# chenchen235/SemStereo

Measured on AMD Instinct MI355X. Metric: stereo pairs/sec, hot segment (gwc+concat volumes, 3-D hourglass stack, soft-argmax), 1024x1024 maxdisp=128, higher is better.
Workload: dtype f32; 1 GPU; BASELINE.json configs[1]: 1024x1024, maxdisp=128, batch=1/GPU x 1 GPU(s); features [B,128,H/4,W/4]+[B,256,H/8,W/8] -> disparity; input_sets_rotated=3, execution=steps round-robin on 6 HIP streams (PairPipeline); bit-identical to one stream, conv_engine=f16x3, hip_graph=False

## Files before the change

### include/semstereo_hip.h

```cpp
#ifndef SEMSTEREO_HIP_H
#define SEMSTEREO_HIP_H

#ifdef __cplusplus
extern "C" {
#endif

typedef void* ss_stream_t;

enum ss_status {
    SS_OK = 0,
    SS_ERR_INVALID = -1,
    SS_ERR_UNSUPPORTED = -2,
    SS_ERR_LAUNCH = -3
};

int ss_abi_version(void);
int ss_reload_tuning(void);
int ss_set_fill_hint(int pairs_in_flight);
int ss_get_fill_hint(void);
const char* ss_status_string(int status);
const char* ss_last_hip_error(void);


int ss_groupwise_correlation_fwd(const float* fea1, const float* fea2, float* out,
                                 int B, int C, int H, int W, int groups, int normalize,
                                 ss_stream_t stream);

int ss_gwc_volume_fwd(const float* ref, const float* tgt, float* out,
                      int B, int C, int H, int W, int dmin, int ndisp, int groups, int normalize,
                      ss_stream_t stream);
int ss_gwc_patch_gate_fwd(const float* ref, const float* tgt, const float* patch_w, const float* gate_logits, float* out,
                          int B, int C, int H, int W, int dmin, int ndisp, int groups, int normalize, ss_stream_t stream);
int ss_gwc_volume_bwd(const float* grad_out, const float* ref, const float* tgt,
                      float* grad_ref, float* grad_tgt,
                      int B, int C, int H, int W, int dmin, int ndisp, int groups,
                      ss_stream_t stream);

int ss_concat_volume_fwd(const float* ref, const float* tgt, float* out,
                         int B, int C, int H, int W, int dmin, int ndisp, int mask_left, ss_stream_t stream);
int ss_concat_volume_bwd(const float* grad_out, float* grad_ref, float* grad_tgt,
                         int B, int C, int H, int W, int dmin, int ndisp, int mask_left, ss_stream_t stream);

int ss_warp_sampled_fwd(const float* x, const float* y, const float* disp,
                        float* y_warped, float* x_warped,
                        int B, int C, int H, int W, int nd, ss_stream_t stream);
int ss_warp_sampled_bwd(const float* grad_y_warped, const float* grad_x_warped, const float* y, const float* disp,
                        float* grad_x, float* grad_y, float* grad_disp, int B, int C, int H, int W, int nd,
                        ss_stream_t stream);
int ss_concat_sampled_fwd(const float* left, const float* right, const float* disp, const float* att,
                          float* out, int B, int C, int H, int W, int nd, ss_stream_t stream);
int ss_concat_sampled_bwd(const float* grad_out, const float* left, const float* right, const float* disp, const float* att,
                          float* grad_left, float* grad_right, float* grad_att, int B, int C, int H, int W, int nd, int margin,
                          ss_stream_t stream);
int ss_concat_sampled_presplit_fwd(const float* right, const float* disp, const float* att, void* xs, int* xexp,
                                   int B, int C, int H, int W, int nd, ss_stream_t stream);
int ss_stem_left_fwd(const float* q, const float* att, float* out, int B, int Cout, int nd, int H, int W,
                     ss_stream_t stream);
int ss_stem_left_fused_fwd(const float* left, const void* wsplit, const float* att, float* out, int B, int C,
                           int Cout, int nd, int H, int W, int nterms, ss_stream_t stream);
int ss_stem_left_mfma_fwd(const float* left, const void* wsplit, const float* att, float* out, int B, int C,
                          int Cout, int nd, int H, int W, ss_stream_t stream);
int ss_pack_stem_left_weights_f16s(const float* w, void* wsplit, int Cout, int C, ss_stream_t stream);
int ss_pack_stem_left_weights_f16s_bytes(int Cout, int C, long long* bytes);
int ss_warp_correlation_fwd(const float* x, const float* y, const float* disp, float* out,
                            int B, int C, int H, int W, int nd, ss_stream_t stream);

int ss_disparity_regression_fwd(const float* prob, float* out, int B, int dmin, int ndisp, int H, int W,
                                ss_stream_t stream);
int ss_disparity_regression_bwd(const float* grad_out, float* grad_prob, int B, int dmin, int ndisp, int H, int W,
                                ss_stream_t stream);
int ss_disparity_variance_fwd(const float* prob, const float* disparity, float* out,
                              int B, int dmin, int ndisp, int H, int W, ss_stream_t stream);
int ss_softmax_regression_fwd(const float* logits, float* prob, float* disp, float* var,
                              int B, int dmin, int ndisp, int H, int W, ss_stream_t stream);
int ss_upsample_softmax_regression_fwd(const float* coarse, float* up, float* disp, float* var,
                                       int B, int dmin, int ndisp, int H, int W, ss_stream_t stream);

int ss_sample_strength_fwd(const float* left, const float* right, const float* pred0, const float* var,
                           const float* gamma, const float* beta, float* strength,
                           int B, int C, int H, int W, ss_stream_t stream);
int ss_topk_candidates_fwd(const float* logits, const float* strength, float* samples, float* att_topk,
                           float* pred_att, int B, int dmin, int ndisp, int H, int W, int k, ss_stream_t stream);

int ss_regression_topk_fwd(const float* cost, const float* samples, float* out,
                           int B, int nd, int H, int W, int k, ss_stream_t stream);
int ss_regression_topk_bwd(const float* grad_out, const float* cost, const float* samples, float* grad_cost,
                           float* grad_samples, int B, int nd, int H, int W, int k, ss_stream_t stream);

int ss_ssr_upsample_fwd(const float* depth_low, const float* weights, const float* pred_label,
                        const float* params, float* out, int B, int h, int w, int num_classes,
                        ss_stream_t stream);
int ss_ssr_param_count(void);
int ss_ssr_upsample_train_fwd(const float* depth_low, const float* weights, const float* pred_label, const float* params,
                              float* out, float* saved, float* rm0, float* rv0, long long* nbt0, float* rma, float* rva,
                              long long* nbta, float* rm1, float* rv1, long long* nbt1, float* rm2, float* rv2, long long* nbt2,
                              float eps0, float epsa, float eps1, float eps2, double mom0, double moma, double mom1, double mom2,
                              int batch_stats, int B, int h, int w, int num_classes, double* workspace, long long workspace_bytes,
                              ss_stream_t stream);
int ss_ssr_upsample_train_bwd(const float* depth_low, const float* weights, const float* pred_label, const float* params,
                              const float* saved, const float* grad_out, float* grad_depth_low, float* grad_weights,
                              float* grad_pred_label, float* grad_params, int batch_stats, int B, int h, int w, int num_classes,
                              double* workspace, long long workspace_bytes, ss_stream_t stream);

int ss_channel_gate_fwd(const float* att_logits, const float* cv, float* out,
                        int B, int C, int D, int H, int W, ss_stream_t stream);

int ss_channel_att_logits_fwd(const float* im, const void* w1_split, const float* scale1, const float* shift1,
                              const void* w2_split, const float* bias2, float* out,
                              int B, int Cin, int Cmid, int Cout, int H, int W, int sigmoid, ss_stream_t stream);

int ss_conv3d_fwd(const float* in, const float* wpack, const float* scale, const float* shift,
                  const float* residual, const float* gate, float* out,
                  int B, int Cin, int D, int H, int W, int Cout, int k, int stride, int relu,
                  ss_stream_t stream);
int ss_conv3d_bf16s_fwd(const float* in, const void* wsplit, const float* scale, const float* shift,
                        const float* residual, const float* gate, float* out,
                        int B, int Cin, int D, int H, int W, int Cout, int stride, int relu, int nterms,
                        ss_stream_t stream);
int ss_conv3d_bf16s_partial_fwd(const float* in, const void* wsplit, const float* partial, const float* scale,
                                const float* shift, const float* gate, float* out,
                                int B, int Cin, int D, int H, int W, int Cout, int relu, int nterms,
                                ss_stream_t stream);
int ss_conv3d_gather_fwd(const float* right, const float* cand, const float* att, const void* wsplit, const float* partial,
                         const float* scale, const float* shift, const float* gate, float* out,
                         int B, int Cin, int nd, int H, int W, int Cout, int relu, int nterms, ss_stream_t stream);
int ss_conv3d_presplit_fwd(const void* xs, const int* xexp, const void* wsplit, const float* partial, const float* scale,
                           const float* shift, const float* gate, float* out, int B, int Cin, int D, int H, int W,
                           int Cout, int relu, ss_stream_t stream);
int ss_pack_conv3d_weights_bf16s(const float* w, void* wsplit, int Cout, int Cin, ss_stream_t stream);
int ss_pack_conv3d_weights_bf16s_bytes(int Cout, int Cin, long long* bytes);
int ss_pack_conv3d_weights_f16s(const float* w, void* wsplit, int Cout, int Cin, ss_stream_t stream);
int ss_pack_conv3d_weights_f16s_bytes(int Cout, int Cin, long long* bytes);
int ss_conv2d_bf16s_fwd(const float* in, const void* wsplit, const float* scale, const float* shift,
                        const float* residual, float* out, int B, int Cin, int H, int W, int Cout, int relu,
                        int nterms, ss_stream_t stream);
int ss_conv2d_bf16s_pair_fwd(const float* in_a, const float* in_b, const void* wsplit, const float* scale, const float* shift,
                             float* out, int B, int Cin, int H, int W, int Cout, int relu, int nterms, ss_stream_t stream);
int ss_pack_conv2d_weights_bf16s(const float* w, void* wsplit, int Cout, int Cin, ss_stream_t stream);
int ss_pack_conv2d_weights_bf16s_bytes(int Cout, int Cin, long long* bytes);
int ss_conv2d_bf16s_cat_fwd(const float* x_a, const float* rem_a, const float* x_b, const float* rem_b, const void* wsplit,
                            const float* scale, const float* shift, float* out, int B, int Csplit, int Cin, int H, int W, int Cout,
                            int relu, int nterms, ss_stream_t stream);
int ss_deconv2d_bf16s_fwd(const float* in, const void* wsplit, const float* scale, const float* shift, float* out, int B, int Cin,
                          int H, int W, int Cout, int relu, int nterms, ss_stream_t stream);
int ss_deconv2d_bf16s_pair_fwd(const float* in_a, const float* in_b, const void* wsplit, const float* scale, const float* shift,
                               float* out, int B, int Cin, int H, int W, int Cout, int relu, int nterms, ss_stream_t stream);
int ss_pack_deconv2d_weights_f16s(const float* w, void* wsplit, int Cin, int Cout, ss_stream_t stream);
int ss_pack_deconv2d_weights_f16s_bytes(int Cin, int Cout, long long* bytes);
int ss_conv2d_k4s2_f16s_fwd(const float* in, const void* wsplit, float* out, int B, int Cin, int H, int W, int Cout, ss_stream_t stream);
int ss_pack_conv2d_k4s2_weights_f16s(const float* w, void* wsplit, int Cout, int Cin, ss_stream_t stream);
int ss_pack_conv2d_k4s2_weights_f16s_bytes(int Cout, int Cin, long long* bytes);
int ss_deconv2d_k4s2_wgrad_fwd(const float* in, const float* grad_out, float* grad_w, float* workspace, int B, int Cin, int H, int W,
                               int Cout, ss_stream_t stream);
int ss_deconv2d_k4s2_wgrad_workspace_bytes(int B, int Cin, int H, int W, int Cout, long long* bytes);
int ss_conv2d_k3_wgrad_fwd(const float* grad_out, const float* in0, const float* in1, float* grad_w, float* workspace, int B, int C0,
                           int C1, int H, int W, int Cout, ss_stream_t stream);
int ss_conv2d_k3_wgrad_workspace_bytes(int B, int C0, int C1, int H, int W, int Cout, long long* bytes);
int ss_conv2d_k1_f16s_fwd(const float* in, const void* wsplit, const float* scale, const float* shift, float* out, int B, int Cin,
                          long long npos, int Cout, int relu, ss_stream_t stream);
int ss_conv2d_k1_f16s_pair_fwd(const float* in_a, const float* in_b, const void* wsplit, const float* scale, const float* shift,
                               float* out, int B, int Cin, long long npos, int Cout, int relu, ss_stream_t stream);
int ss_pack_conv2d_k1_weights_f16s(const float* w, void* wsplit, int Cout, int Cin, ss_stream_t stream);
int ss_pack_conv2d_k1_weights_f16s_bytes(int Cout, int Cin, long long* bytes);
int ss_seghead_logits_fwd(const float* in, const void* wsplit, const float* scale, const float* shift, const float* w2,
                          const float* bias, float* out, int B, int Cin, int H, int W, int K, ss_stream_t stream);
int ss_pack_seghead_weights_f16s(const float* w, void* wsplit, int Cin, ss_stream_t stream);
int ss_pack_seghead_weights_f16s_bytes(int Cin, long long* bytes);
int ss_bilinear_up2_fwd(const float* in, float* out, int B, int C, int H, int W, ss_stream_t stream);
int ss_seghead_tail_fwd(const float* a, const float* w2, const float* bias, float* out, int B, int K, int C, int H, int W, int up2,
                        ss_stream_t stream);
int ss_seghead_tail_bwd(const float* grad_out, const float* a, const float* w2, float* grad_a, float* grad_w2, float* grad_bias,
                        float* workspace, int B, int K, int C, int H, int W, int up2, ss_stream_t stream);
int ss_seghead_tail_workspace_bytes(int B, int K, int C, int H, int W, long long* bytes);
int ss_pack_conv2d_weights_f16s(const float* w, void* wsplit, int Cout, int Cin, ss_stream_t stream);
int ss_pack_conv2d_weights_f16s_bytes(int Cout, int Cin, long long* bytes);
int ss_conv3d_head_bf16s_fwd(const float* in, const void* wsplit, const float* scale, const float* shift,
                             float* out, int B, int Cin, int D, int H, int W, int relu, int nterms,
                             ss_stream_t stream);
int ss_pack_conv3d_head_weights_bf16s(const float* w, void* wsplit, int Cin, ss_stream_t stream);
int ss_pack_conv3d_head_weights_bf16s_bytes(int Cin, long long* bytes);
int ss_pack_conv3d_head_weights_f16s(const float* w, void* wsplit, int Cin, ss_stream_t stream);
int ss_pack_conv3d_head_weights_f16s_bytes(int Cin, long long* bytes);
int ss_conv3d_bf16s_cl_fwd(const float* in, const void* wsplit, const float* scale, const float* shift, float* out,
                           int B, int Cin, int D, int H, int W, int Cout, int relu, int nterms, ss_stream_t stream);
int ss_conv3d_head_bf16s_cl_fwd(const float* in, const void* wsplit, const float* scale, const float* shift,
                                float* out, int B, int Cin, int D, int H, int W, int relu, int nterms,
                                ss_stream_t stream);
int ss_pack_classifier_head_weights(const float* w2, void* out, ss_stream_t stream);
int ss_pack_classifier_head_weights_bytes(long long* bytes);
int ss_conv3d_classifier_fused_fwd(const float* in, const void* wsplit, const float* scale, const float* shift,
                                   const void* head_w, float* patches, float* out, int B, int Cin, int D, int H, int W,
                                   int nterms, ss_stream_t stream);
int ss_regression_topk_patched_fwd(const float* patches, const float* samples, float* out, int B, int nd, int H, int W, int k,
                                   ss_stream_t stream);
int ss_conv3d_pointwise_bf16s_fwd(const float* in, const void* wsplit, const float* scale, const float* shift,
                                  float* out, int B, int Cin, int Cout, long long npos, int relu, int nterms,
                                  ss_stream_t stream);
int ss_pack_pointwise_weights_bf16s(const float* w, void* wsplit, int Cout, int Cin, ss_stream_t stream);
int ss_pack_pointwise_weights_bf16s_bytes(int Cout, int Cin, long long* bytes);

int ss_deconv3d_fwd(const float* in, const float* wpack, const float* scale, const float* shift,
                    const float* skip, const float* skip_wpack, const float* skip_scale, const float* skip_shift,
                    float* out, int B, int Cin, int D, int H, int W, int Cout, int Cs, int relu,
                    ss_stream_t stream);
int ss_deconv3d_bf16s_fwd(const float* in, const void* wsplit, const float* shift, const float* skip,
                          const void* skip_wsplit, float* out, int B, int Cin, int D, int H, int W, int Cout,
                          int Cs, int relu, int nterms, ss_stream_t stream);
int ss_pack_deconv3d_weights_bf16s(const float* wpack, void* wsplit, int Cin, int Cout, int ntaps, ss_stream_t stream);
int ss_pack_deconv3d_weights_bf16s_bytes(int Cin, int Cout, int ntaps, long long* bytes);
int ss_pack_deconv3d_weights_f16s(const float* wpack, void* wsplit, int Cin, int Cout, ss_stream_t stream);
int ss_pack_deconv3d_weights_f16s_bytes(int Cin, int Cout, long long* bytes);
int ss_pack_conv3d_weights(const float* w, float* wpack, int Cout, int Cin, int k, int transposed,
                           ss_stream_t stream);
int ss_conv3d_wgrad_fwd(const float* grad_out, const float* in, float* grad_w, int B, int Cin, int D, int H, int W,
                        int Cout, int stride, ss_stream_t stream);
int ss_conv3d_wgrad_bf16s_fwd(const float* grad_out, const float* in, float* grad_w, float* workspace, int B, int Cin, int D, int H,
                              int W, int Cout, int stride, ss_stream_t stream);

int ss_depthwise_patch_fwd(const float* in, const float* w, const float* gate, float* out,
                           int B, int C, int D, int H, int W, ss_stream_t stream);
int ss_window_attention_fwd(const float* x, const float* wqkv_t, const float* bqkv,
                            const float* wout_t, const float* bout, float* out,
                            int B, int C, int D, int H, int W, int heads, int bd, int bh, int bw,
                            ss_stream_t stream);
int ss_window_attention_core_fwd(const float* qkv, const float* bqkv, float* y, int B, int C, int D, int H,
                                 int W, int heads, int bd, int bh, int bw, ss_stream_t stream);

int ss_batchnorm_train_fwd(const float* x, const float* weight, const float* bias, float* y, float* mean, float* invstd,
                           float* var_unbiased, double* work, int B, int C, long long N, float eps, int relu,
                           ss_stream_t stream);
int ss_batchnorm_train_bwd(const float* grad_y, const float* x, const float* y, const float* mean, const float* invstd,
                           const float* weight, float* grad_x, double* work, int B, int C, long long N, int relu,
                           ss_stream_t stream);
int ss_batchnorm_train_res_fwd(const float* x, const float* residual, const float* weight, const float* bias, float* y, float* mean,
                               float* invstd, float* var_unbiased, double* work, int B, int C, long long N, float eps, int relu,
                               ss_stream_t stream);
int ss_batchnorm_train_res_bwd(const float* grad_y, const float* x, const float* y, const float* mean, const float* invstd,
                               const float* weight, float* grad_x, float* grad_residual, double* work, int B, int C, long long N,
                               int relu, ss_stream_t stream);
int ss_batchnorm_eval_fwd(const float* x, const float* residual, const float* mean, const float* invstd, const float* weight,
                          const float* bias, float* y, int B, int C, long long N, int relu, ss_stream_t stream);
int ss_batchnorm_eval_bwd(const float* grad_y, const float* x, const float* y, const float* mean, const float* invstd,
                          const float* weight, float* grad_x, float* grad_residual, double* work, int B, int C, long long N,
                          int relu, ss_stream_t stream);
int ss_batchnorm_train_fwd_rs(const float* x, const float* residual, const float* weight, const float* bias, float* y, float* mean,
                              float* invstd, float* var_unbiased, double* work, float* running_mean, float* running_var,
                              long long* num_batches_tracked, double momentum, int B, int C, long long N, float eps, int relu,
                              ss_stream_t stream);
int ss_batchnorm_bwd_pg(const float* grad_y, const float* x, const float* y, const float* mean, const float* invstd,
                        const float* weight, const float* bias, float* grad_x, float* grad_residual, double* work, float* grad_weight,
                        float* grad_bias, int batch_statistics, int B, int C, long long N, int relu, ss_stream_t stream);
int ss_group_normalise_fwd(const float* x, float* y, int B, int C, int H, int W, int groups, float eps, ss_stream_t stream);
int ss_group_normalise_bwd(const float* grad_y, const float* x, float* grad_x, int B, int C, int H, int W, int groups, float eps,
                           ss_stream_t stream);
int ss_conv_k1_wgrad_fwd(const float* grad_out, const float* in, float* grad_w, int B, int Cin, int Cout, long long npos,
                         ss_stream_t stream);
int ss_channel_sum_fwd(const float* a, double* sums, int B, int C, long long N, ss_stream_t stream);
int ss_depthwise_patch_wgrad_fwd(const float* grad_out, const float* in, float* grad_w, int B, int C, int D, int H, int W,
                                 ss_stream_t stream);
int ss_channel_gate_bwd_logits(const float* grad_out, const float* cv, const float* att_logits, float* grad_att, int B, int C,
                               int D, int H, int W, ss_stream_t stream);
int ss_window_attention_core_bwd(const float* qkv, const float* grad_y, float* grad_qkv, int B, int C, int D, int H, int W,
                                 int heads, int bd, int bh, int bw, ss_stream_t stream);
int ss_window_attention_core_pad_bwd(const float* qkv, const float* bqkv, const float* grad_y, float* grad_qkv, float* grad_bias, int B,
                                     int C, int D, int H, int W, int heads, int bd, int bh, int bw, ss_stream_t stream);
int ss_upsample_softmax_regression_bwd(const float* up, const float* grad_up, const float* grad_disp, const float* grad_var,
                                       float* grad_coarse, float* work, int B, int dmin, int ndisp, int H, int W, ss_stream_t stream);
int ss_sample_strength_bwd(const float* left, const float* right, const float* pred0, const float* var, const float* gamma,
                           const float* beta, const float* grad_strength, float* grad_left, float* grad_right, float* grad_pred0,
                           float* grad_var, float* grad_gamma_beta, int B, int C, int H, int W, ss_stream_t stream);
int ss_sample_strength_bwd_ws(const float* left, const float* right, const float* pred0, const float* var, const float* gamma,
                              const float* beta, const float* grad_strength, float* grad_left, float* grad_right, float* grad_pred0,
                              float* grad_var, float* grad_gamma_beta, float* work, int B, int C, int H, int W, ss_stream_t stream);
int ss_topk_candidates_bwd(const float* logits, const float* strength, const float* samples, const float* grad_att_topk,
                           const float* grad_pred_att, float* grad_logits, float* grad_strength, int B, int dmin, int ndisp, int H, int W,
                           int k, ss_stream_t stream);
int ss_loss_workspace_bytes(int kind, long long* bytes);
int ss_disparity_loss_fwd(const float* est0, const float* gt0, const unsigned char* mask0, long long n0, const float* est1,
                          const float* gt1, const unsigned char* mask1, long long n1, const float* est2, const float* gt2,
                          const unsigned char* mask2, long long n2, const float* est3, const float* gt3, const unsigned char* mask3,
                          long long n3, float w0, float w1, float w2, float w3, float lo, float hi, int nterms, int l1, double* record,
                          float* loss, double* workspace, long long workspace_bytes, ss_stream_t stream);
int ss_disparity_loss_bwd(const float* est0, const float* gt0, const unsigned char* mask0, float* grad0, long long n0, const float* est1,
                          const float* gt1, const unsigned char* mask1, float* grad1, long long n1, const float* est2, const float* gt2,
                          const unsigned char* mask2, float* grad2, long long n2, const float* est3, const float* gt3,
                          const unsigned char* mask3, float* grad3, long long n3, float w0, float w1, float w2, float w3, float lo,
                          float hi, int nterms, int l1, const double* record, const float* grad_loss, ss_stream_t stream);
int ss_label_loss_fwd(const float* logits, const void* labels, int label_dtype, int B, int num_classes, int H, int W, int ignore, float scale,
                      double* record, float* loss, double* workspace, long long workspace_bytes, ss_stream_t stream);
int ss_label_loss_bwd(const float* logits, const void* labels, int label_dtype, int B, int num_classes, int H, int W, int ignore, float scale,
                      const double* record, const float* grad_loss, float* grad_logits, ss_stream_t stream);
int ss_lrsc_loss_fwd(const float* logits_right, const float* disp, const void* labels, int label_dtype, int B, int num_classes, int H, int W,
                     double* record, float* loss, long long* warped, double* workspace, long long workspace_bytes, ss_stream_t stream);
int ss_lrsc_loss_bwd(const float* logits_right, const float* disp, const void* labels, int label_dtype, int B, int num_classes, int H, int W,
                     const double* record, const float* grad_loss, float* grad_logits, ss_stream_t stream);
int ss_metrics_workspace_bytes(int kind, long long* bytes);
int ss_disparity_metrics_fwd(const float* est0, const float* est1, const float* est2, const float* est3, const float* gt,
                             const unsigned char* mask, const unsigned char* mask_img, int n_est, int B, long long pixels_per_image,
                             float lo, float hi, float t0, float t1, float t2, float t3, int n_thr, float* out, long long* counts,
                             double* sums, void* workspace, long long workspace_bytes, ss_stream_t stream);
int ss_seg_confusion_fwd(const float* logits, const void* labels, int label_dtype, int B, int num_classes, int H, int W,
                         long long label_row_stride, long long label_image_stride, long long* joint, int accumulate, void* workspace,
                         long long workspace_bytes, ss_stream_t stream);
int ss_vis_workspace_bytes(int kind, long long* bytes);
int ss_disp_error_image_fwd(const float* est, const float* gt, const float* table, int B, int H, int W, float abs_thres, float rel_thres,
                            int legend, int is_signed, float lo, float hi, float* out, ss_stream_t stream);
int ss_class_color_fwd(const void* src, int src_dtype, int B, int num_classes, int H, int W, long long label_row_stride,
                       long long label_image_stride, void* out, int out_dtype, ss_stream_t stream);
int ss_image_minmax_fwd(const float* x, int B, long long elements_per_image, float* minmax, void* workspace, long long workspace_bytes,
                        ss_stream_t stream);
int ss_image_normalize_fwd(const float* x, const float* minmax, float* out, int B, int C, long long pixels_per_channel, ss_stream_t stream);
int ss_prep_workspace_bytes(int B, int H, int W, long long* bytes);
int ss_prep_views_fwd(const unsigned char* left, const unsigned char* right, const float* table, int B, int H, int W, float* out_left,
                      float* out_right, ss_stream_t stream);
int ss_prep_pyramid_fwd(const void* disparity, int disp_dtype, float disp_scale, const void* label, int label_dtype,
                        long long label_row_stride, long long label_image_stride, int B, int H, int W, float* disparity_out,
                        float* disparity_4, float* disparity_8, float* disparity_16, float* label_out, float* label_2, float* label_4,
                        ss_stream_t stream);
int ss_prep_luma_stats_fwd(const unsigned char* left, int B, int H, int W, void* workspace, long long workspace_bytes, ss_stream_t stream);
int ss_prep_gradients_fwd(const void* workspace, long long workspace_bytes, int B, int H, int W, float* gx, float* gy, ss_stream_t stream);
int ss_tool_copy_fwd(const void* src, void* dst, long long bytes, ss_stream_t stream);

#ifdef __cplusplus
}
#endif
#endif
```

### semstereo_amd/csrc/deconv3d_bf16s.hip

```cpp
#include <algorithm>
#include <type_traits>

#include "common.h"
#include "split_f16.h"

namespace {

using ss_u32x2 = __attribute__((ext_vector_type(2))) unsigned;

__host__ __device__ constexpr int tap_of(int s) {
    constexpr int T[27] = {13, 14, 16, 17, 22, 23, 25, 26, 12, 15, 21, 24, 10, 11, 19, 20, 9, 18, 4, 5, 7, 8, 3, 6, 1, 2, 0};
    return T[s];
}
__host__ __device__ constexpr int cls_of(int s) {
    constexpr int T[27] = {0, 1, 2, 3, 4, 5, 6, 7, 1, 3, 5, 7, 2, 3, 6, 7, 3, 7, 4, 5, 6, 7, 5, 7, 6, 7, 7};
    return T[s];
}
__host__ __device__ constexpr int off_of(int s) {
    constexpr int T[27] = {0, 0, 0, 0, 0, 0, 0, 0, 1, 1, 1, 1, 2, 2, 2, 2, 3, 3, 4, 4, 4, 4, 5, 5, 6, 6, 7};
    return T[s];
}

constexpr int KST = 27;
#ifndef SS_DECONV_XCD
#define SS_DECONV_XCD 0
#endif
#ifndef SS_DECONV_SKIP_AUX
#define SS_DECONV_SKIP_AUX 0
#endif

struct GrpTable { int ns; int step[KST]; int next_off[KST]; };
constexpr bool grp_has(int grp, int cls) { return grp < 0 || (grp == 0 ? (cls < 2 || cls >= 6) : (cls >= 2 && cls < 6)); }
constexpr GrpTable make_grp_table(int grp) {
    GrpTable t{};
    for (int s = 0; s < KST; ++s)
        if (grp_has(grp, cls_of(s))) t.step[t.ns++] = s;
    for (int k = t.ns; k < KST; ++k) t.step[k] = KST - 1;
    for (int k = 0; k < KST; ++k) {
        t.next_off[k] = -1;
        for (int j = k + 1; j < t.ns; ++j)
            if (off_of(t.step[j]) != off_of(t.step[k])) { t.next_off[k] = off_of(t.step[j]); break; }
    }
    return t;
}
template <int GRP>
struct Grp {
    static constexpr int NA = GRP < 0 ? 8 : 4;
    static constexpr int NQ2 = GRP < 0 ? 4 : 2;
    static constexpr int idx(int cls) { return GRP < 0 ? cls : (GRP == 0 ? (cls < 2 ? cls : cls - 4) : cls - 2); }
    static constexpr int q(int j) { return GRP < 0 ? j : (GRP == 0 ? (j == 0 ? 0 : 3) : (j == 0 ? 1 : 2)); }
    static constexpr GrpTable T = make_grp_table(GRP);
    static constexpr int NS = T.ns;
};
struct GroupSteps { int s[2][16]; };
constexpr GroupSteps make_group_steps() {
    GroupSteps t{};
    for (int k = 0; k < 16; ++k) { t.s[0][k] = Grp<0>::T.step[k]; t.s[1][k] = Grp<1>::T.step[k]; }
    return t;
}
__device__ const GroupSteps kGroupSteps = make_group_steps();

template <int TD, int TH, int LT = 3, bool WLDS = false, int WSTEPS = 27>
struct DB {
    static constexpr int ID = TD + 1, IH = TH + 1, IW = 33;
    static constexpr int CS = ID * IH * IW;
    static constexpr int NPOS = (CS + 255) / 256;
    static constexpr int WSLOTS = WLDS ? WSTEPS * 2 * 64 : 0;
    static constexpr size_t LDS_BYTES = (size_t)(LT * 2 * CS + 1 + 16 + WSLOTS) * 16;
    static_assert(TD * TH == 4, "4 waves x one input row each");
};

template <int TD, int TH, int NTERMS, bool HAS_SKIP, bool SPLIT = false, bool ACCB = false, bool STREAM = false>
__global__ __launch_bounds__(256, (SPLIT && !ACCB) ? 3 : 2) void deconv3d_bf16s(const float* __restrict__ in, const uint4* __restrict__ wsplit,
                                                          const float* __restrict__ shift, const float* __restrict__ skip,
                                                          const uint4* __restrict__ skip_wsplit, float* __restrict__ out,
                                                          int Cin, int D, int H, int W, int Cout, int Cs, int tiles_w,
                                                          int tiles_h, int relu, int nunits) {
    static_assert(!SPLIT || NTERMS == F16X3, "the class-group split exists for the fp16 form (weights through LDS)");
    static_assert(!ACCB || SPLIT, "chunk-blocked accumulation: in the registers the split frees");
    constexpr bool F16 = (NTERMS == F16X3);
    constexpr int NC = (NTERMS == 6) ? 3 : 2;
    constexpr int NCW = F16 ? 2 : 3;
    using C = DB<TD, TH, NC, F16, SPLIT ? 15 : 27>;
    constexpr int MSLOT = NC * 2 * C::CS;
    constexpr int WL = MSLOT + 1 + 16;
    extern __shared__ __attribute__((aligned(16))) uint4 lds[];
    const int tid = threadIdx.x, lane = tid & 63, wave = tid >> 6;
    const int l31 = lane & 31, half = lane >> 5;
    int iw0 = 0, ih0 = 0, id0 = 0, grp = -1;
    auto unit_origin = [&](int u, int& w0, int& h0, int& d0) {
        int t = SPLIT ? (u >> 1) : u;
        const int tw = t % tiles_w; t /= tiles_w;
        const int th = t % tiles_h; t /= tiles_h;
        w0 = tw * 32; h0 = th * TH; d0 = t * TD;
    };
    const int co0 = blockIdx.y * 32;
    const int b = blockIdx.z;
    const int dzw = wave / TH, hyw = wave % TH;
    const int lane_pos = (dzw * C::IH + hyw) * C::IW + l31;

    const size_t in_plane = (size_t)H * W, chan = (size_t)D * in_plane;
    const float* inb = in + (size_t)b * Cin * chan;

    unsigned poff[C::NPOS];
    auto make_poff = [&](int u) {
        int w0, h0, d0;
        unit_origin(u, w0, h0, d0);
#pragma unroll
        for (int i = 0; i < C::NPOS; ++i) {
            const int p = tid + 256 * i;
            const int wx = p % C::IW;
            int r = p / C::IW;
            const int hy = r % C::IH, dz = r / C::IH;
            const int gw = w0 + wx, gh = h0 + hy, gd = d0 + dz;
            const bool ok = (p < C::CS) && gd < D && gh < H && gw < W && u < nunits;
            poff[i] = ok ? (unsigned)(((size_t)gd * in_plane + (size_t)gh * W + gw) * 4) : 0x80000000u;
        }
    };
    constexpr int NQ = 16 * C::NPOS;
    float rin[NQ];

    const int nchunks = (Cin + 15) / 16;
    const int G = nchunks * KST;
    const int wlane = (half * Cout + min(co0 + l31, Cout - 1)) * 16;
    const int wstep = NCW * 2 * Cout * 16;
    const int swstep = 3 * 2 * Cout * 16;
    const float* wunscale = reinterpret_cast<const float*>(reinterpret_cast<const char*>(wsplit) + (size_t)G * wstep);
    const __amdgpu_buffer_rsrc_t wres = __builtin_amdgcn_make_buffer_rsrc(
        const_cast<uint4*>(wsplit), 0, (int)min((long long)G * wstep, 0x7fffffffLL), 0x00020000);
    const __amdgpu_buffer_rsrc_t ires = __builtin_amdgcn_make_buffer_rsrc(
        const_cast<float*>(inb), 0, (int)min((long long)Cin * (long long)chan * 4, 0x7fffffffLL), 0x00020000);
    const int chan_b = (int)(chan * 4);
    auto load_a = [&](int g, int c) {
        return __builtin_bit_cast(uint4, __builtin_amdgcn_raw_buffer_load_b128(wres, wlane, g * wstep + c * 2 * Cout * 16, 0));
    };
    auto load_in = [&](int ch, int i) {
        return __builtin_bit_cast(float, __builtin_amdgcn_raw_buffer_load_b32(ires, (int)poff[i], min(ch, Cin - 1) * chan_b, 0));
    };
    auto load_in_masked = [&](int ch, int i, unsigned mask) {
        return __builtin_bit_cast(float, __builtin_amdgcn_raw_buffer_load_b32(ires, (int)(poff[i] | mask), min(ch, Cin - 1) * chan_b, 0));
    };
    constexpr int AQ = F16 ? 2 : 3;
    uint4 aq[AQ][NC];

    const int Do = 2 * D, Ho = 2 * H, Wo = 2 * W;
    const size_t out_plane = (size_t)Ho * Wo;
    float* aff = reinterpret_cast<float*>(&lds[MSLOT + 1]);
    if (tid < 32) {
        const int co = min(co0 + tid, Cout - 1);
        aff[tid] = shift ? shift[co] : 0.0f;
        aff[32 + tid] = F16 ? wunscale[co] : 1.0f;
    }
    constexpr int SNT = F16 ? 6 : NTERMS, SNC = (SNT == 6) ? 3 : 2;
    auto body = [&](auto grp_tag, const int unit) {
    constexpr int GRP = decltype(grp_tag)::value;
    using GP = Grp<GRP>;
    constexpr int NA = GP::NA, NS = GP::NS;
    constexpr bool XPF = false;
    const bool has_next = XPF && unit + (int)gridDim.x < nunits;
    if (!XPF) {
        make_poff(unit);
#pragma unroll
        for (int q = 0; q < NQ; ++q) rin[q] = load_in(q / C::NPOS, q % C::NPOS);
    }
    if (!F16) {
#pragma unroll
        for (int k = 0; k < 2; ++k)
#pragma unroll
            for (int c = 0; c < NC; ++c) aq[k][c] = load_a(min(k, G - 1), c);
    }
    f32x16 acc[NA];
#pragma unroll
    for (int p = 0; p < NA; ++p)
#pragma unroll
        for (int r = 0; r < 16; ++r) acc[p][r] = 0.f;
    auto skip_phase = [&]() {
#ifdef SS_EXP_DECONV_NOSKIP
        return;
#endif
        const size_t schan = (size_t)Do * out_plane;
        const int jw_ = min(iw0 + l31, W - 1), jd_ = min(id0 + dzw, D - 1), jh_ = min(ih0 + hyw, H - 1);
        const __amdgpu_buffer_rsrc_t sres = __builtin_amdgcn_make_buffer_rsrc(
            const_cast<float*>(skip + (size_t)b * Cs * schan), 0, (int)min((long long)Cs * (long long)schan * 4, 0x7fffffffLL), 0x00020000);
        const int nks = (Cs + 15) / 16;
        const __amdgpu_buffer_rsrc_t swres = __builtin_amdgcn_make_buffer_rsrc(
            const_cast<uint4*>(skip_wsplit), 0, nks * swstep, 0x00020000);
        const unsigned lane_s = (unsigned)(((size_t)(2 * jd_) * out_plane + (size_t)(2 * jh_) * Wo + 2 * jw_) * 4);
        const unsigned schan_b = (unsigned)(schan * 4);
        auto batch_load = [&](float2 (&v)[2][8], int ks, auto q0_tag, unsigned dead) {
            constexpr int q0 = decltype(q0_tag)::value;
#pragma unroll
            for (int q = 0; q < 2; ++q) {
                const unsigned qo = (unsigned)(((size_t)(GP::q(q0 + q) >> 1) * out_plane + (size_t)(GP::q(q0 + q) & 1) * Wo) * 4);
#pragma unroll
                for (int j = 0; j < 8; ++j) {
                    const int cs = ks * 16 + 8 * half + j;
                    v[q][j] = __builtin_bit_cast(float2, __builtin_amdgcn_raw_buffer_load_b64(
                                                             sres, (int)((lane_s + qo + (unsigned)min(cs, Cs - 1) * schan_b) | dead), 0, SS_DECONV_SKIP_AUX));
                }
            }
        };
        auto batch_mfma = [&](float2 (&v)[2][8], int ks, auto q0_tag, const bf16x8 (&a)[SNC]) {
            constexpr int q0 = decltype(q0_tag)::value;
#pragma unroll
            for (int q = 0; q < 2; ++q) {
#pragma unroll
                for (int j = 0; j < 8; ++j)
                    if (ks * 16 + 8 * half + j >= Cs) v[q][j] = make_float2(0.f, 0.f);
#pragma unroll
                for (int pw = 0; pw < 2; ++pw) {
                    unsigned bh[4], bm[4], bl[4];
#pragma unroll
                    for (int c = 0; c < 4; ++c)
                        split3_pk(pw ? v[q][2 * c].y : v[q][2 * c].x, pw ? v[q][2 * c + 1].y : v[q][2 * c + 1].x, bh[c], bm[c], bl[c]);
                    const bf16x8 h8 = __builtin_bit_cast(bf16x8, make_uint4(bh[0], bh[1], bh[2], bh[3]));
                    const bf16x8 m8 = __builtin_bit_cast(bf16x8, make_uint4(bm[0], bm[1], bm[2], bm[3]));
                    const int cls = (q0 + q) * 2 + pw;
                    if (SNT == 6) {
                        const bf16x8 l8 = __builtin_bit_cast(bf16x8, make_uint4(bl[0], bl[1], bl[2], bl[3]));
                        acc[cls] = __builtin_amdgcn_mfma_f32_32x32x16_bf16(a[1], m8, acc[cls], 0, 0, 0);
                        acc[cls] = __builtin_amdgcn_mfma_f32_32x32x16_bf16(a[0], l8, acc[cls], 0, 0, 0);
                        acc[cls] = __builtin_amdgcn_mfma_f32_32x32x16_bf16(a[SNC - 1], h8, acc[cls], 0, 0, 0);
                    }
                    acc[cls] = __builtin_amdgcn_mfma_f32_32x32x16_bf16(a[0], m8, acc[cls], 0, 0, 0);
                    acc[cls] = __builtin_amdgcn_mfma_f32_32x32x16_bf16(a[1], h8, acc[cls], 0, 0, 0);
                    acc[cls] = __builtin_amdgcn_mfma_f32_32x32x16_bf16(a[0], h8, acc[cls], 0, 0, 0);
                }
            }
        };
        using Q0 = std::integral_constant<int, 0>;
        using Q2 = std::integral_constant<int, 2>;
#pragma unroll 1
        for (int ks = 0; ks < nks; ++ks) {
            bf16x8 a[SNC];
#pragma unroll
            for (int c = 0; c < SNC; ++c)
                a[c] = __builtin_bit_cast(bf16x8, __builtin_amdgcn_raw_buffer_load_b128(swres, wlane, ks * swstep + c * 2 * Cout * 16, 0));
            float2 v[2][8];
            batch_load(v, ks, Q0{}, 0u);
            __builtin_amdgcn_sched_barrier(0);
            batch_mfma(v, ks, Q0{}, a);
            if constexpr (GP::NQ2 == 4) {
                batch_load(v, ks, Q2{}, 0u);
                __builtin_amdgcn_sched_barrier(0);
                batch_mfma(v, ks, Q2{}, a);
            }
        }
    };


    const bool skip_first = !SPLIT && HAS_SKIP && ((unit ^ blockIdx.y) & 1);
    if (HAS_SKIP && skip_first) {
        skip_phase();
        if (F16) {
#pragma unroll
            for (int r = 0; r < 16; ++r) {
                const float ws = __uint_as_float((254u << 23) - __float_as_uint(wunscale[min(co0 + (r & 3) + 8 * (r >> 2) + 4 * half, Cout - 1)]));
#pragma unroll
                for (int p = 0; p < NA; ++p) acc[p][r] *= ws;
            }
        }
    }
    BlockExp bexp;
    auto publish_max = [&](float m0) {
        const unsigned wm = wave_max_bits(__float_as_uint(abs_max<false>(rin, m0)));
        if (lane == 0) reinterpret_cast<unsigned*>(&lds[MSLOT])[wave] = wm;
    };
    if (F16) {
        float m0 = 0.f;
        if (HAS_SKIP && skip_first) {
#pragma unroll
            for (int p = 0; p < NA; ++p)
#pragma unroll
                for (int r = 0; r < 16; ++r) m0 = fmaxf(m0, fabsf(acc[p][r]));
            m0 *= pow2_biased(127 - E_INIT_SHIFT);
        }
        publish_max(m0);
        __syncthreads();
    }
    const int nchunks_run = nchunks;
    for (int ck = 0, g0 = 0; ck < nchunks_run; ++ck, g0 += KST) {
        const int ci0 = ck * 16;
        if (F16) {
            int wv = __builtin_amdgcn_readfirstlane(wave);
            asm volatile("" : "+s"(wv));
#pragma unroll
            for (int k = 0; k < (NS * 2 + 3) / 4; ++k) {
                const int i = wv + 4 * k;
                if (i < NS * 2) {
                    const int sg = GRP < 0 ? i / 2 : __builtin_amdgcn_readfirstlane(kGroupSteps.s[GRP < 0 ? 0 : GRP][i / 2]);
                    lds_dma16(wres, &lds[WL + i * 64], wlane, (g0 + sg) * wstep + (i & 1) * 2 * Cout * 16);
                }
            }
        }
        float in_scale = 1.f;
        if (F16) {
            if (bexp.advance(lds[MSLOT])) {
                const float ratio = bexp.rescale();
#pragma unroll
                for (int p = 0; p < NA; ++p)
#pragma unroll
                    for (int r = 0; r < 16; ++r) acc[p][r] *= ratio;
            }
            in_scale = bexp.in_scale();
        }
#pragma unroll
        for (int i = 0; i < C::NPOS; ++i) {
            const int p = tid + 256 * i;
            if (p >= C::CS) continue;
#pragma unroll
            for (int hf = 0; hf < 2; ++hf) {
                unsigned hh[4], mm[4], ll[4];
#pragma unroll
                for (int c = 0; c < 4; ++c) {
                    const int c0 = hf * 8 + 2 * c;
                    const float x0 = (ci0 + c0 < Cin) ? rin[c0 * C::NPOS + i] : 0.f;
                    const float x1 = (ci0 + c0 + 1 < Cin) ? rin[(c0 + 1) * C::NPOS + i] : 0.f;
                    if (F16) split2_pk_f16(x0 * in_scale, x1 * in_scale, hh[c], mm[c]);
                    else split3_pk(x0, x1, hh[c], mm[c], ll[c]);
                }
                lds[(0 * 2 + hf) * C::CS + p] = make_uint4(hh[0], hh[1], hh[2], hh[3]);
                lds[(1 * 2 + hf) * C::CS + p] = make_uint4(mm[0], mm[1], mm[2], mm[3]);
                if (NC == 3) lds[(2 * 2 + hf) * C::CS + p] = make_uint4(ll[0], ll[1], ll[2], ll[3]);
            }
        }
#ifndef SS_EXP_DECONV_NOWAIT
        if (F16) __builtin_amdgcn_s_waitcnt(0x0F70);
#endif
        __syncthreads();
        const bool more = ck + 1 < nchunks;
        if (XPF && !more) make_poff(unit + (int)gridDim.x);
        const unsigned nomore = (more || has_next) ? 0u : 0x80000000u;
        const int ch_next = more ? ci0 + 16 : 0;

        uint4 bcur[NC], bnxt[NC];
        auto read_b = [&](uint4 (&dst)[NC], int o) {
            const int slot = lane_pos + (((o >> 2) & 1) * C::IH + ((o >> 1) & 1)) * C::IW + (o & 1);
#pragma unroll
            for (int c = 0; c < NC; ++c) dst[c] = lds[(c * 2 + half) * C::CS + slot];
        };
        constexpr int QSG = (NQ + (NS * 20 / 27) - 1) / (NS * 20 / 27);
        read_b(bcur, off_of(GP::T.step[0]));
        if (F16) {
#pragma unroll
            for (int c = 0; c < NC; ++c) aq[0][c] = lds[WL + c * 64 + lane];
        }
        f32x16 tacc[ACCB ? NA : 1];
        if constexpr (ACCB) {
#pragma unroll
            for (int p = 0; p < NA; ++p)
#pragma unroll
                for (int r = 0; r < 16; ++r) tacc[p][r] = 0.f;
        }
#pragma unroll
        for (int k = 0; k < NS; ++k) {
            const int s = GP::T.step[k];
            if (!F16) {
#pragma unroll
                for (int c = 0; c < NC; ++c) aq[(s + 2) % AQ][c] = load_a(min(g0 + s + 2, G - 1), c);
            } else if (k + 1 < NS) {
#pragma unroll
                for (int c = 0; c < NC; ++c) aq[(k + 1) % AQ][c] = lds[WL + ((k + 1) * 2 + c) * 64 + lane];
            }
#pragma unroll
            for (int q = k * QSG; q < (k + 1) * QSG && q < NQ; ++q) rin[q] = load_in_masked(ch_next + q / C::NPOS, q % C::NPOS, nomore);
            if ((k == 0 || off_of(s) != off_of(GP::T.step[k > 0 ? k - 1 : 0])) && GP::T.next_off[k] >= 0) read_b(bnxt, GP::T.next_off[k]);
            const int ai = GP::idx(cls_of(s));
            f32x16& dst = ACCB ? tacc[ACCB ? ai : 0] : acc[ai];
            if (F16) {
                f16x8 a[NC], bq[NC];
#pragma unroll
                for (int c = 0; c < NC; ++c) {
                    a[c] = __builtin_bit_cast(f16x8, aq[k % AQ][c]);
                    bq[c] = __builtin_bit_cast(f16x8, bcur[c]);
                }
                dst = __builtin_amdgcn_mfma_f32_32x32x16_f16(a[0], bq[1], dst, 0, 0, 0);
                dst = __builtin_amdgcn_mfma_f32_32x32x16_f16(a[1], bq[0], dst, 0, 0, 0);
                dst = __builtin_amdgcn_mfma_f32_32x32x16_f16(a[0], bq[0], dst, 0, 0, 0);
            } else {
                bf16x8 a[NC], bq[NC];
#pragma unroll
                for (int c = 0; c < NC; ++c) {
                    a[c] = __builtin_bit_cast(bf16x8, aq[s % AQ][c]);
                    bq[c] = __builtin_bit_cast(bf16x8, bcur[c]);
                }
                if (NTERMS == 6) {
                    dst = __builtin_amdgcn_mfma_f32_32x32x16_bf16(a[1], bq[1], dst, 0, 0, 0);
                    dst = __builtin_amdgcn_mfma_f32_32x32x16_bf16(a[0], bq[NC - 1], dst, 0, 0, 0);
                    dst = __builtin_amdgcn_mfma_f32_32x32x16_bf16(a[NC - 1], bq[0], dst, 0, 0, 0);
                }
                dst = __builtin_amdgcn_mfma_f32_32x32x16_bf16(a[0], bq[1], dst, 0, 0, 0);
                dst = __builtin_amdgcn_mfma_f32_32x32x16_bf16(a[1], bq[0], dst, 0, 0, 0);
                dst = __builtin_amdgcn_mfma_f32_32x32x16_bf16(a[0], bq[0], dst, 0, 0, 0);
            }
            if (k + 1 < NS && off_of(GP::T.step[k + 1 < NS ? k + 1 : k]) != off_of(s)) {
#pragma unroll
                for (int c = 0; c < NC; ++c) bcur[c] = bnxt[c];
            }
            __builtin_amdgcn_sched_barrier(0);
        }
        if constexpr (ACCB) {
#pragma unroll
            for (int p = 0; p < NA; ++p)
#pragma unroll
                for (int r = 0; r < 16; ++r) acc[p][r] += tacc[p][r];
        }
        if (F16 && more) publish_max(0.f);
        __syncthreads();
    }
    if (F16) {
        const float au = bexp.acc_unscale();
#pragma unroll
        for (int r = 0; r < 16; ++r) {
            const float un = au * aff[32 + (r & 3) + 8 * (r >> 2) + 4 * half];
#pragma unroll
            for (int p = 0; p < NA; ++p) acc[p][r] *= un;
        }
    }

    if (HAS_SKIP && !skip_first) skip_phase();

    const int jw = iw0 + l31, jd = id0 + dzw, jh = ih0 + hyw;
    const unsigned ochan_b = (unsigned)((size_t)Do * out_plane * 4);
    const __amdgpu_buffer_rsrc_t ores = __builtin_amdgcn_make_buffer_rsrc(
        out + (size_t)b * Cout * Do * out_plane, 0, (int)min((long long)Cout * (long long)ochan_b, 0x7fffffffLL), 0x00020000);
    const bool ok = jw < W && jd < D && jh < H;
    unsigned vo[GP::NQ2];
#pragma unroll
    for (int j = 0; j < GP::NQ2; ++j)
        vo[j] = ok ? (unsigned)((((size_t)(2 * jd + (GP::q(j) >> 1)) * Ho + 2 * jh + (GP::q(j) & 1)) * Wo + 2 * jw) * 4) + 4u * half * ochan_b
                   : 0x80000000u;
    const float floor_v = relu ? 0.f : -__builtin_inff();
#pragma unroll
    for (int r = 0; r < 16; ++r) {
        const int cb = co0 + (r & 3) + 8 * (r >> 2);
        const bool cok = cb + 4 * half < Cout;
        const float sh = aff[(r & 3) + 8 * (r >> 2) + 4 * half];
#pragma unroll
        for (int j = 0; j < GP::NQ2; ++j) {
            const float v0 = fmaxf(ss::add_rn(acc[j * 2 + 0][r], sh), floor_v);
            const float v1 = fmaxf(ss::add_rn(acc[j * 2 + 1][r], sh), floor_v);
#ifdef SS_EXP_DECONV_NOSTORE
            if (r == 0 && j == 0)
#endif
            __builtin_amdgcn_raw_buffer_store_b64(__builtin_bit_cast(ss_u32x2, make_float2(v0, v1)), ores,
                                                  (int)(cok ? vo[j] : 0x80000000u), cb * (int)ochan_b, STREAM ? 2 : 0);
        }
    }
    };
#if SS_DECONV_XCD
    const int unit = [&]() {
        const int x = blockIdx.x & 7, j = blockIdx.x >> 3, q = nunits >> 3, r = nunits & 7;
        return x * q + min(x, r) + j;
    }();
#else
    const int unit = blockIdx.x;
#endif
    unit_origin(unit, iw0, ih0, id0);
    if constexpr (!SPLIT) {
        body(std::integral_constant<int, -1>{}, unit);
    } else {
        grp = unit & 1;
        if (grp == 0) body(std::integral_constant<int, 0>{}, unit);
        else body(std::integral_constant<int, 1>{}, unit);
    }
}

__global__ void pack_deconv_weights_kernel(const float* __restrict__ wpack, unsigned short* __restrict__ wsplit, int Cin,
                                           int Cout, int ntaps, long long total) {
    const long long i = blockIdx.x * (long long)blockDim.x + threadIdx.x;
    if (i >= total) return;
    const int j = (int)(i % 8);
    long long r = i / 8;
    const int co = (int)(r % Cout); r /= Cout;
    const int hf = (int)(r % 2); r /= 2;
    const int term = (int)(r % 3); r /= 3;
    const int s = (int)(r % ntaps);
    const int chunk = (int)(r / ntaps);
    const int ci = chunk * 16 + hf * 8 + j;
    const int tap = (ntaps == 27) ? tap_of(s) : 0;
    const float x = (ci < Cin) ? wpack[((size_t)ci * ntaps + tap) * Cout + co] : 0.f;
    unsigned h, m, l;
    split3_pk(x, 0.f, h, m, l);
    wsplit[i] = (unsigned short)((term == 0 ? h : (term == 1 ? m : l)) & 0xffffu);
}

__global__ __launch_bounds__(256) void deconv_weight_unscale_f16s_kernel(const float* __restrict__ wpack, float* __restrict__ wunscale,
                                                                          int Cout, int rows) {
    __shared__ unsigned wmax[4];
    float m = 0.f;
    for (int i = threadIdx.x; i < rows; i += 256) m = fmaxf(m, fabsf(wpack[(size_t)i * Cout + blockIdx.x]));
    const float u = weight_unscale(m, wmax);
    if (threadIdx.x == 0) wunscale[blockIdx.x] = u;
}
__global__ void pack_deconv_weights_f16s_kernel(const float* __restrict__ wpack, unsigned short* __restrict__ wsplit,
                                                const float* __restrict__ wunscale, int Cin, int Cout, long long total) {
    const long long i = blockIdx.x * (long long)blockDim.x + threadIdx.x;
    if (i >= total) return;
    const int j = (int)(i % 8);
    long long r = i / 8;
    const int co = (int)(r % Cout); r /= Cout;
    const int hf = (int)(r % 2); r /= 2;
    const int term = (int)(r % 2); r /= 2;
    const int s = (int)(r % 27);
    const int chunk = (int)(r / 27);
    const int ci = chunk * 16 + hf * 8 + j;
    const float x = (ci < Cin) ? wpack[((size_t)ci * 27 + tap_of(s)) * Cout + co] / wunscale[co] : 0.f;
    wsplit[i] = split_weight_f16(x, term);
}

template <int TD, int TH, int NTERMS, bool HAS_SKIP, bool SPLIT = false, bool ACCB = false, bool STREAM = false>
int launch_db(const float* in, const void* wsplit, const float* shift, const float* skip, const void* skip_wsplit, float* out,
              int B, int Cin, int D, int H, int W, int Cout, int Cs, int relu, hipStream_t st) {
    using C = DB<TD, TH, (NTERMS == 6) ? 3 : 2, NTERMS == F16X3, SPLIT ? 15 : 27>;
    const int tiles_w = ss::ceil_div(W, 32), tiles_h = ss::ceil_div(H, TH), tiles_d = ss::ceil_div(D, TD);
    const long long nt = (long long)tiles_w * tiles_h * tiles_d;
    if (nt > 0x7fffffffLL || B > 65535) return SS_ERR_UNSUPPORTED;
    auto kern = deconv3d_bf16s<TD, TH, NTERMS, HAS_SKIP, SPLIT, ACCB, STREAM>;
    if (C::LDS_BYTES > 64 * 1024) {
        if (ss::ensure_dynamic_lds(reinterpret_cast<const void*>(kern), (int)C::LDS_BYTES) != SS_OK) return SS_ERR_LAUNCH;
    }
    if (nt > 0x3fffffffLL) return SS_ERR_UNSUPPORTED;
    const long long nunits = SPLIT ? 2 * nt : nt;
    dim3 grid((unsigned)nunits, ss::ceil_div(Cout, 32), B);
    hipLaunchKernelGGL(kern, grid, dim3(256), C::LDS_BYTES, st, in, reinterpret_cast<const uint4*>(wsplit), shift, skip,
                       reinterpret_cast<const uint4*>(skip_wsplit), out, Cin, D, H, W, Cout, Cs, tiles_w, tiles_h, relu, (int)nunits);
    return ss::check_launch();
}

template <int TD, int TH>
int launch_db_all(const float* in, const void* wsplit, const float* shift, const float* skip, const void* skip_wsplit,
                  float* out, int B, int Cin, int D, int H, int W, int Cout, int Cs, int relu, int nterms, hipStream_t st) {
#define SS_DB(NTERMS, HAS_SKIP) launch_db<TD, TH, NTERMS, HAS_SKIP>(in, wsplit, shift, skip, skip_wsplit, out, B, Cin, D, H, W, Cout, Cs, relu, st)
#define SS_DF(HAS_SKIP, SPLIT, ACCB, STREAM) \
    launch_db<TD, TH, F16X3, HAS_SKIP, SPLIT, ACCB, STREAM>(in, wsplit, shift, skip, skip_wsplit, out, B, Cin, D, H, W, Cout, Cs, relu, st)
    if (nterms == F16X3) {
        const long long per_pair = (long long)ss::ceil_div(W, 32) * ss::ceil_div(H, TH) * ss::ceil_div(D, TD) * ss::ceil_div(Cout, 32);
        int groups = ss::tuning().deconv_groups;
        if (groups < 0) groups = per_pair < 256 ? 2 : 0;
        const int stream_env = ss::tuning().deconv_stream;
        const bool stream = stream_env >= 0 ? stream_env != 0 : (long long)B * Cout * 8 * D * H * W * 4 >= (192LL << 20);
        if (groups == 2) return skip != nullptr ? SS_DF(true, true, true, false) : SS_DF(false, true, true, false);
        if (groups == 1) return skip != nullptr ? SS_DF(true, true, false, false) : SS_DF(false, true, false, false);
        if (stream) return skip != nullptr ? SS_DF(true, false, false, true) : SS_DF(false, false, false, true);
        return skip != nullptr ? SS_DF(true, false, false, false) : SS_DF(false, false, false, false);
    }
    if (skip != nullptr) return nterms == 6 ? SS_DB(6, true) : SS_DB(3, true);
    return nterms == 6 ? SS_DB(6, false) : SS_DB(3, false);
#undef SS_DF
#undef SS_DB
}

}

static ss::Packed deconv_packed(int Cin, int Cout, int ntaps, bool f16) {
    const long long terms = (long long)ss::ceil_div(Cin, 16) * ntaps * (f16 ? 2 : 3) * 2 * Cout * 16;
    return {terms, terms + (f16 ? 4LL * Cout : 0)};
}

extern "C" int ss_pack_deconv3d_weights_bf16s_bytes(int Cin, int Cout, int ntaps, long long* bytes) {
    SS_REQUIRE(bytes && Cin > 0 && Cout > 0 && (ntaps == 27 || ntaps == 1));
    *bytes = deconv_packed(Cin, Cout, ntaps, false).total;
    return SS_OK;
}

extern "C" int ss_pack_deconv3d_weights_f16s_bytes(int Cin, int Cout, long long* bytes) {
    SS_REQUIRE(bytes && Cin > 0 && Cout > 0);
    *bytes = deconv_packed(Cin, Cout, 27, true).total;
    return SS_OK;
}

extern "C" int ss_pack_deconv3d_weights_bf16s(const float* wpack, void* wsplit, int Cin, int Cout, int ntaps, ss_stream_t stream) {
    SS_REQUIRE(wpack && wsplit && Cin > 0 && Cout > 0 && (ntaps == 27 || ntaps == 1));
    const long long total = deconv_packed(Cin, Cout, ntaps, false).terms / 2;
    hipLaunchKernelGGL(pack_deconv_weights_kernel, dim3((unsigned)ss::ceil_div_ll(total, 256)), dim3(256), 0, ss::as_stream(stream),
                       wpack, reinterpret_cast<unsigned short*>(wsplit), Cin, Cout, ntaps, total);
    return ss::check_launch();
}

extern "C" int ss_pack_deconv3d_weights_f16s(const float* wpack, void* wsplit, int Cin, int Cout, ss_stream_t stream) {
    SS_REQUIRE(wpack && wsplit && Cin > 0 && Cout > 0);
    const ss::Packed p = deconv_packed(Cin, Cout, 27, true);
    const long long total = p.terms / 2;
    float* wunscale = ss::scales_of(wsplit, p);
    hipLaunchKernelGGL(deconv_weight_unscale_f16s_kernel, dim3(Cout), dim3(256), 0, ss::as_stream(stream), wpack, wunscale, Cout, Cin * 27);
    hipLaunchKernelGGL(pack_deconv_weights_f16s_kernel, dim3((unsigned)ss::ceil_div_ll(total, 256)), dim3(256), 0, ss::as_stream(stream),
                       wpack, reinterpret_cast<unsigned short*>(wsplit), wunscale, Cin, Cout, total);
    return ss::check_launch();
}

extern "C" int ss_deconv3d_bf16s_fwd(const float* in, const void* wsplit, const float* shift, const float* skip,
                                     const void* skip_wsplit, float* out, int B, int Cin, int D, int H, int W, int Cout,
                                     int Cs, int relu, int nterms, ss_stream_t stream) {
    SS_REQUIRE(in && wsplit && out);
    SS_REQUIRE(B > 0 && Cin > 0 && D > 0 && H > 0 && W > 0 && Cout > 0 && (nterms == 3 || nterms == 6 || nterms == F16X3));
    SS_REQUIRE((skip == nullptr) || (skip_wsplit != nullptr && Cs > 0));
    SS_REQUIRE((reinterpret_cast<uintptr_t>(wsplit) & 15) == 0 && (reinterpret_cast<uintptr_t>(skip_wsplit) & 15) == 0);
    if ((reinterpret_cast<uintptr_t>(out) & 7) != 0) return SS_ERR_INVALID;
    if ((long long)Cin * D * H * W * 4 >= 0x7fffffffLL) return SS_ERR_UNSUPPORTED;
    if (skip != nullptr && (long long)Cs * 8 * D * H * W * 4 >= 0x7fffffffLL) return SS_ERR_UNSUPPORTED;
    if ((long long)Cout * 8 * D * H * W * 4 >= 0x7fffffffLL) return SS_ERR_UNSUPPORTED;
    hipStream_t st = ss::as_stream(stream);
    if (D >= 2 && H < 4)
        return launch_db_all<2, 2>(in, wsplit, shift, skip, skip_wsplit, out, B, Cin, D, H, W, Cout, Cs, relu, nterms, st);
    return launch_db_all<1, 4>(in, wsplit, shift, skip, skip_wsplit, out, B, Cin, D, H, W, Cout, Cs, relu, nterms, st);
}
```

### semstereo_amd/csrc/window_attention.hip

```cpp
#include <algorithm>

#include "common.h"
#include "split_f16.h"

namespace {


constexpr int HD = 8;
constexpr int HG = 4;

template <int T, int C>
struct ACfg {
    static constexpr int NTL = (T + 31) / 32;
    static constexpr int TP = NTL * 32;
    static constexpr int XS = C * TP;
    static constexpr int QKV = 3 * 32 * TP;
    static constexpr int YG = 32 * TP;
    static constexpr int FLAGS = TP;
    static constexpr int WL = C * 96;
    static constexpr size_t LDS_BYTES = (size_t)(XS + QKV + YG + FLAGS + WL) * 4;
};

template <int T, int C>
__global__ __launch_bounds__(256) void window_attention_kernel(
    const float* __restrict__ x, const float* __restrict__ wqkv_t, const float* __restrict__ bqkv,
    const float* __restrict__ wout_t, const float* __restrict__ bout, float* __restrict__ out, int D, int H, int W,
    int bd, int bh, int bw, int nwh, int nww, int use_mask) {
    using A = ACfg<T, C>;
    extern __shared__ __attribute__((aligned(16))) float lds[];
    float* xs = lds;
    float* qkv = xs + A::XS;
    float* yg = qkv + A::QKV;
    float* flag = yg + A::YG;
    float* wl = flag + A::FLAGS;

    const int tid = threadIdx.x, lane = tid & 63, wave = tid >> 6;
    const int l31 = lane & 31, half = lane >> 5;
    int wi = blockIdx.x;
    const int ww = wi % nww; wi /= nww;
    const int wh = wi % nwh; wi /= nwh;
    const int wd = wi;
    const int b = blockIdx.y;
    const size_t plane = (size_t)H * W, vol = (size_t)D * plane;
    const float* xb = x + (size_t)b * C * vol;

    if (bw == 4 && (W & 3) == 0 && ((reinterpret_cast<uintptr_t>(x) & 15) == 0)) {
        constexpr int NQ = C * (A::TP / 4) / 256;
        static_assert(C * (A::TP / 4) % 256 == 0, "whole batches");
#pragma unroll
        for (int i = 0; i < NQ; ++i) {
            const int e = tid + 256 * i;
            const int tq = e % (A::TP / 4), c = e / (A::TP / 4);
            const int ih = tq % bh, id = tq / bh;
            const int gh = wh * bh + ih, gd = wd * bd + id, gw = ww * 4;
            const bool ok = gh < H && gw < W;
            const float4 q = *reinterpret_cast<const float4*>(xb + (size_t)c * vol + (size_t)gd * plane +
                                                              (size_t)min(gh, H - 1) * W + min(gw, W - 4));
            *reinterpret_cast<float4*>(&xs[e * 4]) = ok ? q : make_float4(0.f, 0.f, 0.f, 0.f);
        }
    } else {
        for (int e = tid; e < C * A::TP; e += 256) {
            const int t = e % A::TP, c = e / A::TP;
            float v = 0.f;
            if (t < T) {
                const int iw = t % bw, ih = (t / bw) % bh, id = t / (bw * bh);
                const int gw = ww * bw + iw, gh = wh * bh + ih, gd = wd * bd + id;
                if (gh < H && gw < W) v = xb[(size_t)c * vol + (size_t)gd * plane + (size_t)gh * W + gw];
            }
            xs[e] = v;
        }
    }
    for (int t = tid; t < A::TP; t += 256) {
        float f = 0.f;
        if (t < T) {
            const int iw = t % bw, ih = (t / bw) % bh;
            f = ((wh * bh + ih >= H) || (ww * bw + iw >= W)) ? 1.f : 0.f;
        }
        flag[t] = f;
    }
    __syncthreads();

    static_assert(C == 128, "4 waves x 32 output channels");
    f32x16 oacc[A::NTL];
#pragma unroll
    for (int n = 0; n < A::NTL; ++n)
#pragma unroll
        for (int r = 0; r < 16; ++r) oacc[n][r] = 0.f;

    const float scale = 0.35355339059327379f;
    constexpr int NGROUPS = C / (HG * HD);

    constexpr int NWQ = C * 24 / 256;
    float4 wreg[NWQ];
    const float* wsrc[NWQ];
#pragma unroll
    for (int i = 0; i < NWQ; ++i) {
        const int e = tid + 256 * i;
        wsrc[i] = wqkv_t + (size_t)(e / 24) * 3 * C + ((e % 24) / 8) * C + ((e % 24) % 8) * 4;
        wreg[i] = *reinterpret_cast<const float4*>(wsrc[i]);
    }

    for (int g = 0; g < NGROUPS; ++g) {
#pragma unroll
        for (int i = 0; i < NWQ; ++i) {
            const int e = tid + 256 * i;
            *reinterpret_cast<float4*>(&wl[(e / 24) * 96 + (e % 24) * 4]) = wreg[i];
        }
        __syncthreads();
        if (g + 1 < NGROUPS) {
#pragma unroll
            for (int i = 0; i < NWQ; ++i) wreg[i] = *reinterpret_cast<const float4*>(wsrc[i] + (g + 1) * 32);
        }
        for (int u = wave; u < 3 * A::NTL; u += 4) {
            const int mt = u / A::NTL, nt = u % A::NTL;
            const int f0 = mt * C + g * 32;
            f32x16 acc;
#pragma unroll
            for (int r = 0; r < 16; ++r) acc[r] = 0.f;
            const float* ap = wl + half * 96 + mt * 32 + l31;
            const float* bp = xs + half * A::TP + nt * 32 + l31;
#pragma unroll 8
            for (int kk = 0; kk < C; kk += 2)
                acc = __builtin_amdgcn_mfma_f32_32x32x2f32(ap[kk * 96], bp[kk * A::TP], acc, 0, 0, 0);
#pragma unroll
            for (int r = 0; r < 16; ++r) {
                const int row = (r & 3) + 8 * (r >> 2) + 4 * half;
                qkv[(mt * 32 + row) * A::TP + nt * 32 + l31] = ss::add_rn(acc[r], bqkv[f0 + row]);
            }
        }
        __syncthreads();

        static_assert(A::TP == T, "windows of 64 / 96 tokens are whole 32-token tiles");
        for (int u = wave; u < HG * A::NTL; u += 4) {
            const int hh = u / A::NTL, qt = u % A::NTL;
            f32x16 st[A::NTL];
#pragma unroll
            for (int kt = 0; kt < A::NTL; ++kt) {
#pragma unroll
                for (int r = 0; r < 16; ++r) st[kt][r] = 0.f;
#pragma unroll
                for (int sd = 0; sd < HD / 2; ++sd)
                    st[kt] = __builtin_amdgcn_mfma_f32_32x32x2f32(
                        qkv[(32 + hh * HD + 2 * sd + half) * A::TP + kt * 32 + l31],
                        qkv[(hh * HD + 2 * sd + half) * A::TP + qt * 32 + l31],
                        st[kt], 0, 0, 0);
            }
            const float fq = flag[qt * 32 + l31];
            float mx = -INFINITY;
#pragma unroll
            for (int kt = 0; kt < A::NTL; ++kt)
#pragma unroll
                for (int r = 0; r < 16; ++r) {
                    float d = ss::mul_rn(st[kt][r], scale);
                    if (use_mask && flag[kt * 32 + (r & 3) + 8 * (r >> 2) + 4 * half] != fq) d = ss::add_rn(d, -1000.0f);
                    st[kt][r] = d;
                    mx = fmaxf(mx, d);
                }
            mx = fmaxf(mx, __shfl_xor(mx, 32));
            float sum = 0.f;
#pragma unroll
            for (int kt = 0; kt < A::NTL; ++kt)
#pragma unroll
                for (int r = 0; r < 16; ++r) { st[kt][r] = ss::exp_fast(st[kt][r] - mx); sum = ss::add_rn(sum, st[kt][r]); }
            sum = ss::add_rn(sum, __shfl_xor(sum, 32));
            const float rsum = 1.0f / sum;
            f32x16 ot;
#pragma unroll
            for (int r = 0; r < 16; ++r) ot[r] = 0.f;
            const float* vrow = qkv + (64 + hh * HD + (l31 & 7)) * A::TP + 4 * half;
#pragma unroll
            for (int kt = 0; kt < A::NTL; ++kt)
#pragma unroll
                for (int r = 0; r < 16; ++r) {
                    const float vv = (l31 < HD) ? vrow[kt * 32 + (r & 3) + 8 * (r >> 2)] : 0.f;
                    ot = __builtin_amdgcn_mfma_f32_32x32x2f32(vv, ss::mul_rn(st[kt][r], rsum), ot, 0, 0, 0);
                }
#pragma unroll
            for (int r = 0; r < 4; ++r) yg[(hh * HD + 4 * half + r) * A::TP + qt * 32 + l31] = ot[r];
        }
        __syncthreads();

        {
            const float* ap = wout_t + (size_t)(g * 32 + half) * C + wave * 32 + l31;
            const float* bp = yg + half * A::TP + l31;
#pragma unroll
            for (int kk = 0; kk < 32; kk += 2) {
                const float a = ap[(size_t)kk * C];
#pragma unroll
                for (int n = 0; n < A::NTL; ++n)
                    oacc[n] = __builtin_amdgcn_mfma_f32_32x32x2f32(a, bp[kk * A::TP + n * 32], oacc[n], 0, 0, 0);
            }
        }
        __syncthreads();
    }

    float* ob = out + (size_t)b * C * vol;
#pragma unroll
    for (int n = 0; n < A::NTL; ++n) {
        const int t = n * 32 + l31;
        if (t >= T) continue;
        const int iw = t % bw, ih = (t / bw) % bh, id = t / (bw * bh);
        const int gw = ww * bw + iw, gh = wh * bh + ih, gd = wd * bd + id;
        if (gh >= H || gw >= W) continue;
        const size_t pos = (size_t)gd * plane + (size_t)gh * W + gw;
#pragma unroll
        for (int r = 0; r < 16; ++r) {
            const int co = wave * 32 + (r & 3) + 8 * (r >> 2) + 4 * half;
            ob[(size_t)co * vol + pos] = ss::add_rn(oacc[n][r], bout[co]);
        }
    }
}

template <int T, int C>
__global__ __launch_bounds__(256) void window_attention_core(const float* __restrict__ qkv_in, const float* __restrict__ bqkv,
                                                              float* __restrict__ y, int D, int H, int W, int bd, int bh,
                                                              int bw, int nwh, int nww, int use_mask) {
    using A = ACfg<T, C>;
    static_assert(A::TP == T, "windows of 64 / 96 tokens are whole 32-token tiles");
    __shared__ __attribute__((aligned(16))) float qkv[3 * 32 * A::TP];
    __shared__ float flag[A::TP];
    const int tid = threadIdx.x, lane = tid & 63, wave = tid >> 6;
    const int l31 = lane & 31, half = lane >> 5;
    constexpr int NGROUPS = C / (HG * HD);
    int wi = blockIdx.x;
    const int g = wi % NGROUPS; wi /= NGROUPS;
    const int ww = wi % nww; wi /= nww;
    const int wh = wi % nwh; wi /= nwh;
    const int wd = wi;
    const int b = blockIdx.y;
    const size_t plane = (size_t)H * W, vol = (size_t)D * plane;
    const float* qb = qkv_in + (size_t)b * 3 * C * vol;

    __shared__ unsigned vmax_w[4];
    float vm = 0.f;
    if (bw == 4 && (W & 3) == 0 && ((reinterpret_cast<uintptr_t>(qkv_in) & 15) == 0)) {
        constexpr int NQ = 96 * (A::TP / 4) / 256;
        static_assert(96 * (A::TP / 4) % 256 == 0, "whole batches");
#pragma unroll
        for (int i = 0; i < NQ; ++i) {
            const int e = tid + 256 * i;
            const int tq = e % (A::TP / 4), row = e / (A::TP / 4);
            const int f = (row >> 5) * C + g * 32 + (row & 31);
            const int ih = tq % bh, id = tq / bh;
            const int gh = wh * bh + ih, gd = wd * bd + id, gw = ww * 4;
            const bool ok = gh < H && gw < W;
            const float4 q = *reinterpret_cast<const float4*>(qb + (size_t)f * vol + (size_t)gd * plane +
                                                              (size_t)min(gh, H - 1) * W + min(gw, W - 4));
            const float bf = bqkv[f];
            const float4 v4 = ok ? q : make_float4(bf, bf, bf, bf);
            *reinterpret_cast<float4*>(&qkv[e * 4]) = v4;
            if (row >= 64) vm = fmaxf(vm, fmaxf(fmaxf(fabsf(v4.x), fabsf(v4.y)), fmaxf(fabsf(v4.z), fabsf(v4.w))));
        }
    } else {
        for (int e = tid; e < 96 * A::TP; e += 256) {
            const int t = e % A::TP, row = e / A::TP;
            const int f = (row >> 5) * C + g * 32 + (row & 31);
            const int iw = t % bw, ih = (t / bw) % bh, id = t / (bw * bh);
            const int gw = ww * bw + iw, gh = wh * bh + ih, gd = wd * bd + id;
            const float v1 = (gh < H && gw < W) ? qb[(size_t)f * vol + (size_t)gd * plane + (size_t)gh * W + gw] : bqkv[f];
            qkv[e] = v1;
            if (row >= 64) vm = fmaxf(vm, fabsf(v1));
        }
    }
    {
        const unsigned wm = wave_max_bits(__float_as_uint(vm));
        if (lane == 0) vmax_w[wave] = wm;
    }
    for (int t = tid; t < A::TP; t += 256) {
        const int iw = t % bw, ih = (t / bw) % bh;
        flag[t] = ((wh * bh + ih >= H) || (ww * bw + iw >= W)) ? 1.f : 0.f;
    }
    __syncthreads();

    const float scale = 0.35355339059327379f;
    const int e_v = workgroup_exponent(vmax_w);
    const float v_scale = scale_for(e_v);
    const float pv_unscale = unscale_for(e_v) * (1.0f / 16384.0f);
    for (int wk = tid; wk < 32 * (A::TP / 16); wk += 256) {
        float* base = qkv + (64 + wk / (A::TP / 16)) * A::TP + (wk % (A::TP / 16)) * 16;
        float f[16];
#pragma unroll
        for (int k4 = 0; k4 < 4; ++k4) ss::lds_read16(base + 4 * k4, &f[4 * k4]);
#pragma unroll
        for (int h = 0; h < 2; ++h) {
            unsigned hi[4], lo[4];
#pragma unroll
            for (int j = 0; j < 4; ++j) {
                const int t0 = (j < 2) ? 4 * h + 2 * j : 8 + 4 * h + 2 * (j - 2);
                split2_pk_f16(f[t0] * v_scale, f[t0 + 1] * v_scale, hi[j], lo[j]);
            }
            *reinterpret_cast<uint4*>(base + 8 * h) = make_uint4(hi[0], hi[1], hi[2], hi[3]);
            *reinterpret_cast<uint4*>(base + 8 * h + 4) = make_uint4(lo[0], lo[1], lo[2], lo[3]);
        }
    }
    __syncthreads();
    float* yb = y + (size_t)b * C * vol;
    for (int u = wave; u < HG * A::NTL; u += 4) {
        const int hh = u / A::NTL, qt = u % A::NTL;
        f32x16 st[A::NTL];
#pragma unroll
        for (int kt = 0; kt < A::NTL; ++kt) {
#pragma unroll
            for (int r = 0; r < 16; ++r) st[kt][r] = 0.f;
#pragma unroll
            for (int sd = 0; sd < HD / 2; ++sd)
                st[kt] = __builtin_amdgcn_mfma_f32_32x32x2f32(
                    qkv[(32 + hh * HD + 2 * sd + half) * A::TP + kt * 32 + l31],
                    qkv[(hh * HD + 2 * sd + half) * A::TP + qt * 32 + l31],
                    st[kt], 0, 0, 0);
        }
        const float fq = flag[qt * 32 + l31];
        float mx = -INFINITY;
#pragma unroll
        for (int kt = 0; kt < A::NTL; ++kt)
#pragma unroll
            for (int r = 0; r < 16; ++r) {
                float d = ss::mul_rn(st[kt][r], scale);
                if (use_mask && flag[kt * 32 + (r & 3) + 8 * (r >> 2) + 4 * half] != fq) d = ss::add_rn(d, -1000.0f);
                st[kt][r] = d;
                mx = fmaxf(mx, d);
            }
        mx = fmaxf(mx, __shfl_xor(mx, 32));
        float sum = 0.f;
#pragma unroll
        for (int kt = 0; kt < A::NTL; ++kt)
#pragma unroll
            for (int r = 0; r < 16; ++r) { st[kt][r] = ss::exp_fast(st[kt][r] - mx); sum = ss::add_rn(sum, st[kt][r]); }
        sum = ss::add_rn(sum, __shfl_xor(sum, 32));
        const float rsum = 1.0f / sum;
        f32x16 ot;
#pragma unroll
        for (int r = 0; r < 16; ++r) ot[r] = 0.f;
        const float* vrow = qkv + (64 + hh * HD + (l31 & 7)) * A::TP + 8 * half;
        const float ps = rsum * 16384.0f;
#pragma unroll
        for (int kt = 0; kt < A::NTL; ++kt)
#pragma unroll
            for (int s8 = 0; s8 < 2; ++s8) {
                float vh[4], vl[4];
                ss::lds_read16(vrow + kt * 32 + 16 * s8, vh);
                ss::lds_read16(vrow + kt * 32 + 16 * s8 + 4, vl);
                unsigned bh_[4], bl_[4];
#pragma unroll
                for (int j = 0; j < 4; ++j)
                    split2_pk_f16(st[kt][8 * s8 + 2 * j] * ps, st[kt][8 * s8 + 2 * j + 1] * ps, bh_[j], bl_[j]);
                const f16x8 a_hi = __builtin_bit_cast(f16x8, make_float4(vh[0], vh[1], vh[2], vh[3]));
                const f16x8 a_lo = __builtin_bit_cast(f16x8, make_float4(vl[0], vl[1], vl[2], vl[3]));
                const f16x8 b_hi = __builtin_bit_cast(f16x8, make_uint4(bh_[0], bh_[1], bh_[2], bh_[3]));
                const f16x8 b_lo = __builtin_bit_cast(f16x8, make_uint4(bl_[0], bl_[1], bl_[2], bl_[3]));
                ot = __builtin_amdgcn_mfma_f32_32x32x16_f16(a_hi, b_lo, ot, 0, 0, 0);
                ot = __builtin_amdgcn_mfma_f32_32x32x16_f16(a_lo, b_hi, ot, 0, 0, 0);
                ot = __builtin_amdgcn_mfma_f32_32x32x16_f16(a_hi, b_hi, ot, 0, 0, 0);
            }
#pragma unroll
        for (int r = 0; r < 4; ++r) ot[r] *= pv_unscale;
        const int t = qt * 32 + l31;
        const int iw = t % bw, ih = (t / bw) % bh, id = t / (bw * bh);
        const int gw = ww * bw + iw, gh = wh * bh + ih, gd = wd * bd + id;
        if (gh < H && gw < W) {
            const size_t pos = (size_t)gd * plane + (size_t)gh * W + gw;
#pragma unroll
            for (int r = 0; r < 4; ++r) yb[(size_t)(g * 32 + hh * HD + 4 * half + r) * vol + pos] = ot[r];
        }
    }
}

template <int T>
int launch_attn_core(const float* qkv, const float* bqkv, float* y, int B, int D, int H, int W, int bd, int bh, int bw,
                     hipStream_t st) {
    const int nwd = D / bd, nwh = ss::ceil_div(H, bh), nww = ss::ceil_div(W, bw);
    const int use_mask = (H % bh != 0) && (W % bw != 0);
    const long long nblk = (long long)nwd * nwh * nww * (128 / (HG * HD));
    if (nblk > 0x7fffffffLL || B > 65535) return SS_ERR_UNSUPPORTED;
    hipLaunchKernelGGL((window_attention_core<T, 128>), dim3((unsigned)nblk, B), dim3(256), 0, st, qkv, bqkv, y, D, H, W, bd,
                       bh, bw, nwh, nww, use_mask);
    return ss::check_launch();
}

template <int T>
int launch_attn(const float* x, const float* wqkv_t, const float* bqkv, const float* wout_t, const float* bout,
                float* out, int B, int D, int H, int W, int bd, int bh, int bw, hipStream_t st) {
    using A = ACfg<T, 128>;
    const int nwd = D / bd, nwh = ss::ceil_div(H, bh), nww = ss::ceil_div(W, bw);
    const int use_mask = (H % bh != 0) && (W % bw != 0);
    auto kern = window_attention_kernel<T, 128>;
    if (A::LDS_BYTES > 64 * 1024) {
        if (ss::ensure_dynamic_lds(reinterpret_cast<const void*>(kern), (int)A::LDS_BYTES) != SS_OK) return SS_ERR_LAUNCH;
    }
    const long long nwin = (long long)nwd * nwh * nww;
    if (nwin > 0x7fffffffLL || B > 65535) return SS_ERR_UNSUPPORTED;
    hipLaunchKernelGGL(kern, dim3((unsigned)nwin, B), dim3(256), A::LDS_BYTES, st, x, wqkv_t, bqkv, wout_t, bout, out, D,
                       H, W, bd, bh, bw, nwh, nww, use_mask);
    return ss::check_launch();
}

}

extern "C" int ss_window_attention_fwd(const float* x, const float* wqkv_t, const float* bqkv, const float* wout_t,
                                       const float* bout, float* out, int B, int C, int D, int H, int W, int heads,
                                       int bd, int bh, int bw, ss_stream_t stream) {
    SS_REQUIRE(x && wqkv_t && bqkv && wout_t && bout && out);
    SS_REQUIRE(B > 0 && C > 0 && D > 0 && H > 0 && W > 0 && heads > 0 && bd > 0 && bh > 0 && bw > 0);
    SS_REQUIRE(D % bd == 0);
    if (C != 128 || heads != 16) return SS_ERR_UNSUPPORTED;
    const int T = bd * bh * bw;
    hipStream_t st = ss::as_stream(stream);
    if (T == 64) return launch_attn<64>(x, wqkv_t, bqkv, wout_t, bout, out, B, D, H, W, bd, bh, bw, st);
    if (T == 96) return launch_attn<96>(x, wqkv_t, bqkv, wout_t, bout, out, B, D, H, W, bd, bh, bw, st);
    return SS_ERR_UNSUPPORTED;
}

extern "C" int ss_window_attention_core_fwd(const float* qkv, const float* bqkv, float* y, int B, int C, int D, int H,
                                            int W, int heads, int bd, int bh, int bw, ss_stream_t stream) {
    SS_REQUIRE(qkv && bqkv && y);
    SS_REQUIRE(B > 0 && C > 0 && D > 0 && H > 0 && W > 0 && heads > 0 && bd > 0 && bh > 0 && bw > 0);
    SS_REQUIRE(D % bd == 0);
    if (C != 128 || heads != 16) return SS_ERR_UNSUPPORTED;
    const int T = bd * bh * bw;
    hipStream_t st = ss::as_stream(stream);
    if (T == 64) return launch_attn_core<64>(qkv, bqkv, y, B, D, H, W, bd, bh, bw, st);
    if (T == 96) return launch_attn_core<96>(qkv, bqkv, y, B, D, H, W, bd, bh, bw, st);
    return SS_ERR_UNSUPPORTED;
}
```

### semstereo_amd/engine.py

```python
import os
import weakref

import torch
import torch.nn as nn

from . import _lib, ops
from ._host import PATH_COUNTS, _c
from ._lib import call, ptr


def _inference(module, *tensors):
    if module.training:
        return False
    if torch.is_grad_enabled():
        if any(t is not None and t.requires_grad for t in tensors):
            return False
        if any(p.requires_grad for p in module.parameters()):
            return False
        if module.__dict__.get("_is_replica", False):
            for m in module.modules():
                if any(p is not None and p.requires_grad for p in getattr(m, "_former_parameters", {}).values()):
                    return False
    return True


_CACHE_GENERATION = [0]
_RETIRED = []
_RETAIN = [0]


def cache_generation():
    return _CACHE_GENERATION[0]


def retain_replaced(on):
    _RETAIN[0] = max(0, _RETAIN[0] + (1 if on else -1))


def drop_retired():
    del _RETIRED[:]


RETIRED_CAP = 256


def _note_build(old):
    _CACHE_GENERATION[0] += 1
    if old is not None and _RETAIN[0]:
        _RETIRED.append(old)
        if len(_RETIRED) > RETIRED_CAP:
            del _RETIRED[:len(_RETIRED) - RETIRED_CAP]


class _ParamCache:

    def __init__(self):
        self._store = {}
        self.owner = None

    def get(self, key, sources, build):
        stamp = tuple((t.data_ptr(), t._version, str(t.device)) for t in sources)
        hit = self._store.get(key)
        if hit is None or hit[0] != stamp:
            _note_build(hit)
            with torch.no_grad():
                hit = (stamp, build())
            self._store[key] = hit
        return hit[1]


class _ReplicaCache:

    def __init__(self, shared, owner, device):
        self.shared, self.owner, self.device = shared, owner, str(device)

    def get(self, key, sources, build):
        stamp = tuple((t.data_ptr(), t._version) for t in list(self.owner.parameters()) + list(self.owner.buffers()))
        k = ("replica", self.device, key)
        hit = self.shared._store.get(k)
        if hit is None or hit[0] != stamp:
            _note_build(hit)
            with torch.no_grad():
                hit = (stamp, build())
            self.shared._store[k] = hit
        return hit[1]


def _cache(module):
    c = module.__dict__.get("_ss_cache")
    if module.__dict__.get("_is_replica", False):
        owner = c.owner() if c is not None and c.owner is not None else None
        if owner is None:
            return _ParamCache()
        dev_ = next((t.device for t in list(module.__dict__.get("_former_parameters", {}).values()) + list(module.buffers()) if t is not None), "?")
        for m in module.modules():
            fp = [t for t in getattr(m, "_former_parameters", {}).values() if t is not None]
            if fp:
                dev_ = fp[0].device
                break
        return _ReplicaCache(c, owner, dev_)
    if c is None:
        c = module.__dict__["_ss_cache"] = _ParamCache()
        c.owner = weakref.ref(module)
    return c


def fold_bn(bn):
    invstd = 1.0 / torch.sqrt(bn.running_var + bn.eps)
    scale = (bn.weight * invstd) if bn.weight is not None else invstd
    shift = (bn.bias if bn.bias is not None else 0.0) - bn.running_mean * scale
    return scale.float().contiguous(), shift.float().contiguous()


def _packed_affine(owner, key, conv, bn, pack, bias=False):
    b = conv.bias if bias else None
    srcs = [conv.weight] + ([b] if b is not None else []) + ([bn.weight, bn.bias, bn.running_mean, bn.running_var] if bn is not None else [])

    def build():
        sc, sh = fold_bn(bn) if bn is not None else (None, None)
        if b is not None:
            sh = (b.detach().float() if bn is None else sh + sc * b.detach().float()).contiguous()
        return pack(conv.weight), sc, sh
    return _cache(owner).get(key, srcs, build)


def pack_conv_weight(w, transposed=False):
    w = w.detach().float().contiguous()
    _lib.require_device(w)
    if transposed:
        Cin, Cout, k = w.shape[0], w.shape[1], w.shape[2]
    else:
        Cout, Cin, k = w.shape[0], w.shape[1], w.shape[2]
    assert w.shape[2] == w.shape[3] == w.shape[4], "cubic kernels only"
    out = torch.empty((Cin, k * k * k, Cout), dtype=torch.float32, device=w.device)
    with torch.cuda.device(w.device):
        call("ss_pack_conv3d_weights", ptr(w), ptr(out), Cout, Cin, k, int(transposed))
    return out


def _pack(entry, w, *dims):
    w = _c(w.detach().float())
    _lib.require_device(w)
    out = torch.empty(_lib.query_bytes(entry + "_bytes", *dims) // 2, dtype=torch.int16, device=w.device)
    with torch.cuda.device(w.device):
        call(entry, ptr(w), ptr(out), *dims)
    return out


def conv3d_hip(x, wpack, scale, shift, k, stride, relu, residual=None, gate=None):
    x = _c(x)
    dev = _lib.require_device(x, wpack, scale, shift, residual, gate)
    B, Cin, D, H, W = x.shape
    assert wpack.shape[0] == Cin and wpack.shape[1] == k ** 3
    Cout = wpack.shape[2]
    pad = k // 2
    Do, Ho, Wo = [(n + 2 * pad - k) // stride + 1 for n in (D, H, W)]
    out = torch.empty((B, Cout, Do, Ho, Wo), dtype=x.dtype, device=x.device)
    if residual is not None:
        assert residual.shape == out.shape and residual.is_contiguous()
    if gate is not None:
        assert gate.shape == (B, Cout, Ho, Wo) and gate.is_contiguous()
    with torch.cuda.device(dev):
        call("ss_conv3d_fwd", ptr(x), ptr(wpack), ptr(scale), ptr(shift), ptr(residual), ptr(gate), ptr(out),
             B, Cin, D, H, W, Cout, k, stride, int(relu))
    return out


def deconv3d_hip(x, wpack, shift, relu, skip=None, skip_wpack=None):
    x = _c(x)
    dev = _lib.require_device(x, wpack, shift, skip, skip_wpack)
    B, Cin, D, H, W = x.shape
    Cout = wpack.shape[2]
    out = torch.empty((B, Cout, 2 * D, 2 * H, 2 * W), dtype=x.dtype, device=x.device)
    Cs = 0
    if skip is not None:
        skip = _c(skip)
        Cs = skip.shape[1]
        assert skip.shape == (B, Cs, 2 * D, 2 * H, 2 * W) and skip_wpack.shape == (Cs, Cout)
    with torch.cuda.device(dev):
        call("ss_deconv3d_fwd", ptr(x), ptr(wpack), None, ptr(shift), ptr(skip), ptr(skip_wpack), None, None,
             ptr(out), B, Cin, D, H, W, Cout, Cs, int(relu))
    return out


def pack_deconv_weight_bf16s(wpack, nterms=6):
    Cin, Cout = wpack.shape[0], wpack.shape[-1]
    ntaps = 1 if wpack.dim() == 2 else wpack.shape[1]
    if nterms == 19:
        assert ntaps == 27
        return _pack("ss_pack_deconv3d_weights_f16s", wpack, Cin, Cout)
    return _pack("ss_pack_deconv3d_weights_bf16s", wpack, Cin, Cout, ntaps)


def deconv3d_bf16s_hip(x, wsplit, Cout, shift, relu, nterms, skip=None, skip_wsplit=None):
    x = _c(x)
    dev = _lib.require_device(x, shift, skip)
    B, Cin, D, H, W = x.shape
    out = torch.empty((B, Cout, 2 * D, 2 * H, 2 * W), dtype=x.dtype, device=x.device)
    Cs = 0
    if skip is not None:
        skip = _c(skip)
        Cs = skip.shape[1]
        assert skip.shape == (B, Cs, 2 * D, 2 * H, 2 * W)
    with torch.cuda.device(dev):
        call("ss_deconv3d_bf16s_fwd", ptr(x), ptr(wsplit), ptr(shift), ptr(skip), ptr(skip_wsplit), ptr(out),
             B, Cin, D, H, W, Cout, Cs, int(relu), int(nterms))
    return out


CONV_ENGINE = os.environ.get("SS_CONV_ENGINE", "f16x3")
_NTERMS_TILED = {"bf16x6": 6, "bf16x3": 3, "f16x3": 19}
_NTERMS_AUX = {"bf16x6": 6, "bf16x3": 3, "f16x3": 6, "f32": 6}


def _tiled_nterms():
    return _NTERMS_TILED[CONV_ENGINE]


def _aux_nterms():
    return _NTERMS_AUX[CONV_ENGINE]


DECONV_F16 = os.environ.get("SS_DECONV_F16", "1") != "0"


def _deconv_nterms():
    return _NTERMS_TILED[CONV_ENGINE] if DECONV_F16 else _NTERMS_AUX[CONV_ENGINE]
DECONV_MIN_WORKGROUPS = int(os.environ.get("SS_DECONV_MIN_WGS", "0"))
DECONV_BF16S = os.environ.get("SS_DECONV_BF16S", "1") != "0"


def pack_conv_weight_bf16s(w, nterms=6):
    Cout, Cin = w.shape[0], w.shape[1]
    assert tuple(w.shape[2:]) == (3, 3, 3)
    return _pack("ss_pack_conv3d_weights_f16s" if nterms == 19 else "ss_pack_conv3d_weights_bf16s", w, Cout, Cin)


def conv3d_bf16s_hip(x, wsplit, Cout, scale, shift, relu, nterms, residual=None, gate=None, partial=None, stride=1):
    x = _c(x)
    dev = _lib.require_device(x, scale, shift, residual, gate, partial)
    B, Cin, D, H, W = x.shape
    Do, Ho, Wo = [(n - 1) // stride + 1 for n in (D, H, W)]
    out = torch.empty((B, Cout, Do, Ho, Wo), dtype=x.dtype, device=x.device)
    if gate is not None:
        assert gate.shape == (B, Cout, Ho, Wo) and gate.is_contiguous()
    with torch.cuda.device(dev):
        if partial is not None:
            assert residual is None and stride == 1 and partial.shape == out.shape and partial.is_contiguous()
            call("ss_conv3d_bf16s_partial_fwd", ptr(x), ptr(wsplit), ptr(partial), ptr(scale), ptr(shift), ptr(gate), ptr(out),
                 B, Cin, D, H, W, Cout, int(relu), int(nterms))
        else:
            call("ss_conv3d_bf16s_fwd", ptr(x), ptr(wsplit), ptr(scale), ptr(shift), ptr(residual), ptr(gate), ptr(out),
                 B, Cin, D, H, W, Cout, int(stride), int(relu), int(nterms))
    return out


def classifier_cl_hip(x, ws0, scale0, shift0, nterms0, ws2, nterms2):
    x = _c(x)
    dev = _lib.require_device(x, scale0, shift0)
    B, C, D, H, W = x.shape
    mid = torch.empty((B, D, H, W, C), dtype=x.dtype, device=x.device)
    out = torch.empty((B, 1, D, H, W), dtype=x.dtype, device=x.device)
    with torch.cuda.device(dev):
        call("ss_conv3d_bf16s_cl_fwd", ptr(x), ptr(ws0), ptr(scale0), ptr(shift0), ptr(mid), B, C, D, H, W, C, 1, int(nterms0))
        call("ss_conv3d_head_bf16s_cl_fwd", ptr(mid), ptr(ws2), None, None, ptr(out), B, C, D, H, W, 0, int(nterms2))
    return out


def classifier_fused_applies(x, nterms0):
    if not (x.is_cuda and x.dtype == torch.float32 and x.dim() == 5 and nterms0 == 19):
        return False
    B, C, D, H, W = x.shape
    return (C % 8 == 0 and D % 4 == 0 and ((W + 31) // 32) * ((H + 7) // 8) * ((D + 1) // 2) >= 512 and C * D * H * W * 4 < 0x7fffffff
            and H <= 65535 and B * D <= 65535)


def pack_classifier_head_weight(w2):
    assert tuple(w2.shape) == (1, 32, 3, 3, 3)
    return _pack("ss_pack_classifier_head_weights", w2)


class PatchedCost:

    def __init__(self, patches, shape):
        self.patches, self.shape = patches, tuple(shape)


CLASSIFIER_FOLD = os.environ.get("SS_CLASSIFIER_FOLD", "0") != "0"


def classifier_fused_hip(x, ws0, scale0, shift0, nterms0, head_w, sum_patches=True):
    x = _c(x)
    dev = _lib.require_device(x, scale0, shift0)
    B, C, D, H, W = x.shape
    ntiles = ((W + 31) // 32) * ((H + 3) // 4) * (D // 4)
    patches = torch.empty((B, ntiles, 6 * 6 * 34), dtype=x.dtype, device=x.device)
    out = torch.empty((B, 1, D, H, W), dtype=x.dtype, device=x.device) if sum_patches else None
    with torch.cuda.device(dev):
        call("ss_conv3d_classifier_fused_fwd", ptr(x), ptr(ws0), ptr(scale0), ptr(shift0), ptr(head_w), ptr(patches), ptr(out),
             B, C, D, H, W, int(nterms0))
    return out if sum_patches else PatchedCost(patches, (B, D, H, W))


def pack_conv2d_weight_bf16s(w, nterms=6):
    Cout, Cin = w.shape[0], w.shape[1]
    assert tuple(w.shape[2:]) == (3, 3)
    return _pack("ss_pack_conv2d_weights_f16s" if nterms == 19 else "ss_pack_conv2d_weights_bf16s", w, Cout, Cin)


def conv2d_bf16s_hip(x, wsplit, Cout, scale, shift, relu, nterms, residual=None):
    x = _c(x)
    dev = _lib.require_device(x, scale, shift, residual)
    B, Cin, H, W = x.shape
    out = torch.empty((B, Cout, H, W), dtype=x.dtype, device=x.device)
    with torch.cuda.device(dev):
        call("ss_conv2d_bf16s_fwd", ptr(x), ptr(wsplit), ptr(scale), ptr(shift), ptr(residual), ptr(out), B, Cin, H, W, Cout,
             int(relu), int(nterms))
    return out


def _is_plain_3x3(conv):
    return (isinstance(conv, nn.Conv2d) and conv.kernel_size == (3, 3) and conv.stride == (1, 1) and conv.padding == (1, 1)
            and conv.dilation == (1, 1) and conv.groups == 1 and conv.bias is None and conv.padding_mode == "zeros")


_c2d = os.environ.get("SS_CONV2D_HIP", "auto")
CONV2D_HIP = "auto" if _c2d == "auto" else (_c2d != "0")


def _conv2d_hip_on():
    return CONV_ENGINE == "f16x3" if CONV2D_HIP == "auto" else bool(CONV2D_HIP)


def run_conv2d(owner, key, conv, bn, x, relu):
    if not (_conv2d_hip_on() and CONV_ENGINE != "f32" and _is_plain_3x3(conv) and x.is_cuda):
        return None
    nterms = _tiled_nterms()
    ws, scale, shift = _packed_affine(owner, key + "/2d_" + CONV_ENGINE, conv, bn, lambda w: pack_conv2d_weight_bf16s(w, nterms))
    return conv2d_bf16s_hip(x, ws, conv.out_channels, scale, shift, relu, nterms)


def run_conv2d_pair(owner, key, conv, bn, xa, xb, relu):
    if not (_conv2d_hip_on() and CONV_ENGINE != "f32" and _is_plain_3x3(conv) and xa.is_cuda and xb.is_cuda
            and xa.shape == xb.shape and xa.dtype == xb.dtype == torch.float32):
        return None
    nterms = _tiled_nterms()
    ws, scale, shift = _packed_affine(owner, key + "/2d_" + CONV_ENGINE, conv, bn, lambda w: pack_conv2d_weight_bf16s(w, nterms))
    xa, xb = xa.contiguous(), xb.contiguous()
    dev = _lib.require_device(xa, xb, scale, shift)
    B, Cin, H, W = xa.shape
    out = torch.empty((2 * B, conv.out_channels, H, W), dtype=xa.dtype, device=xa.device)
    with torch.cuda.device(dev):
        call("ss_conv2d_bf16s_pair_fwd", ptr(xa), ptr(xb), ptr(ws), ptr(scale), ptr(shift), ptr(out), B, Cin, H, W,
             conv.out_channels, int(relu), int(nterms))
    return out


def run_conv2d_cat(owner, key, conv, bn, xa, rema, relu, xb=None, remb=None):
    ts = [xa, rema] + ([xb, remb] if xb is not None else [])
    Cs, Cin = xa.shape[1], xa.shape[1] + rema.shape[1]
    if not (_decoder_hip_on() and CONV_ENGINE != "f32" and _is_plain_3x3(conv) and conv.in_channels == Cin and Cs % 8 == 0
            and all(t.is_cuda and t.dtype == torch.float32 and t.dim() == 4 for t in ts)
            and xa.shape[0] == rema.shape[0] and xa.shape[2:] == rema.shape[2:]
            and (xb is None or (xb.shape == xa.shape and remb.shape == rema.shape))):
        return None
    nterms = _tiled_nterms()
    ws, scale, shift = _packed_affine(owner, key + "/2d_" + CONV_ENGINE, conv, bn, lambda w: pack_conv2d_weight_bf16s(w, nterms))
    ts = [t.contiguous() for t in ts]
    dev = _lib.require_device(*ts, scale, shift)
    B, _, H, W = xa.shape
    out = torch.empty(((2 if xb is not None else 1) * B, conv.out_channels, H, W), dtype=xa.dtype, device=xa.device)
    with torch.cuda.device(dev):
        call("ss_conv2d_bf16s_cat_fwd", ptr(ts[0]), ptr(ts[1]), ptr(ts[2]) if xb is not None else None, ptr(ts[3]) if xb is not None else None,
             ptr(ws), ptr(scale), ptr(shift), ptr(out), B, Cs, Cin, H, W, conv.out_channels, int(relu), int(nterms))
    return out


_dec = os.environ.get("SS_DECODER_HIP", "auto")
DECODER_HIP = "auto" if _dec == "auto" else (_dec != "0")


def _decoder_hip_on():
    return CONV_ENGINE == "f16x3" if DECODER_HIP == "auto" else bool(DECODER_HIP)


def _is_deconv_k4s2(conv):
    return (isinstance(conv, nn.ConvTranspose2d) and conv.kernel_size == (4, 4) and conv.stride == (2, 2) and conv.padding == (1, 1)
            and conv.output_padding == (0, 0) and conv.dilation == (1, 1) and conv.groups == 1)


def pack_deconv2d_weight(w):
    Cin, Cout = w.shape[0], w.shape[1]
    assert tuple(w.shape[2:]) == (4, 4)
    return _pack("ss_pack_deconv2d_weights_f16s", w, Cin, Cout)


def deconv2d_bf16s_hip(x, wsplit, Cout, scale, shift, relu, xb=None):
    x = _c(x)
    dev = _lib.require_device(x, xb, scale, shift)
    B, Cin, H, W = x.shape
    out = torch.empty(((2 if xb is not None else 1) * B, Cout, 2 * H, 2 * W), dtype=x.dtype, device=x.device)
    with torch.cuda.device(dev):
        if xb is not None:
            xb = _c(xb)
            assert xb.shape == x.shape
            call("ss_deconv2d_bf16s_pair_fwd", ptr(x), ptr(xb), ptr(wsplit), ptr(scale), ptr(shift), ptr(out), B, Cin, H, W, Cout,
                 int(relu), 19)
        else:
            call("ss_deconv2d_bf16s_fwd", ptr(x), ptr(wsplit), ptr(scale), ptr(shift), ptr(out), B, Cin, H, W, Cout, int(relu), 19)
    return out


def run_deconv2d(owner, key, deconv, bn, x, relu, xb=None):
    if not (_decoder_hip_on() and CONV_ENGINE == "f16x3" and _is_deconv_k4s2(deconv) and x.is_cuda and x.dtype == torch.float32
            and x.dim() == 4 and x.shape[1] == deconv.in_channels and (bn is None or deconv.bias is None)
            and (xb is None or (xb.is_cuda and xb.shape == x.shape and xb.dtype == x.dtype))):
        return None
    ws, scale, shift = _packed_affine(owner, key + "/dc2d_f16s", deconv, bn, pack_deconv2d_weight, bias=True)
    return deconv2d_bf16s_hip(x, ws, deconv.out_channels, scale, shift, relu, xb)


_hd = os.environ.get("SS_HEADS_HIP", "auto")
HEADS_HIP = "auto" if _hd == "auto" else (_hd != "0")


def _heads_hip_on():
    return CONV_ENGINE == "f16x3" if HEADS_HIP == "auto" else bool(HEADS_HIP)


def _is_conv_k1(conv):
    return (isinstance(conv, nn.Conv2d) and conv.kernel_size == (1, 1) and conv.stride == (1, 1) and conv.padding == (0, 0)
            and conv.dilation == (1, 1) and conv.groups == 1)


def pack_conv2d_k1_weight(w):
    Cout, Cin = w.shape[0], w.shape[1]
    assert w.numel() == Cout * Cin
    return _pack("ss_pack_conv2d_k1_weights_f16s", w, Cout, Cin)


def conv2d_k1_f16s_hip(x, wsplit, Cout, scale, shift, relu, xb=None):
    x = _c(x)
    dev = _lib.require_device(x, xb, scale, shift)
    B, Cin, H, W = x.shape
    out = torch.empty(((2 if xb is not None else 1) * B, Cout, H, W), dtype=x.dtype, device=x.device)
    with torch.cuda.device(dev):
        if xb is not None:
            xb = _c(xb)
            assert xb.shape == x.shape
            call("ss_conv2d_k1_f16s_pair_fwd", ptr(x), ptr(xb), ptr(wsplit), ptr(scale), ptr(shift), ptr(out), B, Cin, H * W, Cout,
                 int(relu))
        else:
            call("ss_conv2d_k1_f16s_fwd", ptr(x), ptr(wsplit), ptr(scale), ptr(shift), ptr(out), B, Cin, H * W, Cout, int(relu))
    return out


def run_conv2d_k1(owner, key, conv, bn, x, relu, xb=None):
    if not (_heads_hip_on() and CONV_ENGINE == "f16x3" and _is_conv_k1(conv) and conv.in_channels % 8 == 0
            and isinstance(x, torch.Tensor) and x.is_cuda and x.dtype == torch.float32 and x.dim() == 4
            and x.shape[1] == conv.in_channels and x.numel() > 0
            and max(conv.in_channels, conv.out_channels) * x.shape[2] * x.shape[3] * 4 < 0x7fffffff
            and (xb is None or (xb.is_cuda and xb.shape == x.shape and xb.dtype == x.dtype))):
        return None
    ws, scale, shift = _packed_affine(owner, key + "/k1_f16s", conv, bn, pack_conv2d_k1_weight, bias=True)
    return conv2d_k1_f16s_hip(x, ws, conv.out_channels, scale, shift, relu, xb)


def pack_seghead_weight(w):
    Cin = w.shape[1]
    assert tuple(w.shape) == (32, Cin, 3, 3) and Cin % 8 == 0
    return _pack("ss_pack_seghead_weights_f16s", w, Cin)


def bilinear_up2_hip(x):
    x = _c(x)
    dev = _lib.require_device(x)
    B, C, H, W = x.shape
    out = torch.empty((B, C, 2 * H, 2 * W), dtype=x.dtype, device=x.device)
    with torch.cuda.device(dev):
        call("ss_bilinear_up2_fwd", ptr(x), ptr(out), B, C, H, W)
    return out


def seghead_applies(head, x):
    a, b = head.conv1, head.conv2
    return (_heads_hip_on() and CONV_ENGINE == "f16x3" and _is_plain_3x3(a.conv) and a.conv.out_channels == 32
            and a.conv.in_channels % 8 == 0 and a.use_bn and a.relu and _is_conv_k1(b) and b.bias is not None
            and b.in_channels == 32 and b.out_channels <= 8 and head.scale_factor in (None, 2)
            and isinstance(x, torch.Tensor) and x.is_cuda and x.dtype == torch.float32 and x.dim() == 4
            and x.shape[1] == a.conv.in_channels and x.numel() > 0 and x.shape[1] * x.shape[2] * x.shape[3] * 4 < 0x7fffffff)


def run_seghead(owner, head, x):
    if not seghead_applies(head, x):
        return None
    a, b = head.conv1, head.conv2
    srcs = [a.conv.weight, a.bn.weight, a.bn.bias, a.bn.running_mean, a.bn.running_var, b.weight, b.bias]

    def build():
        sc, sh = fold_bn(a.bn)
        return (pack_seghead_weight(a.conv.weight), sc, sh, b.weight.detach().float().reshape(b.out_channels, 32).contiguous(),
                b.bias.detach().float().contiguous())
    ws, scale, shift, w2, bias = _cache(owner).get("seghead_f16s", srcs, build)
    x = _c(x)
    dev = _lib.require_device(x, scale, shift, w2, bias)
    B, Cin, H, W = x.shape
    logits = torch.empty((B, b.out_channels, H, W), dtype=x.dtype, device=x.device)
    with torch.cuda.device(dev):
        call("ss_seghead_logits_fwd", ptr(x), ptr(ws), ptr(scale), ptr(shift), ptr(w2), ptr(bias), ptr(logits), B, Cin, H, W,
             b.out_channels)
    return logits if head.scale_factor is None else bilinear_up2_hip(logits)


def pack_head_weight_bf16s(w, nterms=6):
    Cin = w.shape[1]
    assert w.shape[0] == 1 and tuple(w.shape[2:]) == (3, 3, 3) and Cin % 16 == 0
    return _pack("ss_pack_conv3d_head_weights_f16s" if nterms == 19 else "ss_pack_conv3d_head_weights_bf16s", w, Cin)


HEAD_F16 = os.environ.get("SS_HEAD_F16", "0") != "0"


def _head_nterms():
    return 19 if (CONV_ENGINE == "f16x3" and HEAD_F16) else _aux_nterms()


def conv3d_head_bf16s_hip(x, wsplit, scale, shift, relu, nterms):
    x = _c(x)
    dev = _lib.require_device(x, scale, shift)
    B, Cin, D, H, W = x.shape
    out = torch.empty((B, 1, D, H, W), dtype=x.dtype, device=x.device)
    with torch.cuda.device(dev):
        call("ss_conv3d_head_bf16s_fwd", ptr(x), ptr(wsplit), ptr(scale), ptr(shift), ptr(out), B, Cin, D, H, W,
             int(relu), int(nterms))
    return out


def pack_pointwise_weight_bf16s(w):
    Cout, Cin = w.shape[0], w.shape[1]
    assert Cin % 16 == 0
    return _pack("ss_pack_pointwise_weights_bf16s", w.reshape(Cout, Cin), Cout, Cin)


def conv3d_pointwise_bf16s_hip(x, wsplit, Cout, scale, shift, relu, nterms):
    x = _c(x)
    dev = _lib.require_device(x, scale, shift)
    B, Cin = x.shape[0], x.shape[1]
    out = torch.empty((B, Cout) + tuple(x.shape[2:]), dtype=x.dtype, device=x.device)
    with torch.cuda.device(dev):
        call("ss_conv3d_pointwise_bf16s_fwd", ptr(x), ptr(wsplit), ptr(scale), ptr(shift), ptr(out), B, Cin, Cout,
             x[0, 0].numel(), int(relu), int(nterms))
    return out


def _conv_geometry(conv):
    k, s, p = conv.kernel_size, conv.stride, conv.padding
    assert k[0] == k[1] == k[2] and s[0] == s[1] == s[2] and p[0] == p[1] == p[2] == k[0] // 2
    assert conv.bias is None and conv.groups == 1 and conv.dilation == (1, 1, 1)
    return k[0], s[0]


def run_convbn(owner, key, conv, bn, x, relu, residual=None, gate=None):
    k, s = _conv_geometry(conv)
    if CONV_ENGINE != "f32" and k == 3 and s in (1, 2) and conv.out_channels > 1:
        nterms = _tiled_nterms()
        ws, scale, shift = _packed_affine(owner, key + ("/f16s" if nterms == 19 else "/bf16s"), conv, bn,
                                          lambda w: pack_conv_weight_bf16s(w, nterms))
        return conv3d_bf16s_hip(x, ws, conv.out_channels, scale, shift, relu, nterms, residual, gate, stride=s)
    if (CONV_ENGINE != "f32" and k == 3 and s == 1 and conv.out_channels == 1 and conv.in_channels in (16, 32, 64)
            and residual is None and gate is None):
        nterms = _head_nterms()
        ws, scale, shift = _packed_affine(owner, key + "/head_%d" % nterms, conv, bn, lambda w: pack_head_weight_bf16s(w, nterms))
        return conv3d_head_bf16s_hip(x, ws, scale, shift, relu, nterms)
    wp, scale, shift = _packed_affine(owner, key, conv, bn, pack_conv_weight)
    return conv3d_hip(x, wp, scale, shift, k, s, relu, residual, gate)


TRAIN_HIP = os.environ.get("SS_TRAIN_HIP", "1") != "0"
SSR_TRAIN_HIP = os.environ.get("SS_SSR_TRAIN_HIP", "1") != "0"
HEADS_TRAIN_HIP = os.environ.get("SS_HEADS_TRAIN_HIP", "0") != "0"
DECODER_TRAIN_HIP = os.environ.get("SS_DECODER_TRAIN_HIP", "0") != "0"
CONV2D_WGRAD_HIP = os.environ.get("SS_CONV2D_WGRAD_HIP", "0") != "0"
def _fuse_training_on():
    return os.environ.get("SS_FUSE_TRAINING", "1") != "0"


LOSS_HIP = os.environ.get("SS_LOSS_HIP", "1") != "0"
METRICS_HIP = os.environ.get("SS_METRICS_HIP", "1") != "0"
VIS_HIP = os.environ.get("SS_VIS_HIP", "1") != "0"
DATA_HIP = os.environ.get("SS_DATA_HIP", "1") != "0"
CLASSIFIER_CL = os.environ.get("SS_CLASSIFIER_CL", "1") != "0"
CLASSIFIER_FUSED = os.environ.get("SS_CLASSIFIER_FUSED", "1") != "0"


STEM_LEFT_FUSED = os.environ.get("SS_STEM_LEFT_FUSED", "1") != "0"
STEM_LEFT_MFMA = os.environ.get("SS_STEM_LEFT_MFMA", "1") != "0"


def stem_left_takes_mfma(C, Cout, nd):
    return CONV_ENGINE == "f16x3" and STEM_LEFT_FUSED and STEM_LEFT_MFMA and C == 32 and Cout == 32 and nd in (6, 24, 32)


def _stem_halves_params(stem, C):
    conv, bn = stem.conv, stem.bn if stem.use_bn else None
    Cout = conv.out_channels
    assert conv.in_channels == 2 * C and _conv_geometry(conv) == (3, 1)
    srcs = [conv.weight] + ([bn.weight, bn.bias, bn.running_mean, bn.running_var] if bn is not None else [])

    def build():
        sc, sh = fold_bn(bn) if bn is not None else (None, None)
        w = conv.weight.detach().float()
        wl = w[:, :C].reshape(Cout, C, 27)
        wq = wl.permute(2, 0, 1).reshape(27 * Cout, C)
        wf = torch.zeros(Cout // 2, 64, C, dtype=w.dtype, device=w.device)
        wf[:, :54] = wl.reshape(Cout // 2, 2, C, 27).permute(0, 3, 1, 2).reshape(Cout // 2, 54, C)
        wm = ops.pack_stem_left_weights_f16s(wl) if CONV_ENGINE == "f16x3" and C == 32 and Cout == 32 else None
        return (pack_pointwise_weight_bf16s(wq), pack_pointwise_weight_bf16s(wf.reshape(Cout // 2 * 64, C)),
                pack_conv_weight_bf16s(w[:, C:].contiguous(), _tiled_nterms()), sc, sh, wm)
    return _cache(stem).get("bc/halves/" + CONV_ENGINE, srcs, build)


def stem_broadcast_half(stem, left, att):
    assert stem.is_3d and not stem.deconv and CONV_ENGINE != "f32" and _inference(stem, left, att)
    C, Cout = left.shape[1], stem.conv.out_channels
    nterms = _aux_nterms()
    wq, wf, _, _, _, wm = _stem_halves_params(stem, C)
    PATH_COUNTS["hip"] += 1
    if stem_left_takes_mfma(C, Cout, att.shape[-3]):
        return ops.stem_left_mfma(left, wm, att, Cout)
    if C == 32 and Cout % 2 == 0 and STEM_LEFT_FUSED:
        return ops.stem_left_fused(left, wf, att, Cout, nterms)
    q = conv3d_pointwise_bf16s_hip(left, wq, 27 * Cout, None, None, False, nterms)
    return ops.stem_left(q, att)


def stem_volume_half(stem, right_vol, partial, gate=None):
    assert stem.is_3d and not stem.deconv and CONV_ENGINE != "f32" and _inference(stem, right_vol, partial, gate)
    nterms = _tiled_nterms()
    _, _, wr, scale, shift, _ = _stem_halves_params(stem, right_vol.shape[1])
    g = None if gate is None else gate.contiguous()
    return conv3d_bf16s_hip(right_vol, wr, stem.conv.out_channels, scale, shift, bool(stem.relu), nterms, None, g, partial=partial)


STEM_PRESPLIT = os.environ.get("SS_STEM_PRESPLIT", "0") != "0"


def stem_presplit_applies(stem, right):
    return (STEM_PRESPLIT and CONV_ENGINE == "f16x3" and right.shape[1] % 8 == 0 and stem.conv.in_channels == 2 * right.shape[1]
            and _conv_geometry(stem.conv) == (3, 1))


def stem_volume_half_presplit(stem, xs, xexp, partial, gate=None):
    assert stem.is_3d and not stem.deconv and CONV_ENGINE == "f16x3" and _inference(stem, partial, gate)
    B, nchunks, _, D, H, W, _ = xs.shape
    _, _, wr, scale, shift, _ = _stem_halves_params(stem, nchunks * 8)
    Cout = stem.conv.out_channels
    g = None if gate is None else gate.contiguous()
    dev = _lib.require_device(partial, scale, shift, g)
    out = torch.empty((B, Cout, D, H, W), dtype=torch.float32, device=xs.device)
    if partial is not None:
        assert partial.shape == out.shape and partial.is_contiguous()
    with torch.cuda.device(dev if dev is not None else xs.device):
        call("ss_conv3d_presplit_fwd", ptr(xs), ptr(xexp), ptr(wr), ptr(partial), ptr(scale), ptr(shift), ptr(g), ptr(out),
             B, nchunks * 8, D, H, W, Cout, int(bool(stem.relu)))
    return out


STEM_GATHER = os.environ.get("SS_STEM_GATHER", "1") != "0"
STEM_INPLACE = os.environ.get("SS_STEM_INPLACE", "1") != "0"


def stem_gather_applies(stem, right, samples):
    return (STEM_GATHER and CONV_ENGINE == "f16x3" and right.shape[1] % 8 == 0 and right.shape[1] >= 16
            and stem.conv.in_channels == 2 * right.shape[1] and _conv_geometry(stem.conv) == (3, 1)
            and right.dtype == torch.float32 and samples.dtype == torch.float32
            and right.shape[-1] > 1 and right.shape[-2] > 1)


def stem_gather_half(stem, right, samples, att, partial, gate=None, consume_partial=False):
    assert stem.is_3d and not stem.deconv and CONV_ENGINE == "f16x3" and _inference(stem, right, partial, gate)
    right, samples = right.contiguous(), samples.contiguous()
    att = att.reshape(att.shape[0], att.shape[-3], att.shape[-2], att.shape[-1]).contiguous()
    B, C, H, W = right.shape
    nd = samples.shape[1]
    assert samples.shape == (B, nd, H, W) and att.shape == samples.shape
    _, _, wr, scale, shift, _ = _stem_halves_params(stem, C)
    Cout = stem.conv.out_channels
    g = None if gate is None else gate.contiguous()
    dev = _lib.require_device(right, samples, att, partial, scale, shift, g)
    inplace = consume_partial and STEM_INPLACE and partial is not None and partial.is_contiguous() and tuple(partial.shape) == (B, Cout, nd, H, W) and not partial.requires_grad
    out = partial if inplace else torch.empty((B, Cout, nd, H, W), dtype=torch.float32, device=right.device)
    if partial is not None:
        assert partial.shape == out.shape and partial.is_contiguous()
    if g is not None:
        assert g.shape == (B, Cout, H, W)
    PATH_COUNTS["hip"] += 1
    with torch.cuda.device(dev):
        call("ss_conv3d_gather_fwd", ptr(right), ptr(samples), ptr(att), ptr(wr), ptr(partial), ptr(scale), ptr(shift), ptr(g),
             ptr(out), B, C, nd, H, W, Cout, int(bool(stem.relu)), _tiled_nterms())
    return out


def stem_of_broadcast_and_volume(stem, left, att, right_vol, gate=None):
    return stem_volume_half(stem, right_vol, stem_broadcast_half(stem, left, att), gate)

ATTENTION_FORM = os.environ.get("SS_ATTENTION", "split")

SWITCHES = ("CONV_ENGINE", "DECONV_F16", "DECONV_MIN_WORKGROUPS", "DECONV_BF16S", "CLASSIFIER_CL", "CLASSIFIER_FUSED", "CLASSIFIER_FOLD", "TRAIN_HIP", "SSR_TRAIN_HIP", "HEADS_TRAIN_HIP", "DECODER_TRAIN_HIP", "CONV2D_WGRAD_HIP", "LOSS_HIP", "METRICS_HIP", "VIS_HIP", "DATA_HIP", "ATTENTION_FORM",
            "STEM_LEFT_FUSED", "STEM_LEFT_MFMA", "STEM_PRESPLIT", "STEM_GATHER", "STEM_INPLACE", "HEAD_F16", "CONV2D_HIP", "DECODER_HIP", "HEADS_HIP")
```

### semstereo_amd/modules.py

```python
import torch
import torch.nn as nn
import torch.nn.functional as F

from . import _lib, ops
from . import deferred as dfr
from . import engine as E
from . import train as T
from . import train_decoder as TD
from . import train_heads as TH
from . import train_ssr as TS
from ._host import _c
from ._lib import call, ptr
from .engine import (PATH_COUNTS, _cache, _conv_geometry, _inference, _is_plain_3x3, _ParamCache, _ReplicaCache,
                     classifier_cl_hip, classifier_fused_applies, classifier_fused_hip, pack_classifier_head_weight, conv2d_bf16s_hip, conv3d_bf16s_hip, conv3d_head_bf16s_hip, conv3d_hip,
                     conv3d_pointwise_bf16s_hip, deconv3d_bf16s_hip, deconv3d_hip, fold_bn, pack_conv2d_weight_bf16s,
                     pack_conv_weight, pack_conv_weight_bf16s, pack_deconv_weight_bf16s, pack_head_weight_bf16s,
                     pack_pointwise_weight_bf16s, run_conv2d, run_conv2d_pair, run_convbn, stem_broadcast_half, stem_of_broadcast_and_volume,
                     stem_gather_applies, stem_gather_half, stem_presplit_applies, stem_volume_half, stem_volume_half_presplit, _aux_nterms, _deconv_nterms,
                     _head_nterms, _tiled_nterms)
from .train_layers import (_conv_k3_forward, _deconv_k3_forward, conv3d_train, conv3d_wgrad_hip, deconv3d_train)


class _ConvBN3d(nn.Sequential):

    def forward(self, x):
        x = dfr.real(x)
        if _inference(self, x):
            PATH_COUNTS["hip"] += 1
            return run_convbn(self, "cb", self[0], self[1], x, relu=False)
        return self.train_forward(x)

    def train_forward(self, x, relu=False):
        return T.batchnorm_train(self[1], conv3d_train(self[0], x), relu=relu)


def convbn_3d(in_planes, out_planes, kernel_size, stride, pad):
    return _ConvBN3d(nn.Conv3d(in_planes, out_planes, kernel_size=kernel_size, padding=pad, stride=stride, bias=False),
                     nn.BatchNorm3d(out_planes))


class BasicConv(nn.Module):

    def __init__(self, in_channels, out_channels, deconv=False, is_3d=False, bn=True, relu=True, **kwargs):
        super().__init__()
        self.relu = relu
        self.use_bn = bn
        self.is_3d = is_3d
        self.deconv = deconv
        if is_3d:
            layer = nn.ConvTranspose3d if deconv else nn.Conv3d
            self.conv = layer(in_channels, out_channels, bias=False, **kwargs)
            self.bn = nn.BatchNorm3d(out_channels)
        else:
            layer = nn.ConvTranspose2d if deconv else nn.Conv2d
            self.conv = layer(in_channels, out_channels, bias=False, **kwargs)
            self.bn = nn.BatchNorm2d(out_channels)

    @classmethod
    def adopt(cls, ref):
        self = cls.__new__(cls)
        nn.Module.__init__(self)
        self.relu, self.use_bn = ref.relu, ref.use_bn
        self.conv, self.bn = ref.conv, ref.bn
        self.is_3d = isinstance(ref.conv, (nn.Conv3d, nn.ConvTranspose3d))
        self.deconv = isinstance(ref.conv, (nn.ConvTranspose2d, nn.ConvTranspose3d))
        self.train(ref.training)
        return self

    def forward(self, x, gate_logits=None, gate=None):
        if isinstance(x, dfr.Deferred):
            if self.is_3d and not self.deconv and not x.done and gate_logits is None and gate is None and dfr.on(self):
                return dfr.Deferred.call("stem", lambda mod, v: mod(v), self, x)
            x = x.value()
        if self.is_3d and not self.deconv and _inference(self, x, gate_logits, gate):
            PATH_COUNTS["hip"] += 1
            g = gate if gate is not None else (None if gate_logits is None else torch.sigmoid(gate_logits).contiguous())
            return run_convbn(self, "bc", self.conv, self.bn if self.use_bn else None, x, relu=bool(self.relu), gate=g)
        if gate is not None:
            assert gate_logits is None
        if not self.is_3d and not self.deconv and gate_logits is None and gate is None and _inference(self, x):
            y = run_conv2d(self, "bc2d", self.conv, self.bn if self.use_bn else None, x, bool(self.relu))
            if y is not None:
                return y
        if self.deconv:
            PATH_COUNTS["torch"] += 1
            x = self.conv(x)
        elif self.is_3d or T.is_k1(self.conv):
            x = conv3d_train(self.conv, x)
        else:
            x = T.conv2d_k3(self.conv, x)
        if self.use_bn:
            x = T.batchnorm_train(self.bn, x, relu=bool(self.relu))
        elif self.relu:
            x = F.relu(x)
        if gate_logits is not None:
            x = T.channel_gate(gate_logits, x)
        if gate is not None:
            x = gate.unsqueeze(2) * x
        return x


class ConcatFeature(nn.Sequential):

    def __init__(self, channels):
        super().__init__(BasicConv(channels, channels // 2, kernel_size=3, stride=1, padding=1),
                         nn.Conv2d(channels // 2, channels // 4, 3, 1, 1, bias=False))

    @classmethod
    def adopt(cls, ref):
        assert len(ref) == 2 and isinstance(ref[1], nn.Conv2d)
        self = cls.__new__(cls)
        first = ref[0] if isinstance(ref[0], BasicConv) else BasicConv.adopt(ref[0])
        nn.Sequential.__init__(self, first, ref[1])
        self.train(ref.training)
        return self

    def forward(self, x):
        x = dfr.real(x)
        if dfr.on(self, x) and isinstance(x, torch.Tensor) and x.dim() == 4:
            node = dfr.Deferred.call("cfeat", self._forward_now, x)
            node.info["module"] = self
            pend = [r for r in self.__dict__.get("_ss_pending_cf", []) if r() is not None and not r().done]
            pend.append(__import__("weakref").ref(node))
            self.__dict__["_ss_pending_cf"] = pend
            return node
        return self._forward_now(x)

    def _forward_now(self, x):
        x = dfr.real(x)
        a, b = self[0], self[1]
        if (isinstance(getattr(a, "conv", None), nn.Conv2d) and getattr(a, "relu", False) and not getattr(a, "deconv", False)
                and _inference(self, x)):
            y = run_conv2d(a, "bc2d", a.conv, a.bn if getattr(a, "use_bn", True) else None, x, True)
            if y is not None:
                z = run_conv2d(self, "cf1", b, None, y, False)
                return z if z is not None else b(y)
        if _inference(self, x):
            return super().forward(x)
        return T.conv2d_k3(b, a(x))



class attention_block(nn.Module):

    def __init__(self, channels_3d, num_heads=8, block=4):
        super().__init__()
        self.block = block
        self.dim_3d = channels_3d
        self.num_heads = num_heads
        self.scale_3d = (channels_3d // num_heads) ** -0.5
        self.qkv_3d = nn.Linear(channels_3d, channels_3d * 3, bias=True)
        self.final1x1 = nn.Conv3d(channels_3d, channels_3d, 1)

    @classmethod
    def adopt(cls, ref):
        self = cls.__new__(cls)
        nn.Module.__init__(self)
        self.block, self.dim_3d, self.num_heads, self.scale_3d = ref.block, ref.dim_3d, ref.num_heads, ref.scale_3d
        self.qkv_3d, self.final1x1 = ref.qkv_3d, ref.final1x1
        self.train(ref.training)
        return self

    def _params(self):
        srcs = [self.qkv_3d.weight, self.qkv_3d.bias, self.final1x1.weight, self.final1x1.bias]

        def build():
            C = self.dim_3d
            return (self.qkv_3d.weight.detach().float().t().contiguous(),
                    self.qkv_3d.bias.detach().float().contiguous(),
                    self.final1x1.weight.detach().float().reshape(C, C).t().contiguous(),
                    self.final1x1.bias.detach().float().contiguous())
        return _cache(self).get("attn", srcs, build)

    def _params_split(self):
        srcs = [self.qkv_3d.weight, self.qkv_3d.bias, self.final1x1.weight, self.final1x1.bias]

        bf = E.CONV_ENGINE != "f32" and self.dim_3d in (32, 64, 128)

        def build():
            C = self.dim_3d
            pack = pack_pointwise_weight_bf16s if bf else pack_conv_weight
            return (pack(self.qkv_3d.weight.detach().float().reshape(3 * C, C, 1, 1, 1)),
                    self.qkv_3d.bias.detach().float().contiguous(),
                    pack(self.final1x1.weight.detach().float()),
                    self.final1x1.bias.detach().float().contiguous())
        return _cache(self).get("attn_split/" + ("bf16s" if bf else "f32"), srcs, build) + (bf,)

    def hip_supported(self):
        bd, bh, bw = self.block
        return self.dim_3d == 128 and self.num_heads == 16 and bd * bh * bw in (64, 96)

    def forward(self, x):
        x = dfr.real(x)
        if _inference(self, x) and self.hip_supported():
            PATH_COUNTS["hip"] += 1
            x = _c(x)
            dev = _lib.require_device(x)
            B, C, D, H, W = x.shape
            assert C == self.dim_3d and D % self.block[0] == 0
            if E.ATTENTION_FORM == "split":
                wq, bq, wo, bo, bf = self._params_split()
                nterms = _aux_nterms()
                if bf:
                    qkv = conv3d_pointwise_bf16s_hip(x, wq, 3 * C, None, bq, False, nterms)
                else:
                    qkv = conv3d_hip(x, wq, None, bq, 1, 1, False)
                y = torch.empty_like(x)
                with torch.cuda.device(dev):
                    call("ss_window_attention_core_fwd", ptr(qkv), ptr(bq), ptr(y), B, C, D, H, W, self.num_heads,
                         self.block[0], self.block[1], self.block[2])
                if bf:
                    return conv3d_pointwise_bf16s_hip(y, wo, C, None, bo, False, nterms)
                return conv3d_hip(y, wo, None, bo, 1, 1, False)
            wq, bq, wo, bo = self._params()
            out = torch.empty_like(x)
            with torch.cuda.device(dev):
                call("ss_window_attention_fwd", ptr(x), ptr(wq), ptr(bq), ptr(wo), ptr(bo), ptr(out),
                     B, C, D, H, W, self.num_heads, self.block[0], self.block[1], self.block[2])
            return out
        if not _inference(self, x) and self.hip_supported() and T.window_attention_applies(x, self.num_heads, self.block):
            return T.window_attention(x, self.qkv_3d, self.final1x1, self.num_heads, self.block)
        PATH_COUNTS["torch"] += 1
        return self._forward_torch(x)

    def _forward_torch(self, x):
        B, C, D, H0, W0 = x.shape
        bd, bh, bw = self.block
        pad_r, pad_b = (bw - W0 % bw) % bw, (bh - H0 % bh) % bh
        x = F.pad(x, (0, pad_r, 0, pad_b))
        H, W = H0 + pad_b, W0 + pad_r
        nd, nh, nw = D // bd, H // bh, W // bw
        T, hd = bd * bh * bw, C // self.num_heads
        tok = x.reshape(B, C, nd, bd, nh, bh, nw, bw).permute(0, 2, 4, 6, 3, 5, 7, 1).reshape(B, nd * nh * nw, T, C)
        qkv = self.qkv_3d(tok).reshape(B, nd * nh * nw, T, 3, self.num_heads, hd).permute(3, 0, 1, 4, 2, 5)
        logits = (qkv[0] @ qkv[1].transpose(-2, -1)) * self.scale_3d
        if pad_r > 0 and pad_b > 0:
            hh = torch.arange(H, device=x.device).reshape(H, 1) >= H0
            wwf = torch.arange(W, device=x.device).reshape(1, W) >= W0
            flag = (hh | wwf).reshape(nh, bh, nw, bw).permute(0, 2, 1, 3).reshape(nh * nw, bh * bw)
            differs = (flag.unsqueeze(1) != flag.unsqueeze(2)).to(x.dtype) * -1000.0
            logits = logits + differs.repeat(nd, bd, bd).reshape(1, nd * nh * nw, 1, T, T)
        y = torch.softmax(logits, dim=-1) @ qkv[2]
        y = y.reshape(B, nd, nh, nw, self.num_heads, bd, bh, bw, hd).permute(0, 4, 8, 1, 5, 2, 6, 3, 7)
        y = y.reshape(B, C, D, H, W)[:, :, :, :H0, :W0]
        return self.final1x1(y)


class hourglass(nn.Module):
    BLOCK = (4, 4, 4)

    def __init__(self, in_channels):
        super().__init__()
        c = in_channels
        self.conv1 = nn.Sequential(convbn_3d(c, c * 2, 3, 2, 1), nn.ReLU(inplace=True))
        self.conv2 = nn.Sequential(convbn_3d(c * 2, c * 2, 3, 1, 1), nn.ReLU(inplace=True))
        self.conv3 = nn.Sequential(convbn_3d(c * 2, c * 4, 3, 2, 1), nn.ReLU(inplace=True))
        self.conv4 = nn.Sequential(convbn_3d(c * 4, c * 4, 3, 1, 1), nn.ReLU(inplace=True))
        self.attention_block = attention_block(channels_3d=c * 4, num_heads=16, block=self.BLOCK)
        self.conv5 = nn.Sequential(
            nn.ConvTranspose3d(c * 4, c * 2, 3, padding=1, output_padding=1, stride=2, bias=False), nn.BatchNorm3d(c * 2))
        self.conv6 = nn.Sequential(
            nn.ConvTranspose3d(c * 2, c, 3, padding=1, output_padding=1, stride=2, bias=False), nn.BatchNorm3d(c))
        self.redir1 = convbn_3d(c, c, kernel_size=1, stride=1, pad=0)
        self.redir2 = convbn_3d(c * 2, c * 2, kernel_size=1, stride=1, pad=0)

    @classmethod
    def adopt(cls, ref):
        self = cls.__new__(cls)
        nn.Module.__init__(self)
        for name, child in ref.named_children():
            setattr(self, name, attention_block.adopt(child) if name == "attention_block" else child)
        self.BLOCK = tuple(self.attention_block.block)
        self.train(ref.training)
        return self

    def _up_params(self, key, deconv_seq, redir_seq):
        dc, dbn, rc, rbn = deconv_seq[0], deconv_seq[1], redir_seq[0], redir_seq[1]
        srcs = [dc.weight, dbn.weight, dbn.bias, dbn.running_mean, dbn.running_var,
                rc.weight, rbn.weight, rbn.bias, rbn.running_mean, rbn.running_var]

        def build():
            ds, db = fold_bn(dbn)
            rs, rb = fold_bn(rbn)
            wd = pack_conv_weight(dc.weight, transposed=True) * ds.reshape(1, 1, -1)
            wr = pack_conv_weight(rc.weight).reshape(rc.weight.shape[1], rc.weight.shape[0]) * rs.reshape(1, -1)
            wd, wr = wd.contiguous(), wr.contiguous()
            return (wd, wr, (db + rb).contiguous(), pack_deconv_weight_bf16s(wd, _deconv_nterms()) if E.CONV_ENGINE != "f32" else None,
                    pack_deconv_weight_bf16s(wr) if E.CONV_ENGINE != "f32" else None)
        return _cache(self).get(key + "/" + E.CONV_ENGINE, srcs, build)

    def _up(self, key, deconv_seq, redir_seq, x, skip):
        wd, wr, shift, wds, wrs = self._up_params(key, deconv_seq, redir_seq)
        B, _, D, H, W = x.shape
        workgroups = B * D * ((H + 3) // 4) * ((W + 31) // 32) * ((wd.shape[2] + 31) // 32)
        if E.CONV_ENGINE != "f32" and E.DECONV_BF16S and workgroups >= E.DECONV_MIN_WORKGROUPS:
            return deconv3d_bf16s_hip(x, wds, wd.shape[2], shift, True, _deconv_nterms(), skip, wrs)
        return deconv3d_hip(x, wd, shift, relu=True, skip=skip, skip_wpack=wr)

    def forward(self, x):
        x = dfr.real(x)
        if not _inference(self, x):
            def cbr(seq, t):
                cb = seq[0]
                return cb.train_forward(t, relu=True) if isinstance(cb, _ConvBN3d) else seq(t)
            conv1 = cbr(self.conv1, x)
            conv2 = cbr(self.conv2, conv1)
            conv3 = cbr(self.conv3, conv2)
            conv4 = self.attention_block(cbr(self.conv4, conv3))
            def up(seq, t, skip):
                return T.batchnorm_train(seq[1], deconv3d_train(seq[0], t), relu=True, residual=skip)
            conv5 = up(self.conv5, conv4, self.redir2(conv2))
            return up(self.conv6, conv5, self.redir1(x))
        PATH_COUNTS["hip"] += 1
        c1 = run_convbn(self, "c1", self.conv1[0][0], self.conv1[0][1], x, relu=True)
        hook = self.__dict__.get("_mid_hook")

        def at(point):
            if hook is not None:
                hook[1](point)
        c2 = run_convbn(self, "c2", self.conv2[0][0], self.conv2[0][1], c1, relu=True)
        at("c2")
        c3 = run_convbn(self, "c3", self.conv3[0][0], self.conv3[0][1], c2, relu=True)
        at("c3")
        c4 = run_convbn(self, "c4", self.conv4[0][0], self.conv4[0][1], c3, relu=True)
        at("c4")
        c4 = self.attention_block(c4)
        at("att")
        c5 = self._up("u5", self.conv5, self.redir2, c4, c2)
        at("u5")
        return self._up("u6", self.conv6, self.redir1, c5, x)


class hourglass2(hourglass):
    BLOCK = (6, 4, 4)


class Classifier(nn.Sequential):

    def __init__(self, channels=32):
        super().__init__(convbn_3d(channels, channels, 3, 1, 1), nn.ReLU(inplace=True),
                         nn.Conv3d(channels, 1, kernel_size=3, padding=1, stride=1, bias=False))

    @classmethod
    def adopt(cls, ref):
        self = cls.__new__(cls)
        nn.Sequential.__init__(self, ref[0], ref[1], ref[2])
        self.train(ref.training)
        return self

    def patches(self, x):
        x = dfr.real(x)
        c0, bn0, c2 = self[0][0], self[0][1], self[2]
        if not (_inference(self, x) and E.CLASSIFIER_FOLD and E.CLASSIFIER_FUSED and E.CLASSIFIER_CL and E.CONV_ENGINE != "f32"
                and c0.in_channels == c0.out_channels == c2.in_channels == 32 and _conv_geometry(c0) == (3, 1)
                and _conv_geometry(c2) == (3, 1) and c2.out_channels == 1 and classifier_fused_applies(x, _tiled_nterms())):
            return None
        nt0 = _tiled_nterms()

        def build_fused():
            sc, sh = fold_bn(bn0)
            return pack_conv_weight_bf16s(c0.weight, nt0), sc, sh, pack_classifier_head_weight(c2.weight)
        srcs = [c0.weight, bn0.weight, bn0.bias, bn0.running_mean, bn0.running_var, c2.weight]
        ws0, sc, sh, hw = _cache(self).get("fused/%d" % nt0, srcs, build_fused)
        PATH_COUNTS["hip"] += 1
        return classifier_fused_hip(x, ws0, sc, sh, nt0, hw, sum_patches=False)

    def forward(self, x):
        x = dfr.real(x)
        if dfr.on(self, x):
            with dfr.suspended():
                return dfr.Deferred.leaf(self.forward(x), role="cost")
        if _inference(self, x):
            PATH_COUNTS["hip"] += 1
            c0, bn0, c2 = self[0][0], self[0][1], self[2]
            if (E.CLASSIFIER_CL and E.CONV_ENGINE != "f32" and c0.in_channels == c0.out_channels == c2.in_channels == 32
                    and _conv_geometry(c0) == (3, 1) and _conv_geometry(c2) == (3, 1) and c2.out_channels == 1):
                nt0, nt2 = _tiled_nterms(), _head_nterms()
                if E.CLASSIFIER_FUSED and classifier_fused_applies(x, nt0):

                    def build_fused():
                        sc, sh = fold_bn(bn0)
                        return pack_conv_weight_bf16s(c0.weight, nt0), sc, sh, pack_classifier_head_weight(c2.weight)
                    srcs = [c0.weight, bn0.weight, bn0.bias, bn0.running_mean, bn0.running_var, c2.weight]
                    ws0, sc, sh, hw = _cache(self).get("fused/%d" % nt0, srcs, build_fused)
                    return classifier_fused_hip(x, ws0, sc, sh, nt0, hw)

                def build():
                    sc, sh = fold_bn(bn0)
                    return pack_conv_weight_bf16s(c0.weight, nt0), sc, sh, pack_head_weight_bf16s(c2.weight, nt2)
                srcs = [c0.weight, bn0.weight, bn0.bias, bn0.running_mean, bn0.running_var, c2.weight]
                ws0, sc, sh, ws2 = _cache(self).get("cl/%d/%d" % (nt0, nt2), srcs, build)
                return classifier_cl_hip(x, ws0, sc, sh, nt0, ws2, nt2)
            y = run_convbn(self, "h0", c0, bn0, x, relu=True)
            return run_convbn(self, "h2", c2, None, y, relu=False)
        cb = self[0]
        if isinstance(cb, _ConvBN3d) and cb[1].training:
            return conv3d_train(self[2], cb.train_forward(x, relu=True))
        return conv3d_train(self[2], F.relu(cb(x)))


_PROP_TAPS = ((-1, -1), (0, 0), (1, 1), (1, -1), (-1, 1))


def propagation(x):
    H, W = x.shape[-2:]
    p = F.pad(x, (1, 1, 1, 1), mode="replicate")
    return torch.cat([p[..., 1 + dy:1 + dy + H, 1 + dx:1 + dx + W] for dy, dx in _PROP_TAPS], dim=1)


def propagation_prob(v):
    H, W = v.shape[-2:]
    p = F.pad(v, (1, 1, 1, 1, 0, 0), mode="replicate")
    return torch.cat([p[..., 1 + dy:1 + dy + H, 1 + dx:1 + dx + W] for dy, dx in _PROP_TAPS], dim=1)


class Propagation(nn.Module):

    @classmethod
    def adopt(cls, ref):
        return cls().train(ref.training)

    def forward(self, disparity_samples):
        if dfr.on(None, disparity_samples):
            return dfr.Deferred.call("propagation", propagation, disparity_samples)
        return propagation(dfr.real(disparity_samples))


class Propagation_prob(nn.Module):

    @classmethod
    def adopt(cls, ref):
        return cls().train(ref.training)

    def forward(self, prob_volume):
        if dfr.on(None, prob_volume):
            return dfr.Deferred.call("propagation_prob", propagation_prob, prob_volume)
        return propagation_prob(dfr.real(prob_volume))


class DepthwisePatch(nn.Conv3d):

    def __init__(self, channels):
        super().__init__(channels, channels, kernel_size=(1, 3, 3), stride=1, dilation=1, groups=channels,
                         padding=(0, 1, 1), bias=False)

    @classmethod
    def adopt(cls, ref):
        assert ref.kernel_size == (1, 3, 3) and ref.groups == ref.in_channels and ref.bias is None
        self = cls.__new__(cls)
        self.__dict__.update(ref.__dict__)
        return self

    def forward(self, x, gate_logits=None):
        if isinstance(x, dfr.Deferred):
            if x.op == "gwc_norm" and not x.done and gate_logits is None and dfr.on(self):
                return dfr.Deferred.call("patch", lambda mod, v: mod(v), self, x)
            x = x.value()
        if _inference(self, x, gate_logits):
            PATH_COUNTS["hip"] += 1
            x = _c(x)
            dev = _lib.require_device(x, gate_logits)
            B, C, D, H, W = x.shape
            w = self.weight.detach()
            out = torch.empty_like(x)
            g = None if gate_logits is None else gate_logits.contiguous()
            with torch.cuda.device(dev):
                call("ss_depthwise_patch_fwd", ptr(x), ptr(w), ptr(g), ptr(out), B, C, D, H, W)
            return out
        y = T.depthwise_patch(self, x)
        return y if gate_logits is None else T.channel_gate(gate_logits, y)


class channelAtt(nn.Module):

    def __init__(self, cv_chan, im_chan):
        super().__init__()
        self.im_att = nn.Sequential(BasicConv(im_chan, im_chan // 2, kernel_size=1, stride=1, padding=0),
                                    nn.Conv2d(im_chan // 2, cv_chan, 1))

    @classmethod
    def adopt(cls, ref):
        self = cls.__new__(cls)
        nn.Module.__init__(self)
        self.im_att = ref.im_att
        self.train(ref.training)
        return self

    def _hip_params(self):
        a, b = self.im_att[0], self.im_att[1]
        c1 = getattr(a, "conv", None)
        ok = (len(self.im_att) == 2 and isinstance(c1, nn.Conv2d) and isinstance(b, nn.Conv2d) and getattr(a, "relu", False)
              and c1.kernel_size == (1, 1) and b.kernel_size == (1, 1) and c1.bias is None and c1.stride == (1, 1)
              and b.stride == (1, 1) and c1.groups == 1 and b.groups == 1 and c1.padding == (0, 0) and b.padding == (0, 0)
              and (c1.in_channels, c1.out_channels, b.out_channels) in ((256, 128, 32), (128, 64, 32))
              and b.in_channels == c1.out_channels)
        if not ok:
            return None
        bn = a.bn if getattr(a, "use_bn", True) else None
        srcs = [c1.weight, b.weight] + ([b.bias] if b.bias is not None else []) + \
               ([bn.weight, bn.bias, bn.running_mean, bn.running_var] if bn is not None else [])

        def build():
            sc, sh = fold_bn(bn) if bn is not None else (None, None)
            return (pack_pointwise_weight_bf16s(c1.weight), sc, sh, pack_pointwise_weight_bf16s(b.weight),
                    None if b.bias is None else b.bias.detach().float().contiguous())
        return _cache(self).get("im_att", srcs, build)

    def logits(self, im, sigmoid=False):
        if _inference(self, im) and im.is_cuda:
            prm = self._hip_params()
            if prm is not None and im.shape[1] * im.shape[2] * im.shape[3] * 4 < 2 ** 31:
                PATH_COUNTS["hip"] += 1
                w1, sc, sh, w2, b2 = prm
                im = _c(im)
                dev = _lib.require_device(im)
                B, Cin, H, W = im.shape
                c1, c2 = self.im_att[0].conv, self.im_att[1]
                out = torch.empty((B, c2.out_channels, H, W), dtype=im.dtype, device=im.device)
                with torch.cuda.device(dev):
                    call("ss_channel_att_logits_fwd", ptr(im), ptr(w1), ptr(sc), ptr(sh), ptr(w2), ptr(b2), ptr(out),
                         B, Cin, c1.out_channels, c2.out_channels, H, W, int(bool(sigmoid)))
                return out
        att = self.im_att(im)
        return torch.sigmoid(att) if sigmoid else att

    def forward(self, cv, im):
        im = dfr.real(im)
        if isinstance(cv, dfr.Deferred):
            if dfr.on(self, im):
                fused = dfr.gated_volume_of(cv, self, im)
                if fused is None:
                    fused = dfr.stem_of(cv, self, im)
                if fused is not None:
                    return fused
            cv = cv.value()
        if _inference(self, cv, im):
            PATH_COUNTS["hip"] += 1
            return ops.channel_gate(self.logits(im), cv)
        a, b = self.im_att[0], self.im_att[1]
        att = conv3d_train(b, a(im)) if isinstance(b, nn.Conv2d) and T.is_k1(b) else self.im_att(im)
        return T.channel_gate(att, cv)


class SSR_upsample(nn.Module):

    def __init__(self, num_classes):
        super().__init__()
        n = self.num_classes = num_classes
        self.conv = nn.Sequential(nn.BatchNorm2d(1), nn.Conv2d(1, n, kernel_size=3, padding=1), nn.BatchNorm2d(n))
        self.conv1 = nn.Sequential(nn.Conv2d(n, n, kernel_size=1, padding=0), nn.BatchNorm2d(n))
        self.conv2 = nn.Sequential(nn.Conv2d(n, n, kernel_size=1, padding=0), nn.BatchNorm2d(n))
        self.conv3 = nn.Conv2d(n, 1, kernel_size=1, padding=0)

    @classmethod
    def adopt(cls, ref):
        self = cls.__new__(cls)
        nn.Module.__init__(self)
        self.num_classes = ref.num_classes
        for name, child in ref.named_children():
            setattr(self, name, child)
        self.train(ref.training)
        return self

    def _params(self):
        srcs = [t for t in list(self.parameters()) + list(self.buffers()) if t.dtype.is_floating_point]

        def build():
            n = self.num_classes
            f64 = lambda t: t.detach().double()

            def fold64(bn_):
                sc = f64(bn_.weight) / torch.sqrt(f64(bn_.running_var) + bn_.eps)
                return sc, f64(bn_.bias) - f64(bn_.running_mean) * sc
            s0, t0 = fold64(self.conv[0])
            sa, ta = fold64(self.conv[2])
            s1, t1 = fold64(self.conv1[1])
            s2, t2 = fold64(self.conv2[1])
            nl2e = -1.4426950408889634
            parts = [s0, t0, sa[:, None] * f64(self.conv[1].weight).reshape(n, 9), sa * f64(self.conv[1].bias) + ta,
                     nl2e * s1[:, None] * f64(self.conv1[0].weight).reshape(n, n), nl2e * (s1 * f64(self.conv1[0].bias) + t1),
                     nl2e * s2[:, None] * f64(self.conv2[0].weight).reshape(n, n), nl2e * (s2 * f64(self.conv2[0].bias) + t2),
                     f64(self.conv3.weight).reshape(n), f64(self.conv3.bias)]
            return torch.cat([p.reshape(-1) for p in parts]).float().contiguous()
        return _cache(self).get("ssr", srcs, build)

    def forward(self, depth_low, weights, pred_label):
        if dfr._is(pred_label, "seghead"):
            pred_label = pred_label.value()
        if (self.num_classes == 6 and isinstance(weights, torch.Tensor) and isinstance(pred_label, torch.Tensor)
                and dfr.on(self, *[t for t in (depth_low, weights, pred_label) if isinstance(t, torch.Tensor)])):
            dfr.STATS.setdefault("ssr", {"deferred": 0, "computed": 0})["deferred"] += 1
            return dfr.Deferred.call("ssr", self._forward_counted, depth_low, weights, pred_label)
        return self._forward_now(depth_low, weights, pred_label)

    def _forward_counted(self, depth_low, weights, pred_label):
        dfr.STATS.setdefault("ssr", {"deferred": 0, "computed": 0})["computed"] += 1
        return self._forward_now(depth_low, weights, pred_label)

    def _forward_now(self, depth_low, weights, pred_label):
        depth_low, weights, pred_label = dfr.real(depth_low), dfr.real(weights), dfr.real(pred_label)
        if _inference(self, depth_low, weights, pred_label) and self.num_classes == 6:
            PATH_COUNTS["hip"] += 1
            depth_low, weights, pred_label = [_c(t) for t in (depth_low, weights, pred_label)]
            dev = _lib.require_device(depth_low, weights, pred_label)
            b, c, h, w = depth_low.shape
            assert c == 1 and weights.shape == (b, self.num_classes, 4 * h, 4 * w) and pred_label.shape == weights.shape
            prm = self._params()
            assert prm.numel() == _lib.load().ss_ssr_param_count()
            out = torch.empty((b, 4 * h, 4 * w), dtype=depth_low.dtype, device=depth_low.device)
            with torch.cuda.device(dev):
                call("ss_ssr_upsample_fwd", ptr(depth_low), ptr(weights), ptr(pred_label), ptr(prm), ptr(out),
                     b, h, w, self.num_classes)
            return out
        if not _inference(self, depth_low, weights, pred_label) and E.TRAIN_HIP and E.SSR_TRAIN_HIP and TS.supported(
                self, depth_low, weights, pred_label):
            PATH_COUNTS["hip_train"] = PATH_COUNTS.get("hip_train", 0) + 1
            PATH_COUNTS["ssr_train"] = PATH_COUNTS.get("ssr_train", 0) + 1
            return TS.ssr_train(self, depth_low, weights, pred_label)
        PATH_COUNTS["torch"] += 1
        b, c, h, w = depth_low.shape
        depth_ = F.interpolate(depth_low, (h * 4, w * 4), mode="bilinear").reshape(b, 1, h * 4, w * 4)
        depth = self.conv(depth_)
        prob = self._class_gate(weights, pred_label)
        return (depth_ + self.conv3(depth * prob)).squeeze(1)

    def _class_gate(self, weights, pred_label):
        key = (id(weights), id(pred_label), weights._version, pred_label._version, torch.is_grad_enabled(), self.training,
               tuple(p_._version for p_ in self.parameters()))
        hit = _GATE_PARKED.pop(self, None)
        if hit is not None and hit[0] == key and hit[1] is weights and hit[2] is pred_label:
            PATH_COUNTS["ssr_gate_reused"] = PATH_COUNTS.get("ssr_gate_reused", 0) + 1
            with torch.no_grad():
                for bn_, (m0, v0) in zip((self.conv1[1], self.conv2[1]), hit[4]):
                    if m0 is not None:
                        mom = bn_.momentum
                        bn_.running_mean.data.copy_((1 - mom) * bn_.running_mean + (bn_.running_mean - (1 - mom) * m0))
                        bn_.running_var.data.copy_((1 - mom) * bn_.running_var + (bn_.running_var - (1 - mom) * v0))
                        bn_.num_batches_tracked += 1
            return hit[3]
        bns = (self.conv1[1], self.conv2[1])
        tracked = [b_.training and b_.track_running_stats for b_ in bns]
        if any(tracked) and any(b_.momentum is None for b_ in bns):
            tracked = None
        before = None if tracked is None else [(b_.running_mean.clone(), b_.running_var.clone()) if t_ else (None, None)
                                               for b_, t_ in zip(bns, tracked)]
        prob = torch.sigmoid(self.conv1(F.softmax(pred_label, dim=1) * weights))
        prob = torch.sigmoid(self.conv2(prob * weights))
        if before is not None and torch.is_grad_enabled():
            _GATE_PARKED[self] = (key, weights, pred_label, prob, before)
        return prob


_GATE_PARKED = __import__("weakref").WeakKeyDictionary()


def drop_parked_gates(model=None):
    if model is None:
        _GATE_PARKED.clear()
        return
    for m_ in model.modules():
        if isinstance(m_, SSR_upsample):
            _GATE_PARKED.pop(m_, None)



def _stock_basicconv(bc, x):
    PATH_COUNTS["torch"] += 1
    x = bc.conv(x)
    if bc.use_bn:
        x = bc.bn(x)
    if bc.relu:
        x = F.relu(x)
    return x


class Conv2x(nn.Module):

    def __init__(self, in_channels, out_channels, deconv=False, is_3d=False, concat=True, keep_concat=True, bn=True, relu=True, keep_dispc=False):
        super().__init__()
        self.concat = concat
        self.is_3d = is_3d
        if deconv and is_3d:
            kernel = (4, 4, 4)
        elif deconv:
            kernel = 4
        else:
            kernel = 3
        if deconv and is_3d and keep_dispc:
            self.conv1 = BasicConv(in_channels, out_channels, deconv, is_3d, bn=True, relu=True, kernel_size=(1, 4, 4), stride=(1, 2, 2), padding=(0, 1, 1))
        else:
            self.conv1 = BasicConv(in_channels, out_channels, deconv, is_3d, bn=True, relu=True, kernel_size=kernel, stride=2, padding=1)
        if self.concat:
            mul = 2 if keep_concat else 1
            self.conv2 = BasicConv(out_channels * 2, out_channels * mul, False, is_3d, bn, relu, kernel_size=3, stride=1, padding=1)
        else:
            self.conv2 = BasicConv(out_channels, out_channels, False, is_3d, bn, relu, kernel_size=3, stride=1, padding=1)

    @classmethod
    def adopt(cls, ref):
        self = cls.__new__(cls)
        nn.Module.__init__(self)
        self.concat, self.is_3d = ref.concat, ref.is_3d
        self.conv1, self.conv2 = ref.conv1, ref.conv2
        self.train(ref.training)
        return self

    def _hip_applies(self, *xs):
        a, b = self.conv1, self.conv2
        return (self.concat and not self.is_3d and E._decoder_hip_on() and E.CONV_ENGINE == "f16x3"
                and E._is_deconv_k4s2(a.conv) and a.conv.bias is None and a.use_bn and a.relu and _is_plain_3x3(b.conv)
                and all(isinstance(t, torch.Tensor) and t.is_cuda and t.dtype == torch.float32 and t.dim() == 4 for t in xs)
                and _inference(self, *xs))

    def _conv2_after_hip_deconv(self, y, rem, xb=None, remb=None):
        b = self.conv2
        bn2 = b.bn if b.use_bn else None
        z = E.run_conv2d_cat(b, "bc2d", b.conv, bn2, y, rem, bool(b.relu), xb=xb, remb=remb)
        if z is not None:
            return (z,) if xb is None else (z[:y.shape[0]], z[y.shape[0]:])
        outs = []
        for u, r in ((y, rem),) + (((xb, remb),) if xb is not None else ()):
            c = torch.cat((u, r), 1)
            v = run_conv2d(b, "bc2d", b.conv, bn2, c, bool(b.relu))
            outs.append(v if v is not None else _stock_basicconv(b, c))
        return tuple(outs)

    def forward(self, x, rem):
        x, rem = dfr.real(x), dfr.real(rem)
        a, b = self.conv1, self.conv2
        if (self._hip_applies(x, rem)
                and tuple(rem.shape) == (x.shape[0], a.conv.out_channels, 2 * x.shape[2], 2 * x.shape[3])):
            y = E.run_deconv2d(a, "c2x", a.conv, a.bn, x, True)
            if y is not None:
                PATH_COUNTS["hip"] += 1
                return self._conv2_after_hip_deconv(y, rem)[0]
        if (not _inference(self, x, rem) and isinstance(x, torch.Tensor) and isinstance(rem, torch.Tensor)
                and TD.conv2x_train_applies(self, x, rem)):
            return TD.conv2x_train(self, x, rem)
        x = _stock_basicconv(a, x)
        if x.shape != rem.shape:
            x = F.interpolate(x, size=(rem.shape[-2], rem.shape[-1]), mode='bilinear')
        if self.concat:
            x = torch.cat((x, rem), 1)
        else:
            x = x + rem
        return _stock_basicconv(b, x)

    def forward_pair(self, xa, rema, xb, remb):
        xa, rema, xb, remb = dfr.real(xa), dfr.real(rema), dfr.real(xb), dfr.real(remb)
        a = self.conv1
        if (self._hip_applies(xa, rema, xb, remb) and xa.shape == xb.shape and rema.shape == remb.shape
                and tuple(rema.shape) == (xa.shape[0], a.conv.out_channels, 2 * xa.shape[2], 2 * xa.shape[3])):
            B = xa.shape[0]
            y = E.run_deconv2d(a, "c2x", a.conv, a.bn, xa, True, xb=xb)
            if y is not None:
                PATH_COUNTS["hip"] += 1
                return self._conv2_after_hip_deconv(y[:B], rema, xb=y[B:], remb=remb)
        return self.forward(xa, rema), self.forward(xb, remb)


class FeatUp(nn.Module):

    def __init__(self):
        super().__init__()
        chans = [64, 128, 256, 384, 512]
        self.deconv32_16 = Conv2x(chans[4], chans[3], deconv=True, concat=True)
        self.deconv16_8 = Conv2x(chans[3] * 2, chans[2], deconv=True, concat=True)
        self.deconv8_4 = Conv2x(chans[2] * 2, chans[1], deconv=True, concat=True)
        self.deconv4_2 = Conv2x(chans[1] * 2, chans[0], deconv=True, concat=True)

    @classmethod
    def adopt(cls, ref):
        self = cls.__new__(cls)
        nn.Module.__init__(self)
        for name in ("deconv32_16", "deconv16_8", "deconv8_4", "deconv4_2"):
            sub = getattr(ref, name)
            setattr(self, name, sub if isinstance(sub, Conv2x) else Conv2x.adopt(sub))
        self.train(ref.training)
        return self

    def forward(self, featL, featR=None):
        x2, x4, x8, x16, x32 = featL
        y2, y4, y8, y16, y32 = featR
        if E.DECODER_TRAIN_HIP and not _inference(self, *(dfr.real(t) for t in (*featL, *featR))):
            x16, y16 = self.deconv32_16(x32, x16), self.deconv32_16(y32, y16)
            x8, y8 = self.deconv16_8(x16, x8), self.deconv16_8(y16, y8)
            x4, y4 = self.deconv8_4(x8, x4), self.deconv8_4(y8, y4)
            x2, y2 = self.deconv4_2(x4, x2), self.deconv4_2(y4, y2)
            return [x2, x4, x8, x16, x32], [y2, y4, y8, y16, y32]
        x16, y16 = self.deconv32_16.forward_pair(x32, x16, y32, y16)
        x8, y8 = self.deconv16_8.forward_pair(x16, x8, y16, y8)
        x4, y4 = self.deconv8_4.forward_pair(x8, x4, y8, y4)
        x2, y2 = self.deconv4_2.forward_pair(x4, x2, y4, y2)
        return [x2, x4, x8, x16, x32], [y2, y4, y8, y16, y32]


class Spx2(nn.Sequential):

    def __init__(self, in_channels=128, out_channels=6):
        super().__init__(nn.ConvTranspose2d(in_channels, out_channels, kernel_size=4, stride=2, padding=1))

    @classmethod
    def adopt(cls, ref):
        assert len(ref) == 1 and isinstance(ref[0], nn.ConvTranspose2d)
        self = cls.__new__(cls)
        nn.Sequential.__init__(self, ref[0])
        self.train(ref.training)
        return self

    def forward(self, x):
        x = dfr.real(x)
        if isinstance(x, torch.Tensor) and x.is_cuda and _inference(self, x):
            y = E.run_deconv2d(self, "spx2", self[0], None, x, False)
            if y is not None:
                PATH_COUNTS["hip"] += 1
                return y
        elif isinstance(x, torch.Tensor) and TD.spx2_train_applies(self, x):
            return TD.spx2_train(self, x)
        PATH_COUNTS["torch"] += 1
        return self[0](x)



class segmenthead(nn.Module):

    def __init__(self, inplanes, interplanes, outplanes, scale_factor=None):
        super().__init__()
        self.conv1 = BasicConv(inplanes, interplanes, kernel_size=3, padding=1)
        self.conv2 = nn.Conv2d(interplanes, outplanes, kernel_size=1, padding=0, bias=True)
        self.scale_factor = scale_factor

    @staticmethod
    def adoptable(ref):
        a, b = getattr(ref, "conv1", None), getattr(ref, "conv2", None)
        return (isinstance(getattr(a, "conv", None), nn.Conv2d) and isinstance(getattr(a, "bn", None), nn.BatchNorm2d)
                and hasattr(a, "use_bn") and hasattr(a, "relu") and isinstance(b, nn.Conv2d) and hasattr(ref, "scale_factor"))

    @classmethod
    def adopt(cls, ref):
        if not cls.adoptable(ref):
            return None
        self = cls.__new__(cls)
        nn.Module.__init__(self)
        self.conv1, self.conv2 = ref.conv1, ref.conv2
        self.scale_factor = ref.scale_factor
        self.train(ref.training)
        return self

    def forward(self, x):
        if isinstance(x, torch.Tensor) and dfr.on(self, x) and E.seghead_applies(self, x):
            return dfr.Deferred.call("seghead", self._forward_now, x)
        return self._forward_now(x)

    def _forward_now(self, x):
        x = dfr.real(x)
        if isinstance(x, torch.Tensor) and x.is_cuda and _inference(self, x):
            y = E.run_seghead(self, self, x)
            if y is not None:
                PATH_COUNTS["hip"] += 1
                return y
        elif TH.seghead_train_applies(self, x):
            return TH.seghead_train(self, x)
        x = _stock_basicconv(self.conv1, x)
        out = self.conv2(x)
        if self.scale_factor is not None:
            height = x.shape[-2] * self.scale_factor
            width = x.shape[-1] * self.scale_factor
            out = F.interpolate(out, size=[height, width], mode='bilinear', align_corners=False)
        return out


class ChalProjection(nn.Sequential):

    def __init__(self, in_channels, out_channels):
        super().__init__(nn.Conv2d(in_channels, out_channels, kernel_size=1, stride=1), nn.BatchNorm2d(out_channels))

    @staticmethod
    def adoptable(ref):
        return (isinstance(ref, nn.Sequential) and len(ref) == 2 and isinstance(ref[0], nn.Conv2d) and isinstance(ref[1], nn.BatchNorm2d))

    @classmethod
    def adopt(cls, ref):
        if not cls.adoptable(ref):
            return None
        self = cls.__new__(cls)
        nn.Sequential.__init__(self, ref[0], ref[1])
        self.train(ref.training)
        return self

    def _hip(self, x, xb=None):
        ts = [x] + ([xb] if xb is not None else [])
        if all(isinstance(t, torch.Tensor) and t.is_cuda for t in ts) and _inference(self, *ts):
            return E.run_conv2d_k1(self, "chal", self[0], self[1], x, False, xb=xb)
        return None

    def forward(self, x):
        x = dfr.real(x)
        if isinstance(x, torch.Tensor) and x.is_cuda and _inference(self, x):
            y = E.run_conv2d_k1(self, "chal", self[0], self[1], x, False)
            if y is not None:
                PATH_COUNTS["hip"] += 1
                return y
        elif TH.proj_train_applies(self, x):
            return TH.proj_train(self, x)
        PATH_COUNTS["torch"] += 1
        return self[1](self[0](x))

    def forward_pair(self, xl, xr):
        xl, xr = dfr.real(xl), dfr.real(xr)
        if isinstance(xl, torch.Tensor) and isinstance(xr, torch.Tensor) and xl.shape == xr.shape and xl.dtype == xr.dtype:
            y = self._hip(xl, xr)
            if y is not None:
                PATH_COUNTS["hip"] += 1
                return y[:xl.shape[0]], y[xl.shape[0]:]
        return self.forward(xl), self.forward(xr)


def __getattr__(name):
    if name in E.SWITCHES:
        return getattr(E, name)
    raise AttributeError(f"module {__name__!r} has no attribute {name!r}")


class _TwinsModule(__import__("types").ModuleType):

    def __setattr__(self, name, value):
        if name in E.SWITCHES:
            raise AttributeError(f"set semstereo_amd.engine.{name}, not semstereo_amd.modules.{name} (the switches live in engine.py)")
        super().__setattr__(name, value)


__import__("sys").modules[__name__].__class__ = _TwinsModule
```

Before: 635.5 pairs/s.

## Fuse QKV projection into window attention and fold output projection into deconv

Adds a window_attention_proj kernel that computes the QKV pointwise projection in-kernel and then attends, so the qkv tensor is never written to or read back from global memory. The attention block's final 1x1 projection is folded algebraically into the following transposed-conv weights. Its bias becomes a 27-entry boundary-dependent shift table that the deconv epilogue reads from LDS. This removes two pointwise conv launches and their intermediate traffic, at the cost of a more complex deconv epilogue and a different rounding order for the folded weights.

Measured after the change: 645.4 pairs/s (median of 6 runs). +1.6%, better.

```diff
diff --git a/include/semstereo_hip.h b/include/semstereo_hip.h
--- a/include/semstereo_hip.h
+++ b/include/semstereo_hip.h
@@ -206,6 +206,9 @@
 int ss_deconv3d_bf16s_fwd(const float* in, const void* wsplit, const float* shift, const float* skip,
                           const void* skip_wsplit, float* out, int B, int Cin, int D, int H, int W, int Cout,
                           int Cs, int relu, int nterms, ss_stream_t stream);
+int ss_deconv3d_bf16s_shift27_fwd(const float* in, const void* wsplit, const float* shift27, const float* skip,
+                                  const void* skip_wsplit, float* out, int B, int Cin, int D, int H, int W, int Cout,
+                                  int Cs, int relu, int nterms, ss_stream_t stream);
 int ss_pack_deconv3d_weights_bf16s(const float* wpack, void* wsplit, int Cin, int Cout, int ntaps, ss_stream_t stream);
 int ss_pack_deconv3d_weights_bf16s_bytes(int Cin, int Cout, int ntaps, long long* bytes);
 int ss_pack_deconv3d_weights_f16s(const float* wpack, void* wsplit, int Cin, int Cout, ss_stream_t stream);
@@ -225,6 +228,9 @@
                             ss_stream_t stream);
 int ss_window_attention_core_fwd(const float* qkv, const float* bqkv, float* y, int B, int C, int D, int H,
                                  int W, int heads, int bd, int bh, int bw, ss_stream_t stream);
+int ss_window_attention_proj_fwd(const float* x, const void* wqkv_split, const float* bqkv, float* y, int B, int C,
+                                 int D, int H, int W, int heads, int bd, int bh, int bw, int nterms,
+                                 ss_stream_t stream);
 
 int ss_batchnorm_train_fwd(const float* x, const float* weight, const float* bias, float* y, float* mean, float* invstd,
                            float* var_unbiased, double* work, int B, int C, long long N, float eps, int relu,
diff --git a/semstereo_amd/csrc/deconv3d_bf16s.hip b/semstereo_amd/csrc/deconv3d_bf16s.hip
--- a/semstereo_amd/csrc/deconv3d_bf16s.hip
+++ b/semstereo_amd/csrc/deconv3d_bf16s.hip
@@ -70,7 +70,7 @@
     static_assert(TD * TH == 4, "4 waves x one input row each");
 };
 
-template <int TD, int TH, int NTERMS, bool HAS_SKIP, bool SPLIT = false, bool ACCB = false, bool STREAM = false>
+template <int TD, int TH, int NTERMS, bool HAS_SKIP, bool SPLIT = false, bool ACCB = false, bool STREAM = false, bool SHIFT27 = false>
 __global__ __launch_bounds__(256, (SPLIT && !ACCB) ? 3 : 2) void deconv3d_bf16s(const float* __restrict__ in, const uint4* __restrict__ wsplit,
                                                           const float* __restrict__ shift, const float* __restrict__ skip,
                                                           const uint4* __restrict__ skip_wsplit, float* __restrict__ out,
@@ -148,7 +148,7 @@
     float* aff = reinterpret_cast<float*>(&lds[MSLOT + 1]);
     if (tid < 32) {
         const int co = min(co0 + tid, Cout - 1);
-        aff[tid] = shift ? shift[co] : 0.0f;
+        aff[tid] = (shift && !SHIFT27) ? shift[co] : 0.0f;
         aff[32 + tid] = F16 ? wunscale[co] : 1.0f;
     }
     constexpr int SNT = F16 ? 6 : NTERMS, SNC = (SNT == 6) ? 3 : 2;
@@ -418,7 +418,25 @@
         }
     }
 
+    constexpr int NT27 = SHIFT27 ? (27 * 32 + 255) / 256 : 1;
+    float t27[NT27];
+    if constexpr (SHIFT27) {
+#pragma unroll
+        for (int i = 0; i < NT27; ++i) {
+            const int e = min(tid + 256 * i, 27 * 32 - 1);
+            t27[i] = shift[(e >> 5) * Cout + min(co0 + (e & 31), Cout - 1)];
+        }
+    }
+
     if (HAS_SKIP && !skip_first) skip_phase();
+
+    if constexpr (SHIFT27) {
+        static_assert(27 * 32 <= MSLOT * 4, "the table fits in the input tile");
+#pragma unroll
+        for (int i = 0; i < NT27; ++i)
+            if (tid + 256 * i < 27 * 32) reinterpret_cast<float*>(lds)[tid + 256 * i] = t27[i];
+        __syncthreads();
+    }
 
     const int jw = iw0 + l31, jd = id0 + dzw, jh = ih0 + hyw;
     const unsigned ochan_b = (unsigned)((size_t)Do * out_plane * 4);
@@ -431,6 +449,15 @@
         vo[j] = ok ? (unsigned)((((size_t)(2 * jd + (GP::q(j) >> 1)) * Ho + 2 * jh + (GP::q(j) & 1)) * Wo + 2 * jw) * 4) + 4u * half * ochan_b
                    : 0x80000000u;
     const float floor_v = relu ? 0.f : -__builtin_inff();
+    int trow[SHIFT27 ? GP::NQ2 : 1][2];
+    if constexpr (SHIFT27) {
+        const int cd = 9 * (1 + (jd == D - 1)), ch = 3 * (1 + (jh == H - 1)), cw = 1 + (jw == W - 1);
+#pragma unroll
+        for (int j = 0; j < GP::NQ2; ++j)
+#pragma unroll
+            for (int pw = 0; pw < 2; ++pw)
+                trow[j][pw] = (((GP::q(j) >> 1) ? cd : 0) + ((GP::q(j) & 1) ? ch : 0) + (pw ? cw : 0)) * 32 + 4 * half;
+    }
 #pragma unroll
     for (int r = 0; r < 16; ++r) {
         const int cb = co0 + (r & 3) + 8 * (r >> 2);
@@ -438,8 +465,14 @@
         const float sh = aff[(r & 3) + 8 * (r >> 2) + 4 * half];
 #pragma unroll
         for (int j = 0; j < GP::NQ2; ++j) {
-            const float v0 = fmaxf(ss::add_rn(acc[j * 2 + 0][r], sh), floor_v);
-            const float v1 = fmaxf(ss::add_rn(acc[j * 2 + 1][r], sh), floor_v);
+            float sh0 = sh, sh1 = sh;
+            if constexpr (SHIFT27) {
+                const float* tab = reinterpret_cast<const float*>(lds) + (r & 3) + 8 * (r >> 2);
+                sh0 = tab[trow[j][0]];
+                sh1 = tab[trow[j][1]];
+            }
+            const float v0 = fmaxf(ss::add_rn(acc[j * 2 + 0][r], sh0), floor_v);
+            const float v1 = fmaxf(ss::add_rn(acc[j * 2 + 1][r], sh1), floor_v);
 #ifdef SS_EXP_DECONV_NOSTORE
             if (r == 0 && j == 0)
 #endif
@@ -509,14 +542,14 @@
     wsplit[i] = split_weight_f16(x, term);
 }
 
-template <int TD, int TH, int NTERMS, bool HAS_SKIP, bool SPLIT = false, bool ACCB = false, bool STREAM = false>
+template <int TD, int TH, int NTERMS, bool HAS_SKIP, bool SPLIT = false, bool ACCB = false, bool STREAM = false, bool SHIFT27 = false>
 int launch_db(const float* in, const void* wsplit, const float* shift, const float* skip, const void* skip_wsplit, float* out,
               int B, int Cin, int D, int H, int W, int Cout, int Cs, int relu, hipStream_t st) {
     using C = DB<TD, TH, (NTERMS == 6) ? 3 : 2, NTERMS == F16X3, SPLIT ? 15 : 27>;
     const int tiles_w = ss::ceil_div(W, 32), tiles_h = ss::ceil_div(H, TH), tiles_d = ss::ceil_div(D, TD);
     const long long nt = (long long)tiles_w * tiles_h * tiles_d;
     if (nt > 0x7fffffffLL || B > 65535) return SS_ERR_UNSUPPORTED;
-    auto kern = deconv3d_bf16s<TD, TH, NTERMS, HAS_SKIP, SPLIT, ACCB, STREAM>;
+    auto kern = deconv3d_bf16s<TD, TH, NTERMS, HAS_SKIP, SPLIT, ACCB, STREAM, SHIFT27>;
     if (C::LDS_BYTES > 64 * 1024) {
         if (ss::ensure_dynamic_lds(reinterpret_cast<const void*>(kern), (int)C::LDS_BYTES) != SS_OK) return SS_ERR_LAUNCH;
     }
@@ -528,12 +561,13 @@
     return ss::check_launch();
 }
 
-template <int TD, int TH>
+template <int TD, int TH, bool SHIFT27 = false>
 int launch_db_all(const float* in, const void* wsplit, const float* shift, const float* skip, const void* skip_wsplit,
                   float* out, int B, int Cin, int D, int H, int W, int Cout, int Cs, int relu, int nterms, hipStream_t st) {
-#define SS_DB(NTERMS, HAS_SKIP) launch_db<TD, TH, NTERMS, HAS_SKIP>(in, wsplit, shift, skip, skip_wsplit, out, B, Cin, D, H, W, Cout, Cs, relu, st)
+#define SS_DB(NTERMS, HAS_SKIP) launch_db<TD, TH, NTERMS, (HAS_SKIP) || SHIFT27, false, false, false, SHIFT27>(in, wsplit, shift, skip, skip_wsplit, out, B, Cin, D, H, W, Cout, Cs, relu, st)
 #define SS_DF(HAS_SKIP, SPLIT, ACCB, STREAM) \
-    launch_db<TD, TH, F16X3, HAS_SKIP, SPLIT, ACCB, STREAM>(in, wsplit, shift, skip, skip_wsplit, out, B, Cin, D, H, W, Cout, Cs, relu, st)
+    launch_db<TD, TH, F16X3, (HAS_SKIP) || SHIFT27, SPLIT, ACCB, STREAM, SHIFT27>(in, wsplit, shift, skip, skip_wsplit, out, B, Cin, D, H, W, Cout, Cs, relu, st)
+    if (SHIFT27 && skip == nullptr) return SS_ERR_UNSUPPORTED;
     if (nterms == F16X3) {
         const long long per_pair = (long long)ss::ceil_div(W, 32) * ss::ceil_div(H, TH) * ss::ceil_div(D, TD) * ss::ceil_div(Cout, 32);
         int groups = ss::tuning().deconv_groups;
@@ -605,3 +639,19 @@
         return launch_db_all<2, 2>(in, wsplit, shift, skip, skip_wsplit, out, B, Cin, D, H, W, Cout, Cs, relu, nterms, st);
     return launch_db_all<1, 4>(in, wsplit, shift, skip, skip_wsplit, out, B, Cin, D, H, W, Cout, Cs, relu, nterms, st);
 }
+
+extern "C" int ss_deconv3d_bf16s_shift27_fwd(const float* in, const void* wsplit, const float* shift27, const float* skip,
+                                             const void* skip_wsplit, float* out, int B, int Cin, int D, int H, int W, int Cout,
+                                             int Cs, int relu, int nterms, ss_stream_t stream) {
+    SS_REQUIRE(in && wsplit && out && shift27 && skip && skip_wsplit && Cs > 0);
+    SS_REQUIRE(B > 0 && Cin > 0 && D > 0 && H > 0 && W > 0 && Cout > 0 && (nterms == 3 || nterms == 6 || nterms == F16X3));
+    SS_REQUIRE((reinterpret_cast<uintptr_t>(wsplit) & 15) == 0 && (reinterpret_cast<uintptr_t>(skip_wsplit) & 15) == 0);
+    if ((reinterpret_cast<uintptr_t>(out) & 7) != 0) return SS_ERR_INVALID;
+    if ((long long)Cin * D * H * W * 4 >= 0x7fffffffLL) return SS_ERR_UNSUPPORTED;
+    if ((long long)Cs * 8 * D * H * W * 4 >= 0x7fffffffLL) return SS_ERR_UNSUPPORTED;
+    if ((long long)Cout * 8 * D * H * W * 4 >= 0x7fffffffLL) return SS_ERR_UNSUPPORTED;
+    hipStream_t st = ss::as_stream(stream);
+    if (D >= 2 && H < 4)
+        return launch_db_all<2, 2, true>(in, wsplit, shift27, skip, skip_wsplit, out, B, Cin, D, H, W, Cout, Cs, relu, nterms, st);
+    return launch_db_all<1, 4, true>(in, wsplit, shift27, skip, skip_wsplit, out, B, Cin, D, H, W, Cout, Cs, relu, nterms, st);
+}
diff --git a/semstereo_amd/csrc/window_attention.hip b/semstereo_amd/csrc/window_attention.hip
--- a/semstereo_amd/csrc/window_attention.hip
+++ b/semstereo_amd/csrc/window_attention.hip
@@ -20,6 +20,38 @@
     static constexpr int WL = C * 96;
     static constexpr size_t LDS_BYTES = (size_t)(XS + QKV + YG + FLAGS + WL) * 4;
 };
+
+template <int T, int C>
+__device__ __forceinline__ void stage_window_tokens(float* __restrict__ xs, const float* __restrict__ xb, int tid, int wd, int wh,
+                                                    int ww, int H, int W, int bd, int bh, int bw, size_t plane, size_t vol) {
+    using A = ACfg<T, C>;
+    if (bw == 4 && (W & 3) == 0 && ((reinterpret_cast<uintptr_t>(xb) & 15) == 0)) {
+        constexpr int NQ = C * (A::TP / 4) / 256;
+        static_assert(C * (A::TP / 4) % 256 == 0, "whole batches");
+#pragma unroll
+        for (int i = 0; i < NQ; ++i) {
+            const int e = tid + 256 * i;
+            const int tq = e % (A::TP / 4), c = e / (A::TP / 4);
+            const int ih = tq % bh, id = tq / bh;
+            const int gh = wh * bh + ih, gd = wd * bd + id, gw = ww * 4;
+            const bool ok = gh < H && gw < W;
+            const float4 q = *reinterpret_cast<const float4*>(xb + (size_t)c * vol + (size_t)gd * plane +
+                                                              (size_t)min(gh, H - 1) * W + min(gw, W - 4));
+            *reinterpret_cast<float4*>(&xs[e * 4]) = ok ? q : make_float4(0.f, 0.f, 0.f, 0.f);
+        }
+    } else {
+        for (int e = tid; e < C * A::TP; e += 256) {
+            const int t = e % A::TP, c = e / A::TP;
+            float v = 0.f;
+            if (t < T) {
+                const int iw = t % bw, ih = (t / bw) % bh, id = t / (bw * bh);
+                const int gw = ww * bw + iw, gh = wh * bh + ih, gd = wd * bd + id;
+                if (gh < H && gw < W) v = xb[(size_t)c * vol + (size_t)gd * plane + (size_t)gh * W + gw];
+            }
+            xs[e] = v;
+        }
+    }
+}
 
 template <int T, int C>
 __global__ __launch_bounds__(256) void window_attention_kernel(
@@ -44,32 +76,7 @@
     const size_t plane = (size_t)H * W, vol = (size_t)D * plane;
     const float* xb = x + (size_t)b * C * vol;
 
-    if (bw == 4 && (W & 3) == 0 && ((reinterpret_cast<uintptr_t>(x) & 15) == 0)) {
-        constexpr int NQ = C * (A::TP / 4) / 256;
-        static_assert(C * (A::TP / 4) % 256 == 0, "whole batches");
-#pragma unroll
-        for (int i = 0; i < NQ; ++i) {
-            const int e = tid + 256 * i;
-            const int tq = e % (A::TP / 4), c = e / (A::TP / 4);
-            const int ih = tq % bh, id = tq / bh;
-            const int gh = wh * bh + ih, gd = wd * bd + id, gw = ww * 4;
-            const bool ok = gh < H && gw < W;
-            const float4 q = *reinterpret_cast<const float4*>(xb + (size_t)c * vol + (size_t)gd * plane +
-                                                              (size_t)min(gh, H - 1) * W + min(gw, W - 4));
-            *reinterpret_cast<float4*>(&xs[e * 4]) = ok ? q : make_float4(0.f, 0.f, 0.f, 0.f);
-        }
-    } else {
-        for (int e = tid; e < C * A::TP; e += 256) {
-            const int t = e % A::TP, c = e / A::TP;
-            float v = 0.f;
-            if (t < T) {
-                const int iw = t % bw, ih = (t / bw) % bh, id = t / (bw * bh);
-                const int gw = ww * bw + iw, gh = wh * bh + ih, gd = wd * bd + id;
-                if (gh < H && gw < W) v = xb[(size_t)c * vol + (size_t)gd * plane + (size_t)gh * W + gw];
-            }
-            xs[e] = v;
-        }
-    }
+    stage_window_tokens<T, C>(xs, xb, tid, wd, wh, ww, H, W, bd, bh, bw, plane, vol);
     for (int t = tid; t < A::TP; t += 256) {
         float f = 0.f;
         if (t < T) {
@@ -210,6 +217,11 @@
         }
     }
 }
+
+template <int T, int C>
+__device__ __forceinline__ void attend_head_group(float* __restrict__ qkv, const float* __restrict__ flag, const unsigned (&vmax_w)[4],
+                                                  float* __restrict__ y, int b, int g, int wd, int wh, int ww, int D, int H, int W,
+                                                  int bd, int bh, int bw, int use_mask);
 
 template <int T, int C>
 __global__ __launch_bounds__(256) void window_attention_core(const float* __restrict__ qkv_in, const float* __restrict__ bqkv,
@@ -220,7 +232,6 @@
     __shared__ __attribute__((aligned(16))) float qkv[3 * 32 * A::TP];
     __shared__ float flag[A::TP];
     const int tid = threadIdx.x, lane = tid & 63, wave = tid >> 6;
-    const int l31 = lane & 31, half = lane >> 5;
     constexpr int NGROUPS = C / (HG * HD);
     int wi = blockIdx.x;
     const int g = wi % NGROUPS; wi /= NGROUPS;
@@ -271,7 +282,17 @@
         flag[t] = ((wh * bh + ih >= H) || (ww * bw + iw >= W)) ? 1.f : 0.f;
     }
     __syncthreads();
-
+    attend_head_group<T, C>(qkv, flag, vmax_w, y, b, g, wd, wh, ww, D, H, W, bd, bh, bw, use_mask);
+}
+
+template <int T, int C>
+__device__ __forceinline__ void attend_head_group(float* __restrict__ qkv, const float* __restrict__ flag, const unsigned (&vmax_w)[4],
+                                                  float* __restrict__ y, int b, int g, int wd, int wh, int ww, int D, int H, int W,
+                                                  int bd, int bh, int bw, int use_mask) {
+    using A = ACfg<T, C>;
+    const int tid = threadIdx.x, lane = tid & 63, wave = tid >> 6;
+    const int l31 = lane & 31, half = lane >> 5;
+    const size_t plane = (size_t)H * W, vol = (size_t)D * plane;
     const float scale = 0.35355339059327379f;
     const int e_v = workgroup_exponent(vmax_w);
     const float v_scale = scale_for(e_v);
@@ -363,6 +384,120 @@
             for (int r = 0; r < 4; ++r) yb[(size_t)(g * 32 + hh * HD + 4 * half + r) * vol + pos] = ot[r];
         }
     }
+}
+
+template <int T, int C, int NTERMS, int KH>
+__global__ __launch_bounds__(256, KH == 2 ? 4 : 3) void window_attention_proj(const float* __restrict__ x, const uint4* __restrict__ wsplit,
+                                                              const float* __restrict__ bqkv, float* __restrict__ y, int D, int H,
+                                                              int W, int bd, int bh, int bw, int nwh, int nww, int use_mask) {
+    using A = ACfg<T, C>;
+    static_assert(A::TP == T && C % (32 * KH) == 0 && (KH == 1 || KH == 2), "whole 32-token tiles, whole K-steps per stage");
+    constexpr int NC = (NTERMS == 6) ? 3 : 2;
+    constexpr int KS = C / 16;
+    constexpr int CH = C / KH;
+    __shared__ __attribute__((aligned(16))) float buf[(CH > 96 ? CH : 96) * A::TP];
+    __shared__ float flag[A::TP];
+    __shared__ unsigned vmax_w[4];
+    const int tid = threadIdx.x, lane = tid & 63, wave = tid >> 6;
+    const int l31 = lane & 31, half = lane >> 5;
+    constexpr int NGROUPS = C / (HG * HD);
+    int wi = blockIdx.x;
+    const int g = wi % NGROUPS; wi /= NGROUPS;
+    const int ww = wi % nww; wi /= nww;
+    const int wh = wi % nwh; wi /= nwh;
+    const int wd = wi;
+    const int b = blockIdx.y;
+    const size_t plane = (size_t)H * W, vol = (size_t)D * plane;
+
+    for (int t = tid; t < A::TP; t += 256) {
+        const int iw = t % bw, ih = (t / bw) % bh;
+        flag[t] = ((wh * bh + ih >= H) || (ww * bw + iw >= W)) ? 1.f : 0.f;
+    }
+    constexpr int NU = (3 * A::NTL + 3) / 4;
+    f32x16 acc[NU];
+#pragma unroll
+    for (int i = 0; i < NU; ++i)
+#pragma unroll
+        for (int r = 0; r < 16; ++r) acc[i][r] = 0.f;
+#pragma unroll
+    for (int kh = 0; kh < KH; ++kh) {
+        if (kh > 0) __syncthreads();
+        stage_window_tokens<T, CH>(buf, x + ((size_t)b * C + kh * CH) * vol, tid, wd, wh, ww, H, W, bd, bh, bw, plane, vol);
+        __syncthreads();
+#pragma unroll
+        for (int i = 0; i < NU; ++i) {
+            const int u = wave + 4 * i;
+            if (u >= 3 * A::NTL) continue;
+            const int mt = u / A::NTL, nt = u % A::NTL;
+            const uint4* ap = wsplit + (size_t)(mt * (C / 32) + g) * KS * 3 * 64 + half * 32 + l31;
+            const float* bp = buf + 8 * half * A::TP + nt * 32 + l31;
+#pragma unroll
+            for (int k = 0; k < KS / KH; ++k) {
+                const int ks = kh * (KS / KH) + k;
+                bf16x8 a[NC];
+#pragma unroll
+                for (int c = 0; c < NC; ++c) a[c] = __builtin_bit_cast(bf16x8, ap[(ks * 3 + c) * 64]);
+                unsigned bh_[4], bm_[4], bl_[4];
+#pragma unroll
+                for (int j = 0; j < 4; ++j)
+                    split3_pk(bp[(k * 16 + 2 * j) * A::TP], bp[(k * 16 + 2 * j + 1) * A::TP], bh_[j], bm_[j], bl_[j]);
+                const bf16x8 h8 = __builtin_bit_cast(bf16x8, make_uint4(bh_[0], bh_[1], bh_[2], bh_[3]));
+                const bf16x8 m8 = __builtin_bit_cast(bf16x8, make_uint4(bm_[0], bm_[1], bm_[2], bm_[3]));
+                if (NTERMS == 6) {
+                    const bf16x8 l8 = __builtin_bit_cast(bf16x8, make_uint4(bl_[0], bl_[1], bl_[2], bl_[3]));
+                    acc[i] = __builtin_amdgcn_mfma_f32_32x32x16_bf16(a[1], m8, acc[i], 0, 0, 0);
+                    acc[i] = __builtin_amdgcn_mfma_f32_32x32x16_bf16(a[0], l8, acc[i], 0, 0, 0);
+                    acc[i] = __builtin_amdgcn_mfma_f32_32x32x16_bf16(a[NC - 1], h8, acc[i], 0, 0, 0);
+                }
+                acc[i] = __builtin_amdgcn_mfma_f32_32x32x16_bf16(a[0], m8, acc[i], 0, 0, 0);
+                acc[i] = __builtin_amdgcn_mfma_f32_32x32x16_bf16(a[1], h8, acc[i], 0, 0, 0);
+                acc[i] = __builtin_amdgcn_mfma_f32_32x32x16_bf16(a[0], h8, acc[i], 0, 0, 0);
+            }
+        }
+    }
+    float bias[NU][16];
+#pragma unroll
+    for (int i = 0; i < NU; ++i) {
+        const int u = wave + 4 * i;
+        if (u >= 3 * A::NTL) continue;
+#pragma unroll
+        for (int r = 0; r < 16; ++r) bias[i][r] = bqkv[(u / A::NTL) * C + g * 32 + (r & 3) + 8 * (r >> 2) + 4 * half];
+    }
+    __syncthreads();
+    float vm = 0.f;
+#pragma unroll
+    for (int i = 0; i < NU; ++i) {
+        const int u = wave + 4 * i;
+        if (u >= 3 * A::NTL) continue;
+        const int mt = u / A::NTL, nt = u % A::NTL;
+#pragma unroll
+        for (int r = 0; r < 16; ++r) {
+            const float v = ss::add_rn(acc[i][r], bias[i][r]);
+            buf[(mt * 32 + (r & 3) + 8 * (r >> 2) + 4 * half) * A::TP + nt * 32 + l31] = v;
+            if (mt == 2) vm = fmaxf(vm, fabsf(v));
+        }
+    }
+    {
+        const unsigned wm = wave_max_bits(__float_as_uint(vm));
+        if (lane == 0) vmax_w[wave] = wm;
+    }
+    __syncthreads();
+    attend_head_group<T, C>(buf, flag, vmax_w, y, b, g, wd, wh, ww, D, H, W, bd, bh, bw, use_mask);
+}
+
+#ifndef SS_ATTN_PROJ_KH96
+#define SS_ATTN_PROJ_KH96 2
+#endif
+template <int T, int NTERMS>
+int launch_attn_proj(const float* x, const void* wsplit, const float* bqkv, float* y, int B, int D, int H, int W, int bd, int bh,
+                     int bw, hipStream_t st) {
+    const int nwd = D / bd, nwh = ss::ceil_div(H, bh), nww = ss::ceil_div(W, bw);
+    const int use_mask = (H % bh != 0) && (W % bw != 0);
+    const long long nblk = (long long)nwd * nwh * nww * (128 / (HG * HD));
+    if (nblk > 0x7fffffffLL || B > 65535) return SS_ERR_UNSUPPORTED;
+    hipLaunchKernelGGL((window_attention_proj<T, 128, NTERMS, T == 96 ? SS_ATTN_PROJ_KH96 : 1>), dim3((unsigned)nblk, B), dim3(256), 0, st, x,
+                       reinterpret_cast<const uint4*>(wsplit), bqkv, y, D, H, W, bd, bh, bw, nwh, nww, use_mask);
+    return ss::check_launch();
 }
 
 template <int T>
@@ -422,3 +557,23 @@
     if (T == 96) return launch_attn_core<96>(qkv, bqkv, y, B, D, H, W, bd, bh, bw, st);
     return SS_ERR_UNSUPPORTED;
 }
+
+extern "C" int ss_window_attention_proj_fwd(const float* x, const void* wqkv_split, const float* bqkv, float* y, int B, int C,
+                                            int D, int H, int W, int heads, int bd, int bh, int bw, int nterms,
+                                            ss_stream_t stream) {
+    SS_REQUIRE(x && wqkv_split && bqkv && y);
+    SS_REQUIRE(B > 0 && C > 0 && D > 0 && H > 0 && W > 0 && heads > 0 && bd > 0 && bh > 0 && bw > 0);
+    SS_REQUIRE(D % bd == 0 && (nterms == 3 || nterms == 6));
+    SS_REQUIRE((reinterpret_cast<uintptr_t>(wqkv_split) & 15) == 0);
+    if (C != 128 || heads != 16) return SS_ERR_UNSUPPORTED;
+    const int T = bd * bh * bw;
+    hipStream_t st = ss::as_stream(stream);
+#define SS_AP(TV)                                                                                                     \
+    if (T == TV)                                                                                                      \
+        return nterms == 6 ? launch_attn_proj<TV, 6>(x, wqkv_split, bqkv, y, B, D, H, W, bd, bh, bw, st)              \
+                           : launch_attn_proj<TV, 3>(x, wqkv_split, bqkv, y, B, D, H, W, bd, bh, bw, st);
+    SS_AP(64)
+    SS_AP(96)
+#undef SS_AP
+    return SS_ERR_UNSUPPORTED;
+}
diff --git a/semstereo_amd/engine.py b/semstereo_amd/engine.py
--- a/semstereo_amd/engine.py
+++ b/semstereo_amd/engine.py
@@ -704,7 +704,32 @@
 def stem_of_broadcast_and_volume(stem, left, att, right_vol, gate=None):
     return stem_volume_half(stem, right_vol, stem_broadcast_half(stem, left, att), gate)
 
-ATTENTION_FORM = os.environ.get("SS_ATTENTION", "split")
-
-SWITCHES = ("CONV_ENGINE", "DECONV_F16", "DECONV_MIN_WORKGROUPS", "DECONV_BF16S", "CLASSIFIER_CL", "CLASSIFIER_FUSED", "CLASSIFIER_FOLD", "TRAIN_HIP", "SSR_TRAIN_HIP", "HEADS_TRAIN_HIP", "DECODER_TRAIN_HIP", "CONV2D_WGRAD_HIP", "LOSS_HIP", "METRICS_HIP", "VIS_HIP", "DATA_HIP", "ATTENTION_FORM",
+ATTENTION_FORM = os.environ.get("SS_ATTENTION", "proj")
+ATTN_FOLD = os.environ.get("SS_ATTN_FOLD", "1") != "0"
+
+
+def fold_pointwise_into_deconv(wo, bo, w5, bn_scale, shift, dtype=torch.float32):
+    C = w5.shape[0]
+    wo64, w564 = wo.detach().double().reshape(C, -1), w5.detach().double()
+    s64 = bn_scale.detach().double().reshape(1, -1, 1, 1, 1)
+    wf = torch.einsum("mi,moxyz->ioxyz", wo64, w564) * s64
+    bw = torch.einsum("m,moxyz->oxyz", bo.detach().double(), w564) * s64[0]
+    valid = torch.tensor([[0., 1., 0.], [1., 0., 1.], [0., 0., 1.]], dtype=torch.float64, device=bw.device)
+    t27 = torch.einsum("ax,by,cz,oxyz->abco", valid, valid, valid, bw).reshape(27, -1) + shift.detach().double().reshape(1, -1)
+    return wf.to(dtype).contiguous(), t27.to(dtype).contiguous()
+
+
+def deconv3d_bf16s_shift27_hip(x, wsplit, Cout, shift27, relu, nterms, skip, skip_wsplit):
+    x, skip = _c(x), _c(skip)
+    dev = _lib.require_device(x, shift27, skip)
+    B, Cin, D, H, W = x.shape
+    Cs = skip.shape[1]
+    assert skip.shape == (B, Cs, 2 * D, 2 * H, 2 * W) and shift27.shape == (27, Cout) and shift27.is_contiguous()
+    out = torch.empty((B, Cout, 2 * D, 2 * H, 2 * W), dtype=x.dtype, device=x.device)
+    with torch.cuda.device(dev):
+        call("ss_deconv3d_bf16s_shift27_fwd", ptr(x), ptr(wsplit), ptr(shift27), ptr(skip), ptr(skip_wsplit), ptr(out),
+             B, Cin, D, H, W, Cout, Cs, int(relu), int(nterms))
+    return out
+
+SWITCHES = ("CONV_ENGINE", "DECONV_F16", "DECONV_MIN_WORKGROUPS", "DECONV_BF16S", "CLASSIFIER_CL", "CLASSIFIER_FUSED", "CLASSIFIER_FOLD", "TRAIN_HIP", "SSR_TRAIN_HIP", "HEADS_TRAIN_HIP", "DECODER_TRAIN_HIP", "CONV2D_WGRAD_HIP", "LOSS_HIP", "METRICS_HIP", "VIS_HIP", "DATA_HIP", "ATTENTION_FORM", "ATTN_FOLD",
             "STEM_LEFT_FUSED", "STEM_LEFT_MFMA", "STEM_PRESPLIT", "STEM_GATHER", "STEM_INPLACE", "HEAD_F16", "CONV2D_HIP", "DECODER_HIP", "HEADS_HIP")
diff --git a/semstereo_amd/modules.py b/semstereo_amd/modules.py
--- a/semstereo_amd/modules.py
+++ b/semstereo_amd/modules.py
@@ -190,25 +190,36 @@
         bd, bh, bw = self.block
         return self.dim_3d == 128 and self.num_heads == 16 and bd * bh * bw in (64, 96)
 
-    def forward(self, x):
+    def folds_final(self, x):
+        return _inference(self, dfr.real(x)) and self.hip_supported() and E.ATTENTION_FORM in ("split", "proj")
+
+    def forward(self, x, final=True):
         x = dfr.real(x)
+        assert final or self.folds_final(x)
         if _inference(self, x) and self.hip_supported():
             PATH_COUNTS["hip"] += 1
             x = _c(x)
             dev = _lib.require_device(x)
             B, C, D, H, W = x.shape
             assert C == self.dim_3d and D % self.block[0] == 0
-            if E.ATTENTION_FORM == "split":
+            if E.ATTENTION_FORM in ("split", "proj"):
                 wq, bq, wo, bo, bf = self._params_split()
                 nterms = _aux_nterms()
-                if bf:
-                    qkv = conv3d_pointwise_bf16s_hip(x, wq, 3 * C, None, bq, False, nterms)
+                y = torch.empty_like(x)
+                if E.ATTENTION_FORM == "proj" and bf:
+                    with torch.cuda.device(dev):
+                        call("ss_window_attention_proj_fwd", ptr(x), ptr(wq), ptr(bq), ptr(y), B, C, D, H, W, self.num_heads,
+                             self.block[0], self.block[1], self.block[2], nterms)
                 else:
-                    qkv = conv3d_hip(x, wq, None, bq, 1, 1, False)
-                y = torch.empty_like(x)
-                with torch.cuda.device(dev):
-                    call("ss_window_attention_core_fwd", ptr(qkv), ptr(bq), ptr(y), B, C, D, H, W, self.num_heads,
-                         self.block[0], self.block[1], self.block[2])
+                    if bf:
+                        qkv = conv3d_pointwise_bf16s_hip(x, wq, 3 * C, None, bq, False, nterms)
+                    else:
+                        qkv = conv3d_hip(x, wq, None, bq, 1, 1, False)
+                    with torch.cuda.device(dev):
+                        call("ss_window_attention_core_fwd", ptr(qkv), ptr(bq), ptr(y), B, C, D, H, W, self.num_heads,
+                             self.block[0], self.block[1], self.block[2])
+                if not final:
+                    return y
                 if bf:
                     return conv3d_pointwise_bf16s_hip(y, wo, C, None, bo, False, nterms)
                 return conv3d_hip(y, wo, None, bo, 1, 1, False)
@@ -289,13 +300,34 @@
                     pack_deconv_weight_bf16s(wr) if E.CONV_ENGINE != "f32" else None)
         return _cache(self).get(key + "/" + E.CONV_ENGINE, srcs, build)
 
+    def _up_takes_split_engine(self, key, deconv_seq, redir_seq, x):
+        wd = self._up_params(key, deconv_seq, redir_seq)[0]
+        B, _, D, H, W = x.shape
+        workgroups = B * D * ((H + 3) // 4) * ((W + 31) // 32) * ((wd.shape[2] + 31) // 32)
+        return E.CONV_ENGINE != "f32" and E.DECONV_BF16S and workgroups >= E.DECONV_MIN_WORKGROUPS
+
     def _up(self, key, deconv_seq, redir_seq, x, skip):
         wd, wr, shift, wds, wrs = self._up_params(key, deconv_seq, redir_seq)
-        B, _, D, H, W = x.shape
-        workgroups = B * D * ((H + 3) // 4) * ((W + 31) // 32) * ((wd.shape[2] + 31) // 32)
-        if E.CONV_ENGINE != "f32" and E.DECONV_BF16S and workgroups >= E.DECONV_MIN_WORKGROUPS:
+        if self._up_takes_split_engine(key, deconv_seq, redir_seq, x):
             return deconv3d_bf16s_hip(x, wds, wd.shape[2], shift, True, _deconv_nterms(), skip, wrs)
         return deconv3d_hip(x, wd, shift, relu=True, skip=skip, skip_wpack=wr)
+
+    def _up5_folded_params(self):
+        dc, dbn, rbn, fin = self.conv5[0], self.conv5[1], self.redir2[1], self.attention_block.final1x1
+        srcs = [dc.weight, dbn.weight, dbn.bias, dbn.running_mean, dbn.running_var,
+                rbn.weight, rbn.bias, rbn.running_mean, rbn.running_var, fin.weight, fin.bias]
+
+        def build():
+            ds, db = fold_bn(dbn)
+            _, rb = fold_bn(rbn)
+            wf, t27 = E.fold_pointwise_into_deconv(fin.weight, fin.bias, dc.weight, ds, db + rb)
+            return pack_deconv_weight_bf16s(pack_conv_weight(wf, transposed=True), _deconv_nterms()), t27
+        return _cache(self).get("u5fold/" + E.CONV_ENGINE + "/%d" % _deconv_nterms(), srcs, build)
+
+    def _up5_folded(self, y, skip):
+        wd, _, _, _, wrs = self._up_params("u5", self.conv5, self.redir2)
+        wfs, t27 = self._up5_folded_params()
+        return E.deconv3d_bf16s_shift27_hip(y, wfs, wd.shape[2], t27, True, _deconv_nterms(), skip, wrs)
 
     def forward(self, x):
         x = dfr.real(x)
@@ -324,9 +356,16 @@
         at("c3")
         c4 = run_convbn(self, "c4", self.conv4[0][0], self.conv4[0][1], c3, relu=True)
         at("c4")
-        c4 = self.attention_block(c4)
-        at("att")
-        c5 = self._up("u5", self.conv5, self.redir2, c4, c2)
+        ab = self.attention_block
+        if (E.ATTN_FOLD and isinstance(ab, attention_block) and ab.folds_final(c4)
+                and self._up_takes_split_engine("u5", self.conv5, self.redir2, c4)):
+            y = ab(c4, final=False)
+            at("att")
+            c5 = self._up5_folded(y, c2)
+        else:
+            c4 = ab(c4)
+            at("att")
+            c5 = self._up("u5", self.conv5, self.redir2, c4, c2)
         at("u5")
         return self._up("u6", self.conv6, self.redir1, c5, x)
 
```
